# alexsmith1612/hadoofus

Measured on AMD Instinct MI355X. Metric: CRC32C verify GiB/s (device-resident), 512B chunks over 128MiB HDFS blocks, higher is better.
Workload: dtype u8; 1 GPU; C3 verify: 1024 x 128MiB HDFS blocks per GPU of splitmix64 data, 512B chunks, BE wire CRCs, 1/65537 chunks corrupted, bitmap + first-bad out; blocks_per_gpu=1024, block_bytes=134217728, chunk_size=512, parallelism=shard1

## Files before the change

hadoofus_amd/abi.py:

```python
import ctypes
import os

import numpy as np

HERE = os.path.dirname(os.path.abspath(__file__))
LIB_PATH = os.path.join(HERE, "lib", "libhadoofus_crc32c.so")

CSUM_NULL, CSUM_CRC32, CSUM_CRC32C = 0, 1, 2
ERR_UNSUPPORTED_CHECKSUM = 8
ERR_INVALID_PACKETHEADERPROTO = 18
ERR_PACKET_SIZE = 25
ERR_CRC_LEN = 26
ERR_UNEXPECTED_CRC_LEN = 27
ERR_UNEXPECTED_READ_OFFSET = 28
ERR_BAD_CHECKSUM = 29
ERR_BAD_LASTPACKET = 32
EIO = -5
READ_ALL = -1
AGAIN = 1000
ABI_VERSION = 5
MODE_COMPUTE, MODE_VERIFY = 0, 1
PROTO_V1, PROTO_V2 = 1, 2
SEG_BE, SEG_RAW, SEG_CRC32 = 1, 2, 4

# ... 84 lines not shown
    _bind(lib, "hdfs_crc32c_plan_kernel_ms", _int, [_vp, ctypes.POINTER(ctypes.c_double), ctypes.POINTER(_int)])
    _bind(lib, "hdfs_crc32c_plan_stats", _int, [_vp, ctypes.POINTER(_u64), ctypes.POINTER(_u64), ctypes.POINTER(_u64)])
    _bind(lib, "hdfs_crc32c_plan_destroy", None, [_vp])
    _bind(lib, "hdfs_crc32c_plan_time", _int, [_vp, _vp, _int, ctypes.POINTER(ctypes.c_double)])
    _bind(lib, "hdfs_crc32c_stream_dev", _int, [_u32, _vp, _u64, ctypes.POINTER(_u32)])
    _bind(lib, "hdfs_crc32c_stream_ex", _int, [_int, _u32, _vp, _u64, ctypes.POINTER(_u32)])
    _bind(lib, "hdfs_crc32c_verify_crcdata", _int,
          [_vp, ctypes.c_int32, ctypes.c_int32, ctypes.c_int32, _int, ctypes.POINTER(ctypes.c_int32)])
    _bind(lib, "hdfs_crc32c_compose_crcs", _int,
          [ctypes.POINTER(_vp), ctypes.POINTER(_sz), _int, _sz, _u32, _int, _vp])
    for name in ("hdfs_crc32c_parse_packets", "hdfs_crc32c_verify_packets"):
        _bind(lib, name, _int, [_vp, _u64, _int, _u32, _int, ctypes.POINTER(Packet), _sz,
                                ctypes.POINTER(_sz), ctypes.POINTER(_u64)])
    _bind(lib, "hdfs_crc32c_read_packets", _int,
          [_vp, _u64, _int, _u32, _int, ctypes.c_int64, ctypes.c_int64, ctypes.POINTER(IoVec), _int,
           ctypes.POINTER(Packet), _sz, ctypes.POINTER(_sz), ctypes.POINTER(_u64), ctypes.POINTER(_u64)])
    _bind(lib, "hdfs_crc32c_verify_packets_submit", _int,
          [_vp, _u64, _int, _u32, _int, _sz, ctypes.POINTER(_vp)])
    _bind(lib, "hdfs_crc32c_job_wait", _int,
          [_vp, ctypes.POINTER(Packet), _sz, ctypes.POINTER(_sz), ctypes.POINTER(_u64)])
    _bind(lib, "hdfs_crc32c_verify_blocks_submit", _int,
          [ctypes.POINTER(_vp), ctypes.POINTER(_u64), _sz, _int, _u32, _int, _sz, ctypes.POINTER(_vp)])
    _bind(lib, "hdfs_crc32c_job_wait_blocks", _int,
          [_vp, ctypes.POINTER(Packet), _sz, ctypes.POINTER(_sz), ctypes.POINTER(_u64), ctypes.POINTER(_int)])
    _bind(lib, "hdfs_crc32c_reader_open", _int,
          [_vp, _u64, _int, _u32, _int, ctypes.c_int64, ctypes.c_int64, _sz, ctypes.POINTER(_vp)])
    _bind(lib, "hdfs_crc32c_reader_next", _int,
          [_vp, ctypes.POINTER(IoVec), _int, ctypes.POINTER(Packet), _sz, ctypes.POINTER(_sz), ctypes.POINTER(_u64),
           ctypes.POINTER(_u64)])
    _bind(lib, "hdfs_crc32c_reader_close", None, [_vp])
    _bind(lib, "hdfs_crc32c_read_packets_fd", _int,
          [_vp, _u64, _int, _u32, _int, ctypes.c_int64, ctypes.c_int64, _int, ctypes.c_int64,
           ctypes.POINTER(Packet), _sz, ctypes.POINTER(_sz), ctypes.POINTER(_u64), ctypes.POINTER(_u64)])
    _bind(lib, "hdfs_crc32c_abi_version", _int, [])
    _bind(lib, "hdfs_crc32c_session_create", _int, [ctypes.POINTER(_vp), _int, _u32, _int, _u64, _sz])
    _bind(lib, "hdfs_crc32c_session_buffer", _int, [_vp, ctypes.POINTER(_vp), ctypes.POINTER(_u64)])
    _bind(lib, "hdfs_crc32c_session_commit", _int, [_vp, _u64])
    _bind(lib, "hdfs_crc32c_session_flush", _int, [_vp])
    _bind(lib, "hdfs_crc32c_session_poll", _int, [_vp, ctypes.POINTER(Packet), _sz, ctypes.POINTER(_sz), _int])
    _bind(lib, "hdfs_crc32c_session_pending", _int, [_vp, ctypes.POINTER(_u64), ctypes.POINTER(_sz)])
    _bind(lib, "hdfs_crc32c_session_destroy", None, [_vp])
    _bind(lib, "hdfs_crc32c_composite_crcs", _int, [ctypes.POINTER(Segment), _sz, ctypes.POINTER(_u32)])
    _bind(lib, "hdfs_crc32c_dev_alloc", _int, [ctypes.POINTER(_vp), _u64])
    _bind(lib, "hdfs_crc32c_dev_free", _int, [_vp])
    _bind(lib, "hdfs_crc32c_memcpy", _int, [_vp, _vp, _u64, _int])
    _bind(lib, "hdfs_crc32c_memset", _int, [_vp, _int, _u64])
    _bind(lib, "hdfs_crc32c_stream_create", _int, [ctypes.POINTER(_vp)])
    _bind(lib, "hdfs_crc32c_stream_destroy", _int, [_vp])
    _bind(lib, "hdfs_crc32c_stream_sync", _int, [_vp])
    _bind(lib, "hdfs_crc32c_fill_splitmix64", _int, [_vp, _u64, _u64, _u64, _vp])
    _bind(lib, "hdfs_crc32c_corrupt", _int, [_vp, _u64, _u32, _u64, _u64, _u64, _vp])
    _bind(lib, "hdfs_crc32c_device_sync", _int, [])
    _bind(lib, "hdfs_crc32c_mailbox_create", _int, [ctypes.POINTER(_vp), _u32])
    _bind(lib, "hdfs_crc32c_mailbox_stats", _int, [_vp, ctypes.POINTER(_u64), ctypes.POINTER(_u64)])
    _bind(lib, "hdfs_crc32c_mailbox_destroy", _int, [_vp])
    _bind(lib, "hdfs_crc32c_compose_packets", _int,
          [_vp, _u64, ctypes.c_int64, ctypes.c_int64, _int, _int, _int, _vp, _u64, ctypes.POINTER(OutPacket), _sz,
           ctypes.POINTER(_sz), ctypes.POINTER(_u64)])
    _bind(lib, "hdfs_crc32c_compute_host", _int, [_vp, _u64, _u32, _u32, _u32, _vp, _u64])
    _bind(lib, "hdfs_crc32c_verify_host", _int,
          [_vp, _u64, _u32, _u32, _u32, _vp, _vp, _u64, ctypes.POINTER(_u64), ctypes.POINTER(_u64)])
    _bind(lib, "hdfs_crc32c_host_alloc", _int, [ctypes.POINTER(_vp), _u64])
    _bind(lib, "hdfs_crc32c_host_free", _int, [_vp])
    return check_abi(lib)


def bind_diag(lib):
    _bind(lib, "hdfs_crc32c_set_tile_order", _int, [_int])
    _bind(lib, "hdfs_crc32c_set_group_shift", _int, [_int])
    _bind(lib, "hdfs_crc32c_set_xcd_major", _int, [_int])
    _bind(lib, "hdfs_crc32c_probe_read", _int, [_vp, _u64, _vp, _int, ctypes.POINTER(ctypes.c_double)])
    _bind(lib, "hdfs_crc32c_set_tuning", _int, [_int, _vp])
    _bind(lib, "hdfs_crc32c_set_probe", _int, [_int, _int, _int])
    _bind(lib, "hdfs_crc32c_set_depth", _int, [_int])
    _bind(lib, "hdfs_crc32c_set_shape", _int, [_int, _int])
    _bind(lib, "hdfs_crc32c_set_store_policy", _int, [_int])
    _bind(lib, "hdfs_crc32c_set_runs", _int, [_int])
    _bind(lib, "hdfs_crc32c_diag_device_checks", _int, [ctypes.POINTER(_u32), _int])
    _bind(lib, "hdfs_crc32c_set_speculation", _int, [_int])
    _bind(lib, "hdfs_crc32c_set_job_coalesce", _int, [_int])
    _bind(lib, "hdfs_crc32c_set_job_early", _int, [_int])
    _bind(lib, "hdfs_crc32c_diag_job_early", _int, [ctypes.POINTER(_u64), _int])
    _bind(lib, "hdfs_crc32c_diag_spec_stats", _int, [ctypes.POINTER(_u64), _int])
    _bind(lib, "hdfs_crc32c_diag_stream_queries", _int, [ctypes.POINTER(_u64)])
    _bind(lib, "hdfs_crc32c_diag_stream_queues", _int, [ctypes.POINTER(_u64)])
    _bind(lib, "hdfs_crc32c_diag_job_queues", _int, [ctypes.POINTER(_u64)])
    return lib


def load(path=LIB_PATH):
    global _lib
    if _lib is not None:
        return _lib
    if not os.path.exists(path):
        raise ImportError(f"{path} not built; run `python -m hadoofus_amd.build` "
                          "(or __graft_entry__.build())")
    _lib = bind_product(ctypes.CDLL(path))
    return _lib


def check_abi(lib):
    v = lib.hdfs_crc32c_abi_version()
    if v != ABI_VERSION:
        raise ImportError(f"library ABI version {v}, bindings written for {ABI_VERSION}")
    return lib


def _check(rc, lib=None):
    if rc != 0:
        raise CRC32CError(rc, (lib or load()).hdfs_crc32c_last_error().decode(errors="replace"))


def _host(buf):
    if isinstance(buf, np.ndarray):
        a = np.ascontiguousarray(buf)
        return a, a.ctypes.data, a.nbytes
    a = np.frombuffer(memoryview(buf).cast("B"), dtype=np.uint8)
    return a, (a.ctypes.data if a.nbytes else None), a.nbytes


def device_info(device=-1):
    arch = ctypes.create_string_buffer(64)
    ncu = _int(0)
    _check(load().hdfs_crc32c_device_info(device, arch, 64, ctypes.byref(ncu)))
    return arch.value.decode(), ncu.value


def init(device=-1):
    _check(load().hdfs_crc32c_init(device))


def bound_device():
    d = _int(-1)
    bus = ctypes.create_string_buffer(64)
    _check(load().hdfs_crc32c_bound_device(ctypes.byref(d), bus, 64))
    return d.value, bus.value.decode()


def crc32c(crc, buf, entry="_hdfs_crc32c"):
    keep, p, n = _host(buf)
    return getattr(load(), entry)(crc & 0xFFFFFFFF, p, n)


def stream_crc_dev(crc, dptr, nbytes):
    out = _u32(0)
    _check(load().hdfs_crc32c_stream_dev(crc & 0xFFFFFFFF, dptr, nbytes, ctypes.byref(out)))
    return out.value


def verify_crcdata(region, chunksize, crcdlen, dlen, ctype=CSUM_CRC32C):
    keep, p, n = _host(region)
    fb = ctypes.c_int32(-1)
    rc = load().hdfs_crc32c_verify_crcdata(p, chunksize, crcdlen, dlen, ctype, ctypes.byref(fb))
    if rc < 0:
        _check(rc)
    return rc, fb.value


def stream_ex(ctype, crc, buf):
    keep, p, n = _host(buf)
    out = _u32(0)
    _check(load().hdfs_crc32c_stream_ex(ctype, crc & 0xFFFFFFFF, p if n else None, n, ctypes.byref(out)))
    return out.value


def _packets(fn, stream, proto, chunk_size, ctype, max_pkts, dptr=None, nbytes=None, lib=None):
# ... 383 lines not shown
```

hadoofus_amd/csrc/crc32c_engine.cpp:

```cpp
#include <hip/hip_runtime.h>

#include <algorithm>
#include <cstdarg>
#include <cstdio>
#include <cstdlib>
#include <chrono>
#include <cstring>
#include <mutex>
#include <string>
#include <vector>

#include <unistd.h>

#include "crc32c_engine.h"
#include "crc32c_tables.h"
#ifdef HDFS_CRC32C_DIAG
#include "hadoofus_crc32c_diag.h"
#endif

namespace hdfs_crc32c {

thread_local char g_err[512] = "";

int fail(int code, const char *fmt, ...) {
  va_list ap;
  va_start(ap, fmt);
  vsnprintf(g_err, sizeof(g_err), fmt, ap);
  va_end(ap);
  return code;
}

DevCtx g_ctx[kMaxDev];
std::mutex g_init_mu;
std::atomic<int> g_bound_dev{-1};

#ifdef HDFS_CRC32C_DIAG
int env_int(const char *name, int dflt) {
  const char *e = std::getenv(name);
  return e ? std::atoi(e) : dflt;
}
#define HDFS_KNOB(name, dflt) env_int(name, dflt)
#else
#define HDFS_KNOB(name, dflt) (dflt)
#endif
int g_tile_order = HDFS_KNOB("HDFS_CRC32C_TILE_ORDER", 3);
int g_nt_loads = HDFS_KNOB("HDFS_CRC32C_NT", 2);
int g_depth = HDFS_KNOB("HDFS_CRC32C_DEPTH", 3);
int g_streams = HDFS_KNOB("HDFS_CRC32C_STREAMS", 1);
int g_block = HDFS_KNOB("HDFS_CRC32C_BLOCK", 1024);
uint32_t g_store_policy = uint32_t(HDFS_KNOB("HDFS_CRC32C_STORE", 0));
uint32_t g_group_shift = uint32_t(HDFS_KNOB("HDFS_CRC32C_GROUP", 3)) & 15u;
uint32_t g_xcd_major = uint32_t(HDFS_KNOB("HDFS_CRC32C_XCD", 1)) & 3u;
uint32_t g_spec_pool_min = uint32_t(HDFS_KNOB("HDFS_CRC32C_SPEC_POOL", 32)) & 255u;
uint32_t g_copy_wg_units = uint32_t(HDFS_KNOB("HDFS_CRC32C_COPY_WG_UNITS", 1024));
int g_copy_dev_tab = HDFS_KNOB("HDFS_CRC32C_COPY_DEV_TAB", 1);
int g_tail_small = HDFS_KNOB("HDFS_CRC32C_TAIL_SMALL", 1);
int g_tail_stream = HDFS_KNOB("HDFS_CRC32C_TAIL_STREAM", 1);
uint64_t g_mb_copy_max = uint64_t(HDFS_KNOB("HDFS_CRC32C_MB_COPY_MAX", 96 << 10));
int g_runs = HDFS_KNOB("HDFS_CRC32C_RUNS", 2);
int g_spec = HDFS_KNOB("HDFS_CRC32C_SPEC", 1);
int g_job_coalesce = HDFS_KNOB("HDFS_CRC32C_JOB_COALESCE", 1);
int g_job_early = HDFS_KNOB("HDFS_CRC32C_JOB_EARLY", 1);
std::atomic<uint64_t> g_job_early_stats[2];
int g_job_queues = HDFS_KNOB("HDFS_CRC32C_JOB_QUEUES", 1);
int g_stage_vram = HDFS_KNOB("HDFS_CRC32C_MB_STAGE", 1);
int g_mb_exp = HDFS_KNOB("HDFS_CRC32C_MB_EXP", 0);
int g_mb_queue = HDFS_KNOB("HDFS_CRC32C_MB_QUEUE", 1);
unsigned long long *g_diag = nullptr;


int stream_queue(hipStream_t s, uint64_t *dq, uint64_t *q) {
  HIPCHK(launch_queue_probe(dq, s));
  HIPCHK(hipMemcpyAsync(q, dq, sizeof(uint64_t), hipMemcpyDeviceToHost, s));
  HIPCHK(hipStreamSynchronize(s));
  return HDFS_CRC32C_OK;
}

int stream_on_own_queue(DevCtx &c, hipStream_t *s, uint64_t *q, const uint64_t *avoid, int n) {
  *s = nullptr;
  *q = 0;
  uint64_t *dq = nullptr;
  HIPCHK(hipMalloc(&dq, sizeof(uint64_t)));
  auto shared = [&](uint64_t x) {
    for (int i = 0; i < n; i++)
      if (avoid[i] && avoid[i] == x) return true;
    return false;
  };
  int rc = HDFS_CRC32C_OK;
  if (hipStreamCreateWithFlags(s, hipStreamNonBlocking) != hipSuccess) {
    (void)hipGetLastError();
    *s = nullptr;
    rc = fail(HDFS_CRC32C_EHIP, "stream");
  } else if (!(rc = stream_queue(*s, dq, q)) && g_job_queues && shared(*q)) {
    std::vector<uint32_t> mask(size_t((c.num_cu + 31) / 32), 0u);
    for (int cu = 0; cu < c.num_cu; cu++) mask[size_t(cu / 32)] |= 1u << (cu % 32);
    hipStream_t own = nullptr;
    uint64_t q2 = 0;
    if (hipExtStreamCreateWithCUMask(&own, uint32_t(mask.size()), mask.data()) != hipSuccess) {
      (void)hipGetLastError();
    } else if (!stream_queue(own, dq, &q2) && !shared(q2)) {
      (void)hipStreamDestroy(*s);
      *s = own;
      *q = q2;
    } else {
      (void)hipStreamDestroy(own);
    }
  }
  (void)hipFree(dq);
  return rc;
}

int queue_probe_streams(DevCtx &c) {
  uint64_t *dq = nullptr;
  HIPCHK(hipMalloc(&dq, sizeof(uint64_t)));
  int rc = stream_queue(c.stream, dq, &c.q_main);
  for (int k = 0; k < 2 && !rc; k++) {
    hipStream_t &s = k == 0 ? c.t_stream : c.cp_stream;
    uint64_t &q = k == 0 ? c.q_tail : c.q_copy;
    if ((rc = stream_queue(s, dq, &q))) break;
    if (q != c.q_main) continue;
    std::vector<uint32_t> mask(size_t((c.num_cu + 31) / 32), 0u);
    for (int cu = 0; cu < c.num_cu; cu++) mask[size_t(cu / 32)] |= 1u << (cu % 32);
    hipStream_t own = nullptr;
    uint64_t q2 = 0;
    if (hipExtStreamCreateWithCUMask(&own, uint32_t(mask.size()), mask.data()) != hipSuccess) {
      (void)hipGetLastError();
      continue;
    }
    if ((rc = stream_queue(own, dq, &q2))) break;
    if (q2 == c.q_main) {
      (void)hipStreamDestroy(own);
      continue;
    }
    (void)hipStreamDestroy(s);
    s = own;
    q = q2;
  }
  (void)hipFree(dq);
  return rc;
}

int ctx_init(int device, DevCtx **out) {
  int ndev = 0;
// ... 1297 lines not shown
    (void)hipFree(dq);
    if (rc) return rc;
  }
  const uint64_t ms = idle_ms ? idle_ms : 50u;
  c->mb_idle_ticks = uint32_t(std::min<uint64_t>(ms * 100000u, 0xFFFFFFFFu));
  c->mb_calls = c->mb_launches = 0;
  HIPCHK(hipStreamSynchronize(c->stream));
  c->mb_on = true;
  rc = mb_launch(*c, c->mb_posted);
  if (rc) {
    c->mb_on = false;
    return rc;
  }
  *mb = new hdfs_crc32c_mailbox{c->dev};
  return HDFS_CRC32C_OK;
}

int hdfs_crc32c_mailbox_stats(const hdfs_crc32c_mailbox *mb, uint64_t *calls, uint64_t *launches) {
  if (!mb) return fail(HDFS_CRC32C_EINVAL, "null mailbox");
  DevCtx &c = g_ctx[mb->dev];
  std::lock_guard<std::mutex> lk(c.mu);
  if (calls) *calls = c.mb_calls;
  if (launches) *launches = c.mb_launches;
  return HDFS_CRC32C_OK;
}

int hdfs_crc32c_mailbox_destroy(hdfs_crc32c_mailbox *mb) {
  if (!mb) return HDFS_CRC32C_OK;
  DevCtx &c = g_ctx[mb->dev];
  DeviceGuard g(mb->dev);
  delete mb;
  std::lock_guard<std::mutex> lk(c.mu);
  if (!c.mb_on) return HDFS_CRC32C_OK;
  c.mb_on = false;
  if (c.mb_alive && !mb_exited(c)) {
    mb_post(c, ++c.small_seq, 0u, kMbQuitFlag, 0u, nullptr);
  }
  c.mb_alive = false;
  HIPCHK(hipStreamSynchronize(c.mb_stream));
  return HDFS_CRC32C_OK;
}

#ifdef HDFS_CRC32C_DIAG
int hdfs_crc32c_diag_device_checks(uint32_t *out3, int reset) {
  if (!out3) return fail(HDFS_CRC32C_EINVAL, "null output");
  const hipError_t e = read_device_checks(out3, reset);
  if (e != hipSuccess) return fail(HDFS_CRC32C_EHIP, "reading the device checks: %s", hipGetErrorString(e));
  return HDFS_CRC32C_OK;
}

int hdfs_crc32c_set_store_policy(int policy) {
  if (policy < 0 || policy > 28) return fail(HDFS_CRC32C_EINVAL, "store policy 0..28");
  g_store_policy = uint32_t(policy);
  return HDFS_CRC32C_OK;
}

int hdfs_crc32c_diag_stream_queries(uint64_t *out) {
  DevCtx *c = nullptr;
  int rc = ctx_init(-1, &c);
  if (rc) return rc;
  if (!out) return fail(HDFS_CRC32C_EINVAL, "null out");
  *out = c->stream_queries;
  return HDFS_CRC32C_OK;
}

int hdfs_crc32c_diag_stream_queues(uint64_t *out4) {
  DevCtx *c = nullptr;
  int rc = ctx_init(-1, &c);
  if (rc) return rc;
  if (!out4) return fail(HDFS_CRC32C_EINVAL, "null out");
  out4[0] = c->q_main;
  out4[1] = c->q_tail;
  out4[2] = c->q_copy;
  out4[3] = c->q_mb;
  return HDFS_CRC32C_OK;
}

int hdfs_crc32c_set_speculation(int on) {
  if (on != 0 && on != 1) return fail(HDFS_CRC32C_EINVAL, "speculation 0 or 1");
  g_spec = on;
  return HDFS_CRC32C_OK;
}

int hdfs_crc32c_diag_job_queues(uint64_t *out4) {
  DevCtx *c = nullptr;
  int rc = ctx_init(-1, &c);
  if (rc) return rc;
  if (!out4) return fail(HDFS_CRC32C_EINVAL, "null out");
  std::lock_guard<std::mutex> lk(c->mu);
  for (int i = 0; i < kMaxJobs; i++) out4[i] = c->job_slot[i].q;
  return HDFS_CRC32C_OK;
}

int hdfs_crc32c_set_job_coalesce(int mode) {
  if (mode < 0 || mode > 3)
    return fail(HDFS_CRC32C_EINVAL, "job coalescing 0 (off), 1 (product), 2 (hold) or 3 (no lone run behind a launch)");
  g_job_coalesce = mode;
  return HDFS_CRC32C_OK;
}

int hdfs_crc32c_set_job_early(int on) {
  if (on < 0 || on > 1) return fail(HDFS_CRC32C_EINVAL, "per-run completion 0 (off) or 1 (product)");
  g_job_early = on;
  return HDFS_CRC32C_OK;
}

int hdfs_crc32c_diag_job_early(uint64_t *out2, int reset) {
  if (!out2) return fail(HDFS_CRC32C_EINVAL, "null out");
  for (int i = 0; i < 2; i++) out2[i] = reset ? g_job_early_stats[i].exchange(0) : g_job_early_stats[i].load();
  return HDFS_CRC32C_OK;
}

int hdfs_crc32c_set_runs(int on) {
  if (on < 0 || on > 4)
    return fail(HDFS_CRC32C_EINVAL, "runs 0 (schedule 3), 1 (schedule 4), 2 (gather), 3 (lazy gather) or 4 (columns)");
  g_runs = on;
  return HDFS_CRC32C_OK;
}

int hdfs_crc32c_set_depth(int depth) {
  if (depth < 2 || depth > 4) return fail(HDFS_CRC32C_EINVAL, "depth must be 2..4");
  g_depth = depth;
  return HDFS_CRC32C_OK;
}

int hdfs_crc32c_set_shape(int streams, int block) {
  if (streams != 1 && streams != 2 && streams != 4) return fail(HDFS_CRC32C_EINVAL, "streams must be 1, 2 or 4");
  if (block != 512 && block != 768 && block != 1024) return fail(HDFS_CRC32C_EINVAL, "block must be 512, 768 or 1024");
  g_streams = streams;
  g_block = block;
  return HDFS_CRC32C_OK;
}

int hdfs_crc32c_set_tuning(int nt_loads, void *diag) {
  if (nt_loads < 0 || nt_loads > 2) return fail(HDFS_CRC32C_EINVAL, "nt_loads 0..2");
  g_nt_loads = nt_loads;
  g_diag = static_cast<unsigned long long *>(diag);
  return HDFS_CRC32C_OK;
}

int hdfs_crc32c_set_group_shift(int shift) {
  if (shift < 0 || shift > 6) return fail(HDFS_CRC32C_EINVAL, "group shift must be 0..6");
  g_group_shift = uint32_t(shift);
  return HDFS_CRC32C_OK;
}

int hdfs_crc32c_set_xcd_major(int on) {
  if (on < 0 || on > 2) return fail(HDFS_CRC32C_EINVAL, "xcd_major must be 0, 1 or 2");
  g_xcd_major = uint32_t(on);
  return HDFS_CRC32C_OK;
}

int hdfs_crc32c_set_tile_order(int order) {
  if (order < 0 || order > 3) return fail(HDFS_CRC32C_EINVAL, "tile order must be 0..3");
  g_tile_order = order;
  return HDFS_CRC32C_OK;
}

int g_probe_variant = 0, g_probe_grid_per_cu = 2, g_probe_block = 1024;

int hdfs_crc32c_set_probe(int variant, int grid_per_cu, int block) {
  g_probe_variant = variant;
  g_probe_grid_per_cu = grid_per_cu > 0 ? grid_per_cu : 2;
  g_probe_block = block > 0 ? block : 1024;
  return HDFS_CRC32C_OK;
}
// ... 76 lines not shown
```

hadoofus_amd/csrc/crc32c_engine.h:

```cpp
#pragma once
#include <hip/hip_runtime.h>

#include <atomic>
#include <cstdarg>
#include <cstddef>
#include <cstdint>
#include <initializer_list>
#include <mutex>
#include <vector>

#include "crc32c_hostpin.h"
#include "crc32c_internal.h"
#include "hadoofus_crc32c.h"

namespace hdfs_crc32c {

hipError_t launch_tiles(int mode, int order, int nt, int depth, int streams, int block, int grid,
                        const SegDev *segs, uint32_t nseg, uint64_t total_rounds, uint64_t total_tiles,
                        const uint32_t *gtab, uint32_t *first_bad, unsigned long long *mism,
                        unsigned long long *diag, uint32_t tune, uint32_t *gctr, hipStream_t stream,
                        int copy = 0, int una = 0, const GridSummary *dyn = nullptr, uint32_t utiles = 0,
                        int fuse_generic = 0);
hipError_t launch_probe_read(const uint8_t *p, uint64_t nbytes, uint32_t *out, int grid, int block, int variant,
                             hipStream_t stream);
hipError_t launch_generic(int mode, const SegDev *segs, uint32_t nseg, uint64_t total_gtiles,
                          const uint32_t *gtab, uint32_t *first_bad, unsigned long long *mism,
                          hipStream_t stream, const GridSummary *dyn = nullptr);
hipError_t launch_combine(const uint32_t *raws, uint64_t nraw, uint32_t cs, uint64_t len,
                          const uint32_t *pow2, uint32_t reg0, uint32_t *acc, hipStream_t stream);
hipError_t launch_fill(uint64_t *out, uint64_t nwords, uint64_t seed, uint64_t g0, hipStream_t stream);
hipError_t launch_corrupt(uint8_t *data, uint64_t len, uint32_t cs, uint64_t chunk0, uint64_t modulus,
                          uint64_t bitmul, hipStream_t stream);
hipError_t launch_composite(const SegDev *segs, uint32_t nseg, const uint64_t *run_prefix, uint64_t total_runs,
                            const uint32_t *pow2, uint32_t *out, hipStream_t stream);
hipError_t launch_small_chunks(int mode, const uint8_t *p, uint32_t len, uint32_t exact, uint32_t cs, uint32_t reg0,
                               uint32_t be, const uint32_t *expect, const uint32_t *tab, const uint32_t *kx,
                               uint32_t poly, uint32_t *meta, uint32_t *crcs, uint32_t seq, hipStream_t stream);
hipError_t launch_prep(uint32_t *fb, uint32_t nfb, unsigned long long *mism, uint32_t *gctr, hipStream_t stream);
hipError_t launch_queue_probe(uint64_t *out, hipStream_t stream);
int stream_queue(hipStream_t s, uint64_t *dq, uint64_t *q);
hipError_t launch_mailbox(const uint32_t *req, const uint8_t *in, uint32_t *meta, uint32_t *crcs, const uint32_t *tab0,
                          const uint32_t *tab1, const uint32_t *kx, uint32_t *status, uint32_t epoch, uint32_t seq0,
                          uint32_t idle_ticks, uint32_t exp, hipStream_t stream);
hipError_t launch_gather(const uint8_t *raw, const PktDesc *descs, uint32_t npk, uint32_t units, uint8_t *arena,
                         uint8_t *crc_arena, hipStream_t stream);
hipError_t launch_header_window(const uint8_t *s, uint64_t len, uint64_t base, uint64_t stride, uint32_t count,
                                int proto, uint8_t *out, uint64_t *stride_out, hipStream_t stream);

hipError_t launch_copy_pieces(const CopyPieces &a, int grid, hipStream_t stream);
hipError_t launch_copy_beside(const CopyPieces &a, int grid, hipStream_t stream);
hipError_t launch_small_run(const uint8_t *s, uint64_t len, uint32_t count, int proto, uint32_t cs, int ctype,
                            int verify, const uint32_t *tab, const uint32_t *pow2, uint8_t *copy_dst,
                            uint64_t copy_cap, int win, int64_t client_offset, uint8_t *hout, uint32_t seq,
                            hipStream_t stream);
hipError_t launch_frame_grid(const uint8_t *s, uint64_t len, uint64_t base, uint32_t count, int proto, uint32_t cs,
                             int ctype, int verify, uint32_t sflags, uint8_t *bm_base, uint8_t *copy_base,
                             uint64_t copy_cap, int win, int64_t client_offset, GridBufs g, hipStream_t stream,
                             unsigned long long *stamps = nullptr);
hipError_t launch_spec_verify(const SpecArgs &a, int grid, int copy, hipStream_t stream);
extern int g_spec;
extern int g_job_coalesce;
extern int g_job_early;
extern std::atomic<uint64_t> g_job_early_stats[2];
extern int g_job_queues;
extern unsigned long long *g_diag;
constexpr size_t kFrameStampOff = 65536;
hipError_t launch_grid_finalize(const SegDev *segs, uint32_t nseg, const uint32_t *seg2pkt, const uint32_t *fb,
                                GridBad *bad, uint32_t bad_cap, GridSummary *sum, uint8_t *hsum2, uint32_t host_cap,
                                uint32_t seq, hipStream_t stream);

extern thread_local char g_err[512];
int fail(int code, const char *fmt, ...);
hipError_t read_device_checks(uint32_t out[3], int reset);
int device_checks(const char *call);

#define HIPCHK(expr)                                                                   \
  do {                                                                                 \
    hipError_t e_ = (expr);                                                            \
    if (e_ != hipSuccess)                                                              \
      return ::hdfs_crc32c::fail(HDFS_CRC32C_EHIP, "%s: %s (%s:%d)", #expr,            \
                                 hipGetErrorString(e_), __FILE__, __LINE__);           \
  } while (0)

constexpr int kMaxDev = 64;
constexpr uint32_t kStreamPiece = 4096;
constexpr size_t kStageCap = size_t(64) << 20;
constexpr size_t kSmallIn = kSmallMax + size_t(kSmallMaxChunks) * 4 + 64;
constexpr uint32_t kSmallMeta = 16;
constexpr size_t kSmallOut = (kSmallMeta + size_t(kSmallMaxChunks)) * 4;

struct PieceSlot {
  uint8_t *raw = nullptr, *arena = nullptr, *crc = nullptr, *meta = nullptr;
  size_t raw_cap = 0, arena_cap = 0, crc_cap = 0, meta_cap = 0;
  uint32_t *gctr = nullptr;
  unsigned long long *mism = nullptr;
  hipEvent_t copied = nullptr;
  hipEvent_t done = nullptr;
};

struct CopyCtl {
  uint32_t *hdone = nullptr, *ddone = nullptr, *count = nullptr;
  uint32_t seq = 0;
  uint8_t *htab = nullptr, *dtab = nullptr;
  size_t tab_cap = 0;
  uint8_t *vtab = nullptr;
  size_t vtab_cap = 0;
};

struct SpecSlot {
  SpecCtl *ctl = nullptr;
  SpecExc *exc = nullptr;
  SpecRunTail *xtail = nullptr;
  SpecTabData *tabs = nullptr;
  uint8_t *h = nullptr, *hd = nullptr;
  uint64_t n = 0;
  hipStream_t stream = nullptr;
  uint64_t q = 0;
  uint8_t *scratch = nullptr;
  uint64_t scratch_cap = 0;
};
constexpr int kMaxJobs = 4;
constexpr size_t kMaxJobsOut = 64;
struct JobQueue;

struct DevCtx {
  std::atomic<bool> ready{false};
  int dev = -1;
  int num_cu = 0;
  int num_xcd = 8;
  char arch[64] = "";
  uint32_t *d_tab_main_t[2] = {nullptr, nullptr};
  uint32_t *d_tab_pow2_t[2] = {nullptr, nullptr};
  uint32_t *d_tab_kx = nullptr;
  hipStream_t stream = nullptr;
  uint8_t *h_stage = nullptr;
  uint8_t *d_stage = nullptr;
  uint32_t *d_raw = nullptr;
  size_t raw_cap = 0;
  SegDev *d_seg = nullptr;
  uint32_t *d_small = nullptr;
  uint8_t *h_small_in = nullptr, *dv_small_in = nullptr;
  uint8_t *stage_vram = nullptr;
  uint32_t *h_small_out = nullptr, *dv_small_out = nullptr;
  uint32_t small_seq = 0;
  std::atomic<uint64_t> queued_epoch{0}, confirmed_epoch{0};
  bool unconfirmed() const {
    return queued_epoch.load(std::memory_order_acquire) != confirmed_epoch.load(std::memory_order_acquire);
  }
  void confirm(uint64_t e) {
    uint64_t cur = confirmed_epoch.load(std::memory_order_acquire);
    while (cur < e && !confirmed_epoch.compare_exchange_weak(cur, e, std::memory_order_acq_rel)) {
    }
  }
  uint64_t stream_queries = 0;
  void *d_crc_scratch = nullptr;
  uint64_t crc_scratch_cap = 0;
  hipStream_t copy_stream = nullptr, comp_stream = nullptr;
  hipEvent_t ev_copy[2] = {nullptr, nullptr}, ev_comp[2] = {nullptr, nullptr};
  uint8_t *p_data[2] = {nullptr, nullptr};
  uint32_t *p_crc[2] = {nullptr, nullptr};
  uint8_t *p_bm[2] = {nullptr, nullptr};
  size_t p_cap = 0;
  size_t p_chunk_cap = 0;
  SegDev *p_segs = nullptr;
  uint32_t *p_fb = nullptr;
  uint32_t *p_gctr = nullptr;
  unsigned long long *p_mism = nullptr;
  size_t p_npieces_cap = 0;
  PieceSlot kslot[2];
  uint8_t *k_hmeta = nullptr;
  size_t k_hmeta_cap = 0;
  uint8_t *w_dev = nullptr, *w_host = nullptr;
  uint32_t w_cap = 0;
  struct VBatch {
    uint8_t *h = nullptr, *d = nullptr;
    size_t hcap = 0, dcap = 0;
  };
  std::vector<VBatch> v_batch;
  hipStream_t v_stream = nullptr;
  struct GridSlot {
    uint8_t *d = nullptr, *h = nullptr;
    size_t dcap = 0, hcap = 0;
    uint8_t *hd = nullptr;
  };
  uint32_t grid_seq = 0;
  uint8_t *sr_h = nullptr, *sr_hd = nullptr;
  uint8_t *sr2_h = nullptr, *sr2_hd = nullptr;
  hipStream_t t_stream = nullptr;
  uint64_t q_main = 0, q_tail = 0, q_copy = 0, q_mb = 0;
  hipStream_t r_stream = nullptr;
  std::vector<GridSlot> grid;
  SpecSlot spec;
  SpecSlot job_slot[kMaxJobs];
  bool job_busy[kMaxJobs] = {};
  JobQueue *jobq = nullptr;
  std::mutex rd_mu;
  uint8_t *rd_stage = nullptr;
  uint64_t rd_stage_cap = 0;
  CopyCtl cp;
  CopyCtl cp_beside;
  hipStream_t cp_stream = nullptr;
  std::mutex beside_mu;
  std::vector<CopyCtl> cp_pool;
  bool mb_on = false, mb_alive = false;
  uint32_t *h_mb = nullptr, *dv_mb = nullptr;
  uint32_t *mb_req = nullptr, *mb_req_d = nullptr;
  uint32_t mb_posted = 0;
  hipStream_t mb_stream = nullptr;
  uint32_t mb_epoch = 0, mb_idle_ticks = 0;
  uint64_t mb_calls = 0, mb_launches = 0;
  std::vector<hipStream_t> user_streams;
  int bulk_cus() const { return num_cu - (mb_on ? num_xcd : 0); }
  std::mutex mu;
};

extern DevCtx g_ctx[kMaxDev];
int stream_on_own_queue(DevCtx &c, hipStream_t *s, uint64_t *q, const uint64_t *avoid, int n);

struct DeviceGuard {
  int prev = -1;
  bool changed = false;
  explicit DeviceGuard(int dev) {
    if (hipGetDevice(&prev) == hipSuccess && prev != dev) {
      changed = hipSetDevice(dev) == hipSuccess;
    }
  }
  ~DeviceGuard() {
    if (changed) (void)hipSetDevice(prev);
  }
};

int ctx_init(int device, DevCtx **out);
void classify(SegDev &s, uint64_t &rounds, uint64_t &gtiles, uint64_t &mtiles);
int fill_seg(const hdfs_crc32c_segment &in, int mode, SegDev &s, size_t idx);
inline int seg_ctype(uint32_t flags) { return (flags & HDFS_CRC32C_SEG_CRC32) ? 1 : 0; }
bool device_accessible(const void *p);
int launch_all(DevCtx &c, int mode, const SegDev *d_segs, uint32_t nseg, uint64_t rounds, uint64_t mtiles,
               uint64_t gtiles, uint32_t *d_fb, unsigned long long *d_mism, uint32_t *d_gctr, hipStream_t st,
               hipEvent_t ev0 = nullptr, hipEvent_t ev1 = nullptr, bool reset = true, int ctype = 0,
               bool copy = false, bool gctr_zeroed = false, bool una = false, uint32_t utiles = 0,
               bool runs = false);
bool whole_groups(const SegDev *segs, size_t n);
uint32_t uniform_tiles(const SegDev *segs, size_t n);
int launch_verify_dyn(DevCtx &c, const SegDev *d_segs, const GridSummary *dyn, uint64_t rounds_ub, uint64_t gtiles_ub,
                      uint32_t *d_fb, unsigned long long *d_mism, uint32_t *d_gctr, hipStream_t st, int ctype,
                      bool copy);
uint32_t tile_tune();
extern uint32_t g_spec_pool_min;
extern uint32_t g_copy_wg_units;
extern int g_copy_dev_tab;
bool any_unaligned(const SegDev *segs, size_t n);
int pipe_reserve(DevCtx &c, size_t piece, uint32_t cs, size_t npieces);
int mailbox_copy(DevCtx &c, const CopyEntry *e, uint32_t n);
extern uint64_t g_mb_copy_max;
extern int g_tail_small;
extern int g_tail_stream;

bool small_ok(uint64_t len, uint64_t cs);
int small_call(DevCtx &c, int mode, uint32_t len, uint32_t cs, uint32_t reg0, bool be, int ctype,
               const uint8_t *dsrc = nullptr, const uint8_t *hsrc = nullptr, const uint8_t *hcrc = nullptr,
               uint32_t crc_bytes = 0);
int chunk_crcs_to_host(const void *data, uint64_t len, uint32_t cs, int ctype, uint32_t *out_be);
int host_pipeline(int mode, const uint8_t *data, uint64_t len, uint32_t cs, uint32_t flags, uint32_t crc_init,
                  void *crcs, uint8_t *bitmap, uint64_t piece_req, uint64_t *first_bad, uint64_t *mismatches);

PinRegistry &pins();
struct HostPins {
  PinRegistry::Scope s;
  std::vector<hipStream_t> drain;
  bool finished = false;
  explicit HostPins(std::initializer_list<hipStream_t> st) : s(pins()), drain(st) {}
  HostPins(const HostPins &) = delete;
  HostPins &operator=(const HostPins &) = delete;
  ~HostPins() {
    if (!finished)
      for (hipStream_t st : drain)
        if (st) (void)hipStreamSynchronize(st);
  }
  int pin(std::initializer_list<std::pair<const void *, size_t>> bufs);
  int done(int rc);
};

inline uint64_t align_up(uint64_t v, uint64_t a) { return (v + a - 1) / a * a; }

}
```

hadoofus_amd/csrc/crc32c_internal.h:

```cpp
#pragma once
#include <cstdint>

struct hdfs_crc32c_packet;

namespace hdfs_crc32c {

#ifdef HDFS_CRC32C_DIAG
constexpr bool kDiag = true;
#else
constexpr bool kDiag = false;
#endif

enum DevCheckKernel : uint32_t {
  kDkFrameGrid = 1,
  kDkGridBuild = 2,
  kDkHeaderWindow = 3,
  kDkSmallRun = 4,
  kDkFinalize = 5,
  kDkSpecEarly = 6,
};

enum : uint32_t {
  kSegBigEndian = 1u,
  kSegRaw = 2u,
};

enum Mode : int { kModeCompute = 0, kModeVerify = 1, kModeLoadOnly = 2 };

struct SegDev {
  const uint8_t *data;
  uint32_t *crcs;
  uint8_t *bitmap;
  uint64_t mtile_start;
  uint32_t chunk_size;
  uint32_t flags;
  uint32_t nchunks;
  uint32_t main_tiles;
  uint32_t reg_init;
  uint32_t gen_tiles;
  uint64_t len;
  uint64_t round_start;
  uint64_t gtile_start;
  uint8_t *copy_dst;
  uint32_t copy_w0, copy_w1;
};
static_assert(sizeof(SegDev) == 96, "SegDev layout");

enum : uint32_t {
  kGridOn = 0,
  kGridOff = 1,
  kGridStop = 2,
  kGridMore = 3,
};
struct GridSummary {
  uint32_t first_break;
  uint32_t recorded;
  uint32_t last_status;
  uint32_t nseg;
  uint64_t stride;
  uint64_t rounds, mtiles, gtiles;
  uint64_t payload;
  uint64_t consumed;
  uint64_t next_pos;
  uint64_t bm_bytes;
  uint32_t nbad;
  uint32_t unaligned;
  uint32_t seq;
  uint32_t nonuni;
  uint32_t utiles;
  uint32_t nexc;
};
constexpr uint32_t kExcMax = 64;
constexpr uint32_t kGridRecBytes = 56;
constexpr uint32_t kGridHostRec0 = 256;
constexpr uint32_t kGridHostIdx = kGridHostRec0 + 64;
constexpr uint32_t kGridHostExc = kGridHostIdx + kExcMax * 4;
constexpr uint32_t kGridHostBytes = kGridHostExc + kExcMax * kGridRecBytes;
struct GridBufs {
  ::hdfs_crc32c_packet *recs;
  void *look;
  SegDev *segs;
  uint32_t *seg2pkt;
  uint32_t *fb;
  uint32_t *gctr;
  uint32_t *done;
  uint32_t *exc;
  GridSummary *sum;
  uint8_t *hsum;
  uint32_t seq;
};
constexpr uint32_t kGridLookBytes = 256;

constexpr uint32_t kSpecExcMax = 64;
struct SpecExc {
  uint64_t rec[7];
  uint32_t k, pad;
};
static_assert(sizeof(SpecExc) == 64, "SpecExc");
struct SpecCtl {
  unsigned long long mism;
  uint32_t gctr;
  uint32_t done;
// ... 1 lines not shown
  uint32_t tail_status;
  uint64_t tail_total;
  uint64_t tail[7];
  uint32_t nexc, pad0;
  uint32_t run_done[16];
  uint32_t run_mism[16];
  uint32_t run_bad, pad1[7];
};
static_assert(sizeof(SpecCtl) == 256, "SpecCtl");
struct SpecEarly {
  uint64_t r0[7];
  uint64_t stride;
  uint32_t eligible;
  uint32_t count;
  uint32_t seq;
  uint32_t pad[13];
};
struct SpecFinal {
  unsigned long long mism;
  uint32_t exc, tail_status;
  uint64_t tail_total;
  uint64_t tail[7];
  uint32_t seq, nexc;
  uint32_t pad[10];
};
static_assert(sizeof(SpecEarly) == 128 && sizeof(SpecFinal) == 128, "spec host blocks");
constexpr uint32_t kSpecRunsMax = 16;
struct SpecRunEarly {
  uint64_t r0[7];
  uint32_t count;
  uint32_t early;
};
static_assert(kSpecRunsMax == 16, "SpecCtl's per-run words");
struct SpecRunTail {
  uint64_t rec[7];
  uint64_t total;
  uint32_t status, seq;
};
struct SpecRunDone {
  uint32_t seq, mism, bad, pad;
};
static_assert(sizeof(SpecRunEarly) == 64 && sizeof(SpecRunTail) == 72 && sizeof(SpecRunDone) == 16, "spec run blocks");
constexpr size_t kSpecRunEarlyOff = 256 + size_t(kSpecExcMax) * sizeof(SpecExc);
constexpr size_t kSpecRunTailOff = kSpecRunEarlyOff + size_t(kSpecRunsMax) * sizeof(SpecRunEarly);
constexpr size_t kSpecRunDoneOff = kSpecRunTailOff + size_t(kSpecRunsMax) * sizeof(SpecRunTail);
constexpr size_t kSpecHostBytes = kSpecRunDoneOff + size_t(kSpecRunsMax) * sizeof(SpecRunDone);
struct SpecTabData {
  const uint8_t *crc0;
  uint8_t *bm0, *copy_base;
  uint64_t stride, copy_cap;
  uint32_t nch, cs, cb0, nruns;
  uint64_t um;
  uint32_t per, pad;
  const uint8_t *crc0r[kSpecRunsMax];
  SpecCtl *ctl;
  uint8_t *hdone;
  uint32_t seq, pad1;
};
static_assert(sizeof(SpecTabData) == 56 + 16 + 128 + 24, "SpecTabData");
struct SpecArgs {
  const uint8_t *s;
  uint64_t len, base;
  uint32_t max_count;
  int proto, ctype;
  uint32_t cs, sflags;
  int rwin;
  int64_t client_offset;
  uint8_t *bm;
  uint8_t *copy_base;
  uint64_t copy_cap;
  const uint32_t *gtab;
  uint32_t *fb;
  SpecCtl *ctl;
  SpecExc *exc;
  uint32_t parity, seq, tune;
  uint8_t *hout;
  SpecTabData *tabs;
  unsigned long long *stamps;
  uint32_t nruns;
  uint32_t early;
  const uint8_t *xs[kSpecRunsMax];
  uint64_t xlen[kSpecRunsMax];
  SpecRunTail *xtail;
};
constexpr size_t kSpecStampOff = 98304;
constexpr uint64_t kSpecMaxStride = uint64_t(1) << 26;

struct GridBad {
  uint32_t pkt;
  int32_t first_bad;
  uint32_t bad_chunks;
  uint32_t pad;
};


constexpr uint32_t kLdsSliceBytes = 131072;
constexpr uint32_t kLdsZposBytes = 7 * 4096;
constexpr uint32_t kLdsBytes = kLdsSliceBytes + kLdsZposBytes;
constexpr uint32_t kLdsWords = kLdsBytes / 4;

constexpr uint32_t kTabSliceWords = 1024;
constexpr uint32_t kTabZposWords = 7 * 1024;
constexpr uint32_t kTabMainWords = kTabSliceWords + kTabZposWords;
constexpr uint32_t kPow2Levels = 48;
constexpr uint32_t kTabPow2Words = kPow2Levels * 1024;

constexpr uint32_t kTabKxWords = 1088;

struct PktDesc {
  uint64_t src_crc;
  uint64_t dst_data;
  uint64_t dst_crc;
  uint32_t dlen;
  uint32_t ncrc;
  uint32_t unit0;
  uint32_t nunits;
};
constexpr uint32_t kGatherSlice = 65536;
constexpr uint32_t kHdrWin = 64;

constexpr uint32_t kGridMaxCount = 65536;
constexpr uint32_t kGridGroups = kGridMaxCount / 64 / 64;

constexpr uint32_t kSmallRunMax = 64;
constexpr uint32_t kCopyPiecesMax = 32;
constexpr uint32_t kCopyBlocksMax = 512;
constexpr uint32_t kCopyTabBlocks = 4096;
constexpr uint32_t kCopyTabGrid = 1024;
constexpr uint32_t kCopyTabStage = 64;
struct CopyEntry {
  const uint8_t *src;
  uint8_t *dst;
  uint32_t len, uend;
};
static_assert(sizeof(CopyEntry) == 24, "CopyEntry layout (the mailbox reads it as 6 words)");
struct CopyPieces {
  const uint8_t *src[kCopyPiecesMax];
  uint8_t *dst[kCopyPiecesMax];
  uint32_t len[kCopyPiecesMax];
  uint32_t uend[kCopyPiecesMax];
  uint32_t n, seq;
  uint32_t *done;
  uint32_t *count;
  const CopyEntry *tab;
  const uint32_t *wg0;
  uint32_t per, total;
  unsigned long long *stamps;
};
constexpr size_t kCopyStampOff = 110592;
inline uint32_t copy_units(uintptr_t d, uint64_t len) {
  return len ? uint32_t(((d + len + 15u) & ~uintptr_t(15)) - (d & ~uintptr_t(15))) / 16u : 0u;
}
constexpr uint32_t kSrSlot = 128;
constexpr uint32_t kSrHostBytes = kSmallRunMax * kSrSlot;
constexpr uint64_t kSmallRunBytes = uint64_t(kSmallRunMax) * (65536 + 4096);

constexpr uint32_t kSmallMax = 65536;
constexpr uint32_t kSmallMaxChunks = 2048;

constexpr uint32_t kMbVerifyFlag = 1u << 24, kMbBeFlag = 1u << 25, kMbCrc32Flag = 1u << 26, kMbQuitFlag = 1u << 27;
constexpr uint32_t kMbDevFlag = 1u << 28;
constexpr uint32_t kMbCopyFlag = 1u << 29;


constexpr uint32_t kRoundBytes = 512;
constexpr uint32_t kTileChunks = 8;
// ... 3 lines not shown
```

hadoofus_amd/csrc/crc32c_kernels.hip:

```cpp
#include <hip/hip_runtime.h>

#include "crc32c_frame.h"
#include "crc32c_internal.h"

namespace hdfs_crc32c {

#define DEV __device__ __forceinline__

typedef uint32_t u32x4 __attribute__((ext_vector_type(4)));
#define GAS __attribute__((address_space(1)))
DEV u32x4 gload16(const void *p) { return *(const GAS u32x4 *)(const GAS uint8_t *)p; }
DEV u32x4 gload16_nt(const void *p) {
  return __builtin_nontemporal_load((const GAS u32x4 *)(const GAS uint8_t *)p);
}
DEV uint32_t gload32(const void *p) { return *(const GAS uint32_t *)(const GAS uint8_t *)p; }
DEV uint8_t gload8(const void *p) { return *(const GAS uint8_t *)p; }
DEV void gstore32(void *p, uint32_t v) { *(GAS uint32_t *)(GAS uint8_t *)p = v; }
DEV void gstore8(void *p, uint8_t v) { *(GAS uint8_t *)p = v; }

DEV uint32_t lds_at(const uint32_t *lds, uint32_t byteaddr) {
  return *reinterpret_cast<const uint32_t *>(reinterpret_cast<const char *>(lds) + byteaddr);
}

template <int CTRL>
// ... 8 lines not shown

DEV uint32_t xor3(uint32_t a, uint32_t b, uint32_t c) { return __builtin_amdgcn_bitop3_b32(a, b, c, 0x96); }

DEV uint32_t slice4(const uint32_t *lds, uint32_t x, uint32_t next, uint32_t lb0, uint32_t lb1) {
  const uint32_t a0 = __builtin_amdgcn_perm(x, lb0, 0x0C020400u);
  const uint32_t a1 = __builtin_amdgcn_perm(x, lb0, 0x0C020500u);
  const uint32_t a2 = __builtin_amdgcn_perm(x, lb1, 0x0C020600u);
  const uint32_t a3 = __builtin_amdgcn_perm(x, lb1, 0x0C020700u);
  return xor3(xor3(lds_at(lds, a0), lds_at(lds, a1 + 128u), lds_at(lds, a2)), lds_at(lds, a3 + 128u), next);
}

DEV uint32_t zshift(const uint32_t *lds, uint32_t base, uint32_t x) {
  const uint32_t *t = lds + base;
  return t[x & 0xffu] ^ t[256u + ((x >> 8) & 0xffu)] ^ t[512u + ((x >> 16) & 0xffu)] ^
         t[768u + (x >> 24)];
}

DEV void transpose(uint32_t (&d)[16]) {
#pragma unroll
  for (int c = 0; c < 4; c++) {
#pragma unroll
    for (int k = 0; k < 4; k += 2) {
      const auto r = __builtin_amdgcn_permlane16_swap(d[k * 4 + c], d[(k + 1) * 4 + c], false, false);
      d[k * 4 + c] = r[0];
      d[(k + 1) * 4 + c] = r[1];
    }
  }
#pragma unroll
  for (int c = 0; c < 4; c++) {
#pragma unroll
    for (int k = 0; k < 2; k++) {
      const auto r = __builtin_amdgcn_permlane32_swap(d[k * 4 + c], d[(k + 2) * 4 + c], false, false);
      d[k * 4 + c] = r[0];
      d[(k + 2) * 4 + c] = r[1];
    }
  }
}

DEV uint32_t rfl(uint32_t x) { return __builtin_amdgcn_readfirstlane(x); }
DEV uint64_t rfl64(uint64_t x) {
  return (static_cast<uint64_t>(rfl(static_cast<uint32_t>(x >> 32))) << 32) | rfl(static_cast<uint32_t>(x));
}

#ifdef HDFS_CRC32C_DIAG
__device__ uint32_t g_dchk[4];
DEV bool dchk(bool ok, uint32_t kid, uint32_t line) {
  if (!ok && atomicAdd(&g_dchk[2], 1u) == 0u) {
    g_dchk[0] = kid;
    g_dchk[1] = line;
  }
  return ok;
}
#define DCHK(c, kid) dchk((c), (kid), __LINE__)
#else
#define DCHK(c, kid) true
#endif

#define CAS __attribute__((address_space(4)))
typedef const CAS SegDev *SegP;

struct SegHot {
  const uint8_t *data;
  uint32_t *crcs;
  uint8_t *bitmap;
  uint64_t mtile_start;
  uint32_t chunk_size, flags, nchunks, main_tiles;
};
static_assert(sizeof(SegHot) == 48, "SegHot is the head of SegDev");
DEV SegHot seg_hot(SegP segs, uint32_t s) {
  const CAS SegHot *p = reinterpret_cast<const CAS SegHot *>(&segs[s]);
  return SegHot{p->data, p->crcs, p->bitmap, p->mtile_start, p->chunk_size, p->flags, p->nchunks, p->main_tiles};
}

DEV void spec_run_contribute(SpecCtl *ctl, uint8_t *hdone, uint32_t seq, uint32_t target, uint32_t r) {
  const uint32_t n = __hip_atomic_fetch_add(&ctl->run_done[r], 1u, __ATOMIC_RELAXED, __HIP_MEMORY_SCOPE_AGENT);
  if (n + 1u != target) return;
  const uint32_t mism = __hip_atomic_load(&ctl->run_mism[r], __ATOMIC_RELAXED, __HIP_MEMORY_SCOPE_AGENT);
  const uint32_t bad = (__hip_atomic_load(&ctl->run_bad, __ATOMIC_RELAXED, __HIP_MEMORY_SCOPE_AGENT) >> r) & 1u;
  *(volatile GAS u32x4 *)(GAS uint8_t *)(hdone + sizeof(SpecRunDone) * r) = u32x4{seq, mism, bad, 0u};
}

constexpr uint32_t kEarlyWords = 50, kEarlyOff = 0xFFFFFFFFu;

template <bool BATCH>
struct SpecTabT {
  const CAS SpecTabData *p;
  uint32_t *e;
  DEV uint32_t early_ok(uint32_t nk) const {
    if constexpr (BATCH) return rfl(e[49] != 0u && e[48] == nk ? 1u : 0u);
    return 0u;
  }
  DEV void tile_done(uint32_t k, uint32_t byte, uint32_t lane) const {
    if constexpr (BATCH) {
      const uint32_t r = rfl(static_cast<uint32_t>(__umul64hi(static_cast<uint64_t>(k), p->um)));
      SpecCtl *const ctl = p->ctl;
      if (byte) {
        if (lane == 0)
          __hip_atomic_fetch_add(&ctl->run_mism[r], static_cast<uint32_t>(__builtin_popcount(byte)), __ATOMIC_RELAXED,
                                 __HIP_MEMORY_SCOPE_AGENT);
        __builtin_amdgcn_s_waitcnt(0x0F70);
      }
      uint32_t old = 0;
      if (lane == 0) old = __hip_atomic_fetch_add(&e[r], 1u, __ATOMIC_RELAXED, __HIP_MEMORY_SCOPE_WORKGROUP);
      old = __builtin_amdgcn_readlane(old, 0);
      if (old + 1u == rfl(e[16u + r]) && lane == 0) spec_run_contribute(ctl, p->hdone, p->seq, e[32u + r], r);
    }
  }
  DEV SegDev operator[](uint32_t k) const {
    SegDev d;
    SpecTabData q;
    q.crc0 = p->crc0;
    q.bm0 = p->bm0;
    q.copy_base = p->copy_base;
    q.stride = p->stride;
    q.copy_cap = p->copy_cap;
    q.nch = p->nch;
    q.cs = p->cs;
    q.cb0 = p->cb0;
    const uint32_t T = (q.nch + kTileChunks - 1u) / kTileChunks, dlen = q.nch * q.cs;
    const uint8_t *c;
    if constexpr (BATCH) {
      const uint32_t r = static_cast<uint32_t>(__umul64hi(static_cast<uint64_t>(k), p->um));
      c = p->crc0r[r] + static_cast<uint64_t>(k - r * p->per) * q.stride;
    } else {
      c = q.crc0 + static_cast<uint64_t>(k) * q.stride;
    }
    d.data = c + 4u * q.nch;
    d.crcs = reinterpret_cast<uint32_t *>(const_cast<uint8_t *>(c));
    d.bitmap = q.bm0 + static_cast<uint64_t>(k) * T;
    d.mtile_start = static_cast<uint64_t>(k) * T;
    d.chunk_size = q.cs;
    d.flags = kSegBigEndian;
    d.nchunks = q.nch;
    d.main_tiles = T;
    d.reg_init = 0xFFFFFFFFu;
    d.gen_tiles = 0u;
    d.len = dlen;
    d.round_start = static_cast<uint64_t>(k) * T * (q.cs / kRoundBytes);
    d.gtile_start = 0u;
    const uint32_t w0 = k ? 0u : q.cb0;
    const uint64_t before = k ? static_cast<uint64_t>(k) * dlen - q.cb0 : 0u;
    uint64_t at = 0;
    uint32_t clen = 0;
    frame::read_place(before, dlen - w0, q.copy_cap, at, clen);
    d.copy_dst = q.copy_base && clen ? q.copy_base + at : nullptr;
    d.copy_w0 = w0;
    d.copy_w1 = w0 + clen;
    return d;
  }
};
using SpecTab = SpecTabT<false>;
template <class Tab>
struct TabEarly {
  static constexpr bool value = false;
};
template <>
struct TabEarly<SpecTabT<true>> {
  static constexpr bool value = true;
};
template <bool BATCH>
DEV SegHot seg_hot(const SpecTabT<BATCH> &t, uint32_t k) {
  const SegDev d = t[k];
  return SegHot{d.data, d.crcs, d.bitmap, d.mtile_start, d.chunk_size, d.flags, d.nchunks, d.main_tiles};
}

struct SegCache {
  uint32_t seg;
  uint32_t reg_init;
  SegHot h;
};
template <class Tab>
DEV const SegCache &hot(SegCache &k, Tab segs, uint32_t s) {
  if (s != k.seg) {
    k.h = seg_hot(segs, s);
    k.reg_init = segs[s].reg_init;
    k.seg = s;
  }
  return k;
}

struct Cursor {
  uint32_t seg, tile, r;
  bool valid;
  uint32_t grp = 0;
};

constexpr uint32_t kUnitMaxShift = 8, kUnitMinShift = 4;
constexpr uint32_t kColBytes = 128;
constexpr uint32_t kColShift = 2;
constexpr uint32_t kSlots = 8;
#ifndef HDFS_GATHER_SLOTS
#define HDFS_GATHER_SLOTS 8
#endif
static_assert((HDFS_GATHER_SLOTS & (HDFS_GATHER_SLOTS - 1)) == 0, "gather slots: a power of two");
constexpr uint32_t kGatherSlots = HDFS_GATHER_SLOTS, kGatherWords = kGatherSlots * 65;
#ifndef HDFS_PHASE1_NUM
#define HDFS_PHASE1_NUM 23
#endif
constexpr uint64_t kPhase1Num = HDFS_PHASE1_NUM, kPhase1Den = 25;

struct Sched {
  uint64_t r1;
  uint64_t gfirst;
  uint32_t nk;
  uint32_t *ctr;
  uint32_t lane;
  uint64_t p2first;
  uint64_t ntiles;
  uint32_t *gctr;
  uint64_t *slots;
  uint32_t ushift;
  uint32_t gstride;
  uint32_t gshift;
  uint32_t ut, ush;
  uint64_t um;
};

DEV Cursor ulocate(const Sched &w, uint64_t g) {
  const uint32_t s = w.ush != 0xFFFFFFFFu ? static_cast<uint32_t>(g >> w.ush) : static_cast<uint32_t>(__umul64hi(g, w.um));
  return Cursor{rfl(s), rfl(static_cast<uint32_t>(g - uint64_t(s) * w.ut)), 0u, true};
}

DEV uint32_t grab(const Sched &w) {
  uint32_t k = 0;
  if (w.lane == 0) k = atomicAdd(w.ctr, 1u);
  return rfl(k);
}

template <int ORDER>
DEV bool ticket_tile(const Sched &w, uint32_t t, uint64_t &g) {
  if (t < w.nk) {
    if (ORDER == 4 || ORDER == 7)
      g = (w.gfirst + uint64_t(t) * w.gstride) << w.gshift;
    else if (ORDER == 3)
      g = ((w.gfirst + uint64_t(t >> w.gshift) * w.gstride) << w.gshift) + (t & ((1u << w.gshift) - 1u));
    else
      g = w.gfirst + t;
    return true;
  }
  if (ORDER < 2) return false;
  const uint32_t tsh = (ORDER == 4 || ORDER == 7) ? w.gshift : 0u;
  const uint32_t j = t - w.nk, u = j >> (w.ushift - tsh), o = (j & ((1u << (w.ushift - tsh)) - 1u)) << tsh,
                 s = u % kSlots;
  if (o == 0) {
    uint32_t gu = 0;
    if (w.lane == 0) gu = atomicAdd(w.gctr, 1u);
    gu = rfl(gu);
    if (w.lane == 0)
      __hip_atomic_store(&w.slots[s], (uint64_t(u + 1) << 32) | gu, __ATOMIC_RELAXED, __HIP_MEMORY_SCOPE_WORKGROUP);
  }
  uint64_t v;
  for (;;) {
    v = __hip_atomic_load(&w.slots[s], __ATOMIC_RELAXED, __HIP_MEMORY_SCOPE_WORKGROUP);
    if (rfl(static_cast<uint32_t>(v >> 32)) == u + 1) break;
    __builtin_amdgcn_s_sleep(2);
  }
  g = w.p2first + (uint64_t(rfl(static_cast<uint32_t>(v))) << w.ushift) + o;
  return g < w.ntiles;
}

constexpr uint64_t kWalkTiles = 64;

template <class Tab>
DEV Cursor locate(Tab segs, uint32_t s, uint64_t g) {
  while (g >= segs[s].mtile_start + segs[s].main_tiles) s++;
  return Cursor{rfl(s), rfl(static_cast<uint32_t>(g - segs[s].mtile_start)), 0u, true};
}

template <int ORDER, class Tab>
DEV Cursor find_tile(const Cursor c, const SegHot &sh, Tab segs, uint32_t nseg, const Sched &w, uint64_t g) {
  const uint64_t end = sh.mtile_start + sh.main_tiles;
  if (w.ut && (g < sh.mtile_start || g >= end)) return ulocate(w, g);
  if (g < sh.mtile_start || g >= end + (ORDER >= 3 ? 0u : kWalkTiles)) {
    uint32_t lo = 0, hi = nseg;
    while (hi - lo > 1) {
      const uint32_t mid = (lo + hi) >> 1;
      if (segs[mid].mtile_start <= g) lo = mid; else hi = mid;
    }
    return locate(segs, lo, g);
  }
  if (g < end)
    return Cursor{c.seg, rfl(static_cast<uint32_t>(g - sh.mtile_start)), 0u, true};
  return locate(segs, c.seg, g);
}

template <int ORDER, class Tab>
DEV Cursor advance(Cursor c, Tab segs, uint32_t nseg, const Sched &w, SegCache &kc) {
  if (!c.valid) return c;
  const SegHot &sh = hot(kc, segs, c.seg).h;
  if (c.r + 1 < (ORDER == 7 ? sh.chunk_size / kColBytes : sh.chunk_size / kRoundBytes)) {
    c.r++;
    return c;
  }
  if (ORDER == 4 && ((c.tile + 1u) & ((1u << w.gshift) - 1u)) != 0u) {
    c.tile++;
    c.r = 0;
    return c;
  }
  if (ORDER != 0) {
    uint64_t g;
    const uint32_t tk = grab(w);
    if (!ticket_tile<ORDER>(w, tk, g)) {
      c.valid = false;
      return c;
    }
    Cursor n = find_tile<ORDER>(c, sh, segs, nseg, w, g);
    n.grp = tk >> 3;
    return n;
  }
  uint32_t s = c.seg, t = c.tile + 1;
  while (s < nseg && t >= segs[s].main_tiles) {
    t = 0;
    s++;
  }
  if (s >= nseg || segs[s].round_start + uint64_t(t) * (segs[s].chunk_size / kRoundBytes) >= w.r1) {
    c.valid = false;
    return c;
  }
  return Cursor{rfl(s), rfl(t), 0u, true};
}
// ... 480 lines not shown
        c = lds_at(lds, L.lb1 + 128u + (((c ^ gload8(p++)) & 0xffu) << 8)) ^ (c >> 8);
        n--;
      }
      out = (flags & kSegRaw) ? c : ~c;
    }
  }
  bool bad = false;
  if (valid) {
    uint32_t e = gload32(segs[s].crcs + chunk);
    if (flags & kSegBigEndian) e = __builtin_bswap32(e);
    bad = e != out;
  }
  const uint64_t m = __ballot(bad);
  if (active && g == 0) {
    const uint32_t byte = static_cast<uint32_t>((m >> (L.lane & 56u)) & 0xffu);
    gstore8(segs[s].bitmap + tile, static_cast<uint8_t>(byte));
    if (byte) {
      atomicMin(&first_bad[s], tile * kTileChunks + __builtin_ctz(byte));
      atomicAdd(mism, static_cast<unsigned long long>(__builtin_popcount(byte)));
    }
  }
}

template <int BLOCK>
DEV void bad_list(const SegDev *__restrict__ segs, uint32_t nseg, const uint32_t *__restrict__ seg2pkt,
                  const uint32_t *__restrict__ fb, GridBad *__restrict__ bad, uint32_t bad_cap,
                  GridSummary *__restrict__ sum, uint8_t *__restrict__ hsum2, uint32_t host_cap, uint32_t seq,
                  uint32_t *nb) {
  if (threadIdx.x == 0) *nb = 0u;
  __syncthreads();
  auto *hbad = reinterpret_cast<GridBad *>(hsum2 + 256);
  for (uint32_t i0 = threadIdx.x; i0 < nseg; i0 += 16u * BLOCK) {
    uint32_t f[16];
#pragma unroll
    for (uint32_t u = 0; u < 16; u++) f[u] = i0 + u * BLOCK < nseg ? fb[i0 + u * BLOCK] : 0xFFFFFFFFu;
#pragma unroll
    for (uint32_t u = 0; u < 16; u++) {
      if (f[u] == 0xFFFFFFFFu) continue;
      const uint32_t i = i0 + u * BLOCK;
      const SegDev d = segs[i];
      const uint32_t nbyte = (d.nchunks + 7u) / 8u;
      uint32_t n = 0;
      for (uint32_t j0 = 0; j0 < nbyte; j0 += 16u) {
        uint32_t by[16];
#pragma unroll
        for (uint32_t u = 0; u < 16; u++) by[u] = j0 + u < nbyte ? uint32_t(d.bitmap[j0 + u]) : 0u;
#pragma unroll
        for (uint32_t u = 0; u < 16; u++) {
          uint32_t byte = by[u];
          if (j0 + u == d.nchunks / 8u) byte &= (1u << (d.nchunks % 8u)) - 1u;
          n += __builtin_popcount(byte);
        }
      }
      const uint32_t slot = atomicAdd(nb, 1u);
      const GridBad g{seg2pkt[i], int32_t(f[u]), n, 0u};
      if (slot < bad_cap) bad[slot] = g;
      if (slot < host_cap) hbad[slot] = g;
    }
  }
  __syncthreads();
  if (threadIdx.x == 0) {
    sum->nbad = *nb;
    reinterpret_cast<GridSummary *>(hsum2)->nbad = *nb;
  }
  __threadfence_system();
  __syncthreads();
  if (threadIdx.x == 0)
    __hip_atomic_store(&reinterpret_cast<GridSummary *>(hsum2)->seq, seq, __ATOMIC_RELAXED, __HIP_MEMORY_SCOPE_SYSTEM);
}

template <int BLOCK>
DEV void fused_generic(const uint32_t *lds, const SegDev *__restrict__ segs, const GridSummary *__restrict__ dyn,
                       const LaneConst &L, uint32_t *__restrict__ first_bad, unsigned long long *__restrict__ mism) {
  const uint32_t nseg = dyn->nseg;
  const uint64_t ngt = dyn->gtiles;
  const uint64_t nw = uint64_t(gridDim.x) * (BLOCK / 64);
  const uint64_t wid = uint64_t(blockIdx.x) * (BLOCK / 64) + (threadIdx.x >> 6);
  for (uint64_t g0 = wid * 8u; g0 < ngt; g0 += nw * 8u) {
    const uint64_t gt = g0 + (L.lane >> 3);
    fused_generic_chunk(lds, segs, nseg, gt, gt < ngt, L, first_bad, mism);
  }
}

template <int BLOCK, int GATHER>
DEV void fill_tables(uint32_t *lds, const uint32_t *__restrict__ gtab) {
  if (threadIdx.x < 2 + 2 * kSlots) lds[kLdsWords + threadIdx.x] = 0u;
  if (GATHER && threadIdx.x < kGatherSlots) lds[kLdsWords + 2 + 2 * kSlots + threadIdx.x] = threadIdx.x << 4;
  constexpr uint32_t kStores = kLdsSliceBytes / 16;
  constexpr uint32_t kQ = (kStores + BLOCK - 1) / BLOCK;
  constexpr uint32_t kZ = (kTabZposWords / 4 + BLOCK - 1) / BLOCK;
  uint32_t v[kQ];
#pragma unroll
  for (uint32_t k = 0; k < kQ; k++) {
    const uint32_t idx = 4u * min(k * BLOCK + threadIdx.x, kStores - 1u);
    const uint32_t P = idx >> 14, e = (idx >> 6) & 255u, h = (idx >> 5) & 1u;
    v[k] = gtab[(3u - (2u * P + h)) * 256u + e];
  }
  u32x4 z[kZ];
#pragma unroll
  for (uint32_t k = 0; k < kZ; k++) {
    const uint32_t q = k * BLOCK + threadIdx.x;
    z[k] = q < kTabZposWords / 4 ? gload16(gtab + kTabSliceWords + 4u * q) : u32x4{0u, 0u, 0u, 0u};
  }
#pragma unroll
  for (uint32_t k = 0; k < kQ; k++) {
    const uint32_t q = k * BLOCK + threadIdx.x;
    if (kStores % BLOCK == 0 || q < kStores)
      *reinterpret_cast<u32x4 *>(&lds[4u * q]) = u32x4{v[k], v[k], v[k], v[k]};
  }
#pragma unroll
  for (uint32_t k = 0; k < kZ; k++) {
    const uint32_t q = k * BLOCK + threadIdx.x;
    if (q < kTabZposWords / 4) *reinterpret_cast<u32x4 *>(&lds[kLdsSliceBytes / 4 + 4u * q]) = z[k];
  }
}

template <int MODE, int ORDER, int NT, int DEPTH, int S, int BLOCK, int BUF, int COPY, int UNA, int GATHER,
          class Tab>
DEV void tiles_run(uint32_t *lds, const Tab sg, const SegDev *__restrict__ segs, uint32_t nseg, uint64_t total_rounds,
                   uint64_t total_tiles, uint32_t *__restrict__ first_bad, unsigned long long *__restrict__ mism,
                   unsigned long long *__restrict__ diag, uint32_t tune, uint32_t *__restrict__ gctr,
                   const GridSummary *__restrict__ dyn, uint32_t utiles, bool fused) {
  static_assert(ORDER != 0 || S == 1, "static per-wave slices serve one stream");
  static_assert(ORDER != 7 || (MODE == kModeCompute && S == 1 && BUF && !COPY && !UNA && !GATHER), "columns shape");
  static_assert(DEPTH >= 2 && DEPTH <= 4 && S >= 1 && S <= 4, "shape");
  static_assert(GATHER == 0 || (MODE == kModeCompute && ORDER == 3 && S == 1), "gather: compute, schedule 3");
  LaneConst L;
  L.store_policy = EP::policy(tune & 0xffu);
  L.lane = threadIdx.x & 63u;
  L.hsel = (L.lane >> 3) & 1u;
  L.loff = 16u * (4u * (L.lane & 7u) + (L.lane >> 4));
  L.lb0 = (L.lane & 31u) * 4u;
  L.lb1 = 65536u + (L.lane & 31u) * 4u;
  L.qi = L.lane & 7u;
  L.qg = L.lane >> 3;
  L.zk = 7u - L.qi;
  L.zbase = kLdsSliceBytes / 4 + (L.zk ? L.zk - 1u : 0u) * 1024u;
  L.z448 = kLdsSliceBytes / 4 + 6u * 1024u;
  L.z64 = kLdsSliceBytes / 4;
  L.ntiles = total_tiles;
  L.gslot = &lds[kLdsWords + 2 + 2 * kSlots];
  L.rmask = 7u;
  L.early = 0u;

  constexpr uint32_t wpb = BLOCK / 64;
  const uint32_t wave = rfl(blockIdx.x * wpb + (threadIdx.x >> 6));
  const uint32_t nwaves = gridDim.x * wpb;
  if (kDiag && diag && L.lane == 0) diag[3 * wave] = __builtin_amdgcn_s_memrealtime();
  uint64_t nrounds = 0;
  Sched w{0, 0, 0, &lds[kLdsWords], L.lane};
  w.ut = utiles;
  w.ush = (utiles & (utiles - 1u)) == 0u ? static_cast<uint32_t>(__builtin_ctz(utiles | (utiles == 0u ? 1u : 0u)))
                                         : 0xFFFFFFFFu;
  w.um = (utiles && w.ush == 0xFFFFFFFFu) ? ~0ull / utiles + 1ull : 0ull;
  Cursor cur[DEPTH][S];
#pragma unroll
  for (int s = 0; s < S; s++) cur[0][s] = Cursor{0u, 0u, 0u, false};
  if (ORDER == 0) {
    Cursor &c0 = cur[0][0];
    const uint64_t r0 = rfl64(total_rounds * wave / nwaves);
    w.r1 = rfl64(total_rounds * (wave + 1) / nwaves);
    if (r0 < w.r1) {
      const uint64_t g = tile_at_round(sg, nseg, r0, total_tiles);
      if (g < total_tiles) {
        uint32_t lo = 0, hi = nseg;
        while (hi - lo > 1) {
          const uint32_t mid = (lo + hi) >> 1;
          if (sg[mid].mtile_start <= g) lo = mid; else hi = mid;
        }
        c0 = locate(sg, lo, g);
        c0.valid = sg[c0.seg].round_start + uint64_t(c0.tile) * (sg[c0.seg].chunk_size / kRoundBytes) < w.r1;
      }
    }
  } else {
    const uint32_t pmin = (tune >> 16) & 0xffu;
    const bool pool = ORDER >= 2 && total_rounds >= uint64_t(pmin ? pmin : 32u) * nwaves * S;
    if (ORDER >= 3) {
      w.gshift = ORDER == 7 ? kColShift : ORDER == 4 ? min((tune >> 8) & 15u, 3u) : (tune >> 8) & 15u;
      if (ORDER == 4) L.rmask = (1u << w.gshift) - 1u;
      const uint64_t ngroups = (pool ? total_tiles * kPhase1Num / kPhase1Den : total_tiles) >> w.gshift;
      const uint32_t b = blockIdx.x, G = gridDim.x, xm = (tune >> 12) & 3u;
      if (xm == 2u && (G % 8u) == 0 && ngroups >= 8ull * (G / 8u)) {
        const uint64_t ngx = ngroups / 8u;
        const uint32_t G8 = G / 8u, l = b / 8u;
        w.gfirst = (b % 8u) * ngx + l;
        w.gstride = G8;
        w.nk = static_cast<uint32_t>(((ngx - 1 - l) / G8 + 1) << (ORDER == 4 || ORDER == 7 ? 0u : w.gshift));
        w.p2first = (ngx * 8u) << w.gshift;
      } else {
        w.gfirst = xm != 0u && (G % 8u) == 0 ? (b % 8u) * (G / 8u) + b / 8u : b;
        w.gstride = gridDim.x;
        w.nk = ngroups > w.gfirst
                   ? static_cast<uint32_t>(((ngroups - 1 - w.gfirst) / gridDim.x + 1) << (ORDER == 4 || ORDER == 7 ? 0u : w.gshift))
                   : 0u;
        w.p2first = ngroups << w.gshift;
      }
    } else {
      const uint64_t r_static = pool ? total_rounds * kPhase1Num / kPhase1Den : total_rounds;
      const uint64_t b0 = rfl64(r_static * blockIdx.x / gridDim.x);
      const uint64_t b1 = rfl64(r_static * (blockIdx.x + 1) / gridDim.x);
      w.gfirst = tile_at_round(sg, nseg, b0, total_tiles);
      w.nk = static_cast<uint32_t>(tile_at_round(sg, nseg, b1, total_tiles) - w.gfirst);
      w.p2first = tile_at_round(sg, nseg, r_static, total_tiles);
    }
    w.ntiles = total_tiles;
    if constexpr (TabEarly<Tab>::value) L.early = sg.early_ok(w.nk);
    {
      const uint64_t per = (total_tiles - w.p2first) / (4ull * gridDim.x);
      w.ushift = per >= (1ull << kUnitMaxShift) ? kUnitMaxShift
               : per < (1ull << kUnitMinShift) ? kUnitMinShift
                                               : 63u - static_cast<uint32_t>(__builtin_clzll(per));
    }
    w.gctr = gctr;
    w.slots = reinterpret_cast<uint64_t *>(&lds[kLdsWords + 2]);
#pragma unroll
    for (int s = 0; s < S; s++) {
      uint64_t g;
      const uint32_t tk = grab(w);
      if (ticket_tile<ORDER>(w, tk, g)) {
        if (w.ut) {
          cur[0][s] = ulocate(w, g);
        } else {
          uint32_t lo = 0, hi = nseg;
          while (hi - lo > 1) {
            const uint32_t mid = (lo + hi) >> 1;
            if (sg[mid].mtile_start <= g) lo = mid; else hi = mid;
          }
          cur[0][s] = locate(sg, lo, g);
        }
        cur[0][s].grp = tk >> 3;
      }
    }
  }
  bool any = false;
#pragma unroll
  for (int s = 0; s < S; s++) any |= cur[0][s].valid;
  if (!any) {
    if constexpr (MODE == kModeVerify)
      if (fused) fused_generic<BLOCK>(lds, segs, dyn, L, first_bad, mism);
    if (kDiag && diag && L.lane == 0) diag[3 * wave + 1] = __builtin_amdgcn_s_memrealtime();
    return;
  }
#pragma unroll
  for (int s = 1; s < S; s++)
    if (!cur[0][s].valid) cur[0][s] = Cursor{cur[0][0].seg, cur[0][0].tile, cur[0][0].r, false};

  uint32_t buf[DEPTH][S][16];
  uint32_t ex[DEPTH][S];
  uint32_t tl[DEPTH][S];
  uint32_t sha[DEPTH][S];
  uint32_t st[S];
  Gst gs[S];
  LaneOff lo{0u, {0u, 0u, 0u, 0u}, 0u};
  SegCache kc[S];
#pragma unroll
  for (int s = 0; s < S; s++) {
    st[s] = 0u;
    gs[s] = Gst{0u, 0u, 0u, 0u, kNoSlot, 0u, 0u, 0u, 0u, nullptr};
    kc[s].seg = 0xFFFFFFFFu;
  }
#pragma unroll
  for (int k = 1; k < DEPTH; k++) {
#pragma unroll
    for (int s = 0; s < S; s++) cur[k][s] = advance<ORDER>(cur[k - 1][s], sg, nseg, w, kc[s]);
  }
#pragma unroll
  for (int k = 0; k < DEPTH; k++) {
#pragma unroll
    for (int s = 0; s < S; s++) {
      ex[k][s] = 0u;
      tl[k][s] = 0u;
      sha[k][s] = 0u;
      issue<MODE, NT, BUF, UNA, ORDER == 7>(buf[k][s], ex[k][s], tl[k][s], sha[k][s], cur[k][s], sg, L.hsel, L.loff, L.qg, L.lane,
                                lo, kc[s], L.store_policy);
    }
    if (k + 1 < DEPTH) {
      constexpr int RUN = ORDER == 7 ? 4 : (ORDER == 4 && MODE == kModeCompute) ? 1 : GATHER == 2 ? 3 : GATHER ? 2 : 0;
#pragma unroll
      for (int j = 0; j < S * round_stores<MODE, COPY, RUN>(); j++) pad_store(first_bad);
    }
  }
  for (uint32_t it = 0;; it++) {
    EP::loop_hook(L.store_policy, it);
#pragma unroll
    for (int k = 0; k < DEPTH; k++) {
      process<MODE, S, COPY, UNA,
              ORDER == 7 ? 4 : (ORDER == 4 && MODE == kModeCompute) ? 1 : GATHER == 2 ? 3 : GATHER ? 2 : 0>(
          lds, buf[k], ex[k], tl[k], sha[k], cur[k], sg, st, L, first_bad, mism, kc, gs);
#pragma unroll
      for (int s = 0; s < S; s++) nrounds += cur[k][s].valid ? 1u : 0u;
      const int prev = (k + DEPTH - 1) % DEPTH;
#pragma unroll
      for (int s = 0; s < S; s++) {
        cur[k][s] = advance<ORDER>(cur[prev][s], sg, nseg, w, kc[s]);
        issue<MODE, NT, BUF, UNA, ORDER == 7>(buf[k][s], ex[k][s], tl[k][s], sha[k][s], cur[k][s], sg, L.hsel, L.loff, L.qg,
                                  L.lane, lo, kc[s], L.store_policy);
      }
    }
    bool more = false;
#pragma unroll
    for (int s = 0; s < S; s++) more |= cur[0][s].valid;
    if (!more) break;
  }
  if constexpr (GATHER == 2) {
#pragma unroll
    for (int s = 0; s < S; s++) {
      lazy_pre(gs[s], cur[0][s], sg, kc[s], L);
      lazy_flush<EP>(gs[s], hot(kc[s], sg, cur[0][s].seg).h, L);
    }
  }
  if constexpr (MODE == kModeVerify)
    if (fused) fused_generic<BLOCK>(lds, segs, dyn, L, first_bad, mism);
  if (kDiag && diag && L.lane == 0) {
    diag[3 * wave + 1] = __builtin_amdgcn_s_memrealtime();
    diag[3 * wave + 2] = nrounds;
  }
}

template <int MODE, int ORDER, int NT, int DEPTH, int S, int BLOCK, int BUF = 0, int COPY = 0, int UNA = 0,
          int GATHER = 0>
__global__ __launch_bounds__(BLOCK) void crc32c_tiles_kernel(
    const SegDev *__restrict__ segs, uint32_t nseg, uint64_t total_rounds, uint64_t total_tiles,
    const uint32_t *__restrict__ gtab, uint32_t *__restrict__ first_bad,
    unsigned long long *__restrict__ mism, unsigned long long *__restrict__ diag, uint32_t tune,
    uint32_t *__restrict__ gctr, const GridSummary *__restrict__ dyn, uint32_t utiles, uint32_t fuse) {
  const bool fused = MODE == kModeVerify && dyn && fuse;
  if (dyn) {
    nseg = dyn->nseg;
    total_rounds = dyn->rounds;
    total_tiles = dyn->mtiles;
    utiles = dyn->utiles;
  }
  __shared__ __attribute__((aligned(16))) uint32_t lds[kLdsWords + 2 + 2 * kSlots + (GATHER ? kGatherWords : 0)];
  fill_tables<BLOCK, GATHER>(lds, gtab);
  __syncthreads();
  tiles_run<MODE, ORDER, NT, DEPTH, S, BLOCK, BUF, COPY, UNA, GATHER>(lds, (SegP)(segs), segs, nseg, total_rounds,
                                                                       total_tiles, first_bad, mism, diag, tune, gctr,
                                                                       dyn, utiles, fused);
}


template <int MODE>
__global__ __launch_bounds__(256) void crc32c_generic_kernel(
    const SegDev *__restrict__ segs, uint32_t nseg, uint64_t total_gtiles,
    const uint32_t *__restrict__ gtab, uint32_t *__restrict__ first_bad,
    unsigned long long *__restrict__ mism, const GridSummary *__restrict__ dyn) {
  if (dyn) {
    nseg = dyn->nseg;
    total_gtiles = dyn->gtiles;
  }
// ... 1137 lines not shown
    sum->utiles = (sum->nonuni || (sum->mtiles >> 32)) ? 0u : T;
    GridSummary h = *sum;
    h.seq = 0u;
    *reinterpret_cast<GridSummary *>(hsum) = h;
    const uint64_t *x = reinterpret_cast<const uint64_t *>(&recs[0]);
    uint64_t *y = reinterpret_cast<uint64_t *>(hsum + kGridHostRec0);
    for (int q = 0; q < int(kGridRecBytes / 8); q++) y[q] = x[q];
  }
  for (uint32_t j = t; j < min(nexc, kExcMax); j += kGridBlock) {
    const uint32_t i = exc[j];
    reinterpret_cast<uint32_t *>(hsum + kGridHostIdx)[j] = i;
    const uint64_t *x = reinterpret_cast<const uint64_t *>(&recs[i]);
    uint64_t *y = reinterpret_cast<uint64_t *>(hsum + kGridHostExc + size_t(j) * kGridRecBytes);
    for (int q = 0; q < int(kGridRecBytes / 8); q++) y[q] = x[q];
  }
  __threadfence_system();
  __syncthreads();
  if (t == 0)
    __hip_atomic_store(&reinterpret_cast<GridSummary *>(hsum)->seq, seq, __ATOMIC_RELAXED, __HIP_MEMORY_SCOPE_SYSTEM);
  stamp(6);
}

__global__ __launch_bounds__(1024) void grid_finalize_kernel(const SegDev *__restrict__ segs, uint32_t nseg,
                                                             const uint32_t *__restrict__ seg2pkt,
                                                             const uint32_t *__restrict__ fb,
                                                             GridBad *__restrict__ bad, uint32_t bad_cap,
                                                             GridSummary *__restrict__ sum, uint8_t *__restrict__ hsum2,
                                                             uint32_t host_cap, uint32_t seq) {
  __shared__ uint32_t nb;
  if (nseg == 0xFFFFFFFFu) nseg = sum->nseg;
  if (!DCHK(nseg <= bad_cap, kDkFinalize)) nseg = bad_cap;
  bad_list<1024>(segs, nseg, seg2pkt, fb, bad, bad_cap, sum, hsum2, host_cap, seq, &nb);
}

DEV bool spec_canonical(const uint8_t *w, int proto, uint32_t hl) {
  if (proto == HDFS_CRC32C_PROTO_V1) return hl == 25u;
  const uint32_t n = hl - 6u;
  const uint8_t *p = w + 6;
  return (n == 25u || n == 27u) && p[0] == 0x09 && p[9] == 0x11 && p[18] == 0x18 && p[19] < 0x80 && p[20] == 0x25 &&
         (n == 25u || (p[25] == 0x28 && p[26] < 0x80));
}

template <uint32_t J>
DEV uint32_t spec_hdr_byte(uint32_t b0, bool v1, uint64_t off, uint64_t sq) {
  uint32_t e1 = b0, e2 = b0;
  if constexpr (J >= 4 && J < 12) e1 = static_cast<uint32_t>(off >> (8 * (11 - J))) & 0xffu;
  if constexpr (J >= 12 && J < 20) e1 = static_cast<uint32_t>(sq >> (8 * (19 - J))) & 0xffu;
  if constexpr (J >= 7 && J < 15) e2 = static_cast<uint32_t>(off >> (8 * (J - 7))) & 0xffu;
  if constexpr (J >= 16 && J < 24) e2 = static_cast<uint32_t>(sq >> (8 * (J - 16))) & 0xffu;
  return v1 ? e1 : e2;
}

template <uint32_t D>
DEV uint32_t spec_hdr_word(const uint8_t *w0, bool v1, uint64_t off, uint64_t sq) {
  return spec_hdr_byte<4 * D>(w0[4 * D], v1, off, sq) | (spec_hdr_byte<4 * D + 1>(w0[4 * D + 1], v1, off, sq) << 8) |
         (spec_hdr_byte<4 * D + 2>(w0[4 * D + 2], v1, off, sq) << 16) |
         (spec_hdr_byte<4 * D + 3>(w0[4 * D + 3], v1, off, sq) << 24);
}

struct SpecRun {
  uint32_t eligible, count, hl, crc_len, dlen, nch, T, cb0, v1;
  uint64_t stride, off0, seq0;
};

constexpr uint32_t kSpecHdrBytes = 48;

template <int COPY, int BATCH>
__global__ __launch_bounds__(1024) void spec_verify_kernel(SpecArgs a) {
  static_assert(!(COPY && BATCH), "a batch is verify only");
  __shared__ __attribute__((aligned(16))) uint32_t lds[kLdsWords + 2 + 2 * kSlots];
  __shared__ __attribute__((aligned(16))) uint8_t win[kSpecRunsMax + 1][kHdrWin];
  __shared__ SpecRun run;
  __shared__ uint64_t run_r0[kSpecRunsMax][7];
  __shared__ uint64_t run_total;
  __shared__ const uint8_t *rS[kSpecRunsMax];
  __shared__ uint64_t rN[kSpecRunsMax], rP[kSpecRunsMax], roff0[kSpecRunsMax], rseq0[kSpecRunsMax];
  __shared__ uint32_t rcount[kSpecRunsMax], rprefix[kSpecRunsMax + 1], gprefix[kSpecRunsMax + 1];
  __shared__ SpecCtl *ep_ctl;
  __shared__ SpecExc *ep_exc;
  __shared__ uint8_t *ep_hout;
  __shared__ SpecRunTail *ep_xtail;
  __shared__ uint32_t ep_seq, ep_nruns;
  __shared__ uint32_t ecnt[kEarlyWords];
  const uint32_t t = threadIdx.x, lane = t & 63u, wv = t >> 6;
  unsigned long long *const ps = kDiag && a.stamps ? a.stamps + kSpecStampOff + 8u * blockIdx.x : nullptr;
  auto stamp = [&](int ph) {
    if (kDiag && ps && t == 0) ps[ph] = __builtin_amdgcn_s_memrealtime();
  };
  stamp(0);
  const uint32_t nruns = !BATCH || a.nruns < 1u ? 1u : (a.nruns > kSpecRunsMax ? kSpecRunsMax : a.nruns);
  if (t == 0) {
    ep_ctl = a.ctl + a.parity;
    ep_exc = a.exc + a.parity * kSpecExcMax;
    ep_hout = a.hout;
    ep_xtail = a.xtail ? a.xtail + a.parity * kSpecRunsMax : nullptr;
    ep_seq = a.seq;
    ep_nruns = nruns;
  }
  SpecCtl *const ctl = a.ctl + a.parity;
  const uint64_t rem = a.len > a.base ? a.len - a.base : 0u;
  auto run_of = [&](uint32_t r, const uint8_t *&S, uint64_t &N, uint64_t &P) {
    S = a.s;
    N = a.len;
    P = rem ? a.base : 0u;
#pragma unroll
    for (uint32_t i = 1; i < kSpecRunsMax; i++)
      if (r == i) {
        S = a.xs[i];
        N = a.xlen[i];
        P = 0u;
      }
  };
  if (wv == 0) {
    const uint32_t r = lane >> 2, q = lane & 3u;
    if (r < nruns) {
      const uint8_t *S;
      uint64_t N, P;
      run_of(r, S, N, P);
      const uint64_t left = N > P ? N - P : 0u;
      if (r == 0) {
        const __amdgpu_buffer_rsrc_t rs = __builtin_amdgcn_make_buffer_rsrc(
            const_cast<uint8_t *>(a.s + (rem ? a.base : 0u)), 0, static_cast<int>(rem < kHdrWin ? rem : kHdrWin),
            0x00020000);
        *reinterpret_cast<u32x4 *>(&win[0][16 * q]) =
            __builtin_bit_cast(u32x4, __builtin_amdgcn_raw_buffer_load_b128(rs, 16u * q, 0, 0));
      } else {
        uint32_t wd[4] = {0u, 0u, 0u, 0u};
#pragma unroll
        for (uint32_t i = 0; i < 16; i++)
          if (16u * q + i < left) wd[i / 4] |= uint32_t(S[P + 16u * q + i]) << (8u * (i % 4));
        *reinterpret_cast<u32x4 *>(&win[r][16 * q]) = u32x4{wd[0], wd[1], wd[2], wd[3]};
      }
    }
  }
  fill_tables<1024, 0>(lds, a.gtab);
  if (wv == 0) {
    __builtin_amdgcn_fence(__ATOMIC_ACQUIRE, "wavefront", "local");
    const uint32_t r = lane;
    SpecRun d{};
    hdfs_crc32c_packet rr{};
    uint64_t total = 0;
    bool ok = false;
    uint32_t count = 0;
    const uint8_t *S = a.s;
    uint64_t N = 0, P = 0;
    if (r < nruns) {
      run_of(r, S, N, P);
      const uint64_t left = N > P ? N - P : 0u;
      const uint32_t hl = a.proto == HDFS_CRC32C_PROTO_V2 ? 6u + ((uint32_t(win[r][4]) << 8) | win[r][5]) : 25u;
      const bool fits = left >= 6u && hl <= kHdrWin;
      const int st = fits ? frame::frame_step(win[r], left, P, a.proto, a.cs, a.ctype, rr, total) : frame::kStepMore;
      uint32_t cb0 = 0;
      const bool rwin = a.rwin != 0 && nruns == 1u;
      const uint32_t avail0 = st == frame::kStepNext ? frame::read_avail(rr, rwin, a.client_offset, cb0) : 0u;
      ok = st == frame::kStepNext && !rr.error && !rr.last && rr.crc_len > 0 && rr.data_len > 0 &&
           a.cs % kRoundBytes == 0 && uint32_t(rr.data_len) % a.cs == 0 && total < kSpecMaxStride &&
           spec_canonical(win[r], a.proto, hl) && avail0 > 0u;
      if (ok) {
        const uint64_t by_len = left / total;
        uint64_t cnt = min<uint64_t>(by_len, a.max_count);
        if (rwin && a.copy_cap > avail0)
          cnt = min<uint64_t>(cnt, 1u + (a.copy_cap - avail0 + uint64_t(rr.data_len) - 1u) / uint64_t(rr.data_len));
        else if (rwin)
          cnt = 1u;
        count = static_cast<uint32_t>(cnt);
        ok = count >= 2u;
        d.stride = total;
        d.hl = rr.header_len;
        d.crc_len = uint32_t(rr.crc_len);
        d.dlen = uint32_t(rr.data_len);
        d.nch = uint32_t(rr.crc_len) / 4u;
        d.T = (d.nch + kTileChunks - 1u) / kTileChunks;
        d.cb0 = cb0;
        d.v1 = a.proto == HDFS_CRC32C_PROTO_V1 ? 1u : 0u;
        d.off0 = uint64_t(rr.offset_in_block);
        d.seq0 = uint64_t(rr.seqno);
      }
    }
    const uint32_t hl0 = __builtin_amdgcn_readlane(d.hl, 0), cl0 = __builtin_amdgcn_readlane(d.crc_len, 0),
                   dl0 = __builtin_amdgcn_readlane(d.dlen, 0);
    const uint64_t st0 = (uint64_t(__builtin_amdgcn_readlane(static_cast<uint32_t>(total >> 32), 0)) << 32) |
                         __builtin_amdgcn_readlane(static_cast<uint32_t>(total), 0);
    const uint32_t cnt0 = __builtin_amdgcn_readlane(count, 0);
    const bool bad = r < nruns && !(ok && d.hl == hl0 && d.crc_len == cl0 && d.dlen == dl0 && total == st0 &&
                                    (nruns == 1u || count == cnt0));
    const bool all_ok = __builtin_amdgcn_ballot_w64(bad) == 0ull;
    uint32_t pre = 0, tot = 0, gpre = 0, gtot = 0;
#pragma unroll
    for (uint32_t i = 0; i < kSpecRunsMax; i++) {
      const uint32_t ci = __builtin_amdgcn_readlane(count, i);
      if (i < nruns) {
        if (i < r) {
          pre += ci;
          gpre += (ci + 63u) / 64u;
        }
        tot += ci;
        gtot += (ci + 63u) / 64u;
      }
    }
    if (r < nruns) {
      rS[r] = S;
      rN[r] = N;
      rP[r] = P;
      roff0[r] = d.off0;
      rseq0[r] = d.seq0;
      rcount[r] = count;
      rprefix[r] = pre;
      gprefix[r] = gpre;
      const uint64_t *x = reinterpret_cast<const uint64_t *>(&rr);
#pragma unroll
      for (int q = 0; q < 7; q++) run_r0[r][q] = x[q];
    }
    if (r == 0) {
      rprefix[nruns] = tot;
      gprefix[nruns] = gtot;
      d.eligible = all_ok ? 1u : 0u;
      d.count = tot;
      run = d;
      run_total = total;
    }
    if (all_ok) {
      SpecTabData *q = a.tabs + blockIdx.x;
      if (r < nruns) q->crc0r[r] = S + P + d.hl;
      if (r == 0) {
        q->crc0 = S + P + d.hl;
        q->bm0 = a.bm;
        q->copy_base = COPY ? a.copy_base : nullptr;
        q->stride = d.stride;
        q->copy_cap = COPY ? a.copy_cap : 0u;
        q->nch = d.nch;
        q->cs = a.cs;
        q->cb0 = COPY ? d.cb0 : 0u;
        q->nruns = nruns;
        q->per = count;
        q->um = count ? ~0ull / count + 1ull : 0ull;
        q->pad = 0u;
        q->ctl = ctl;
        q->hdone = a.hout + kSpecRunDoneOff;
        q->seq = a.seq;
      }
      stores_done();
    }
    if (BATCH && r < kSpecRunsMax) ecnt[r] = 0u;
    if (BATCH && r == 0) ecnt[49] = 0u;
  }
  __syncthreads();
  stamp(1);
  SpecRun d;
  d.eligible = rfl(run.eligible);
  d.count = rfl(run.count);
  d.hl = rfl(run.hl);
  d.crc_len = rfl(run.crc_len);
  d.dlen = rfl(run.dlen);
  d.nch = rfl(run.nch);
  d.T = rfl(run.T);
  d.cb0 = rfl(run.cb0);
  d.v1 = rfl(run.v1);
  d.stride = rfl64(run.stride);
  d.off0 = rfl64(run.off0);
  d.seq0 = rfl64(run.seq0);
  if (BATCH && d.eligible) {
    const uint32_t cnt0 = rfl(rcount[0]);
    const uint32_t per_t = cnt0 * d.T, ntl = per_t * nruns;
    const uint32_t G = gridDim.x, b = blockIdx.x, pmin = (a.tune >> 16) & 0xffu;
    const bool pool = uint64_t(ntl) * (a.cs / kRoundBytes) >= uint64_t(pmin ? pmin : 32u) * G * 16u;
    const uint32_t gsh = (a.tune >> 8) & 15u, xm = (a.tune >> 12) & 3u;
    const uint32_t ng = static_cast<uint32_t>((pool ? uint64_t(ntl) * kPhase1Num / kPhase1Den : ntl) >> gsh);
    uint32_t gf, gst, nkg, p2;
    if (xm == 2u && (G % 8u) == 0 && ng >= 8u * (G / 8u)) {
      const uint32_t ngx = ng / 8u, G8 = G / 8u, l = b / 8u;
      gf = (b % 8u) * ngx + l;
      gst = G8;
      nkg = (ngx - 1u - l) / G8 + 1u;
      p2 = (ngx * 8u) << gsh;
    } else {
      gf = xm != 0u && (G % 8u) == 0 ? (b % 8u) * (G / 8u) + b / 8u : b;
      gst = G;
      nkg = ng > gf ? (ng - 1u - gf) / G + 1u : 0u;
      p2 = ng << gsh;
    }
    auto below = [&](uint32_t x) -> uint32_t {
      return x > gf ? min(nkg, (x - gf + gst - 1u) / gst) : 0u;
    };
    const bool on = a.early != 0u && nruns > 1u && (per_t & ((1u << gsh) - 1u)) == 0u &&
                    uint64_t(cnt0) * d.T * nruns < (1ull << 31);
    const uint32_t r = lane;
    uint32_t owned = 0, dis = 1;
    if (r < nruns) {
      owned = (below(((r + 1u) * per_t) >> gsh) - below((r * per_t) >> gsh)) << gsh;
      dis = (r + 1u) * per_t > p2 ? 1u : 0u;
      ecnt[16u + r] = dis ? kEarlyOff : owned;
      ecnt[32u + r] = G + (rcount[r] + 63u) / 64u;
    }
    uint32_t sum = 0;
#pragma unroll
    for (uint32_t i = 0; i < kSpecRunsMax; i++) sum += __builtin_amdgcn_readlane(owned, i);
    if (r == 0) {
      ecnt[48] = sum;
      ecnt[49] = on ? 1u : 0u;
    }
    __builtin_amdgcn_fence(__ATOMIC_RELEASE, "wavefront", "local");
    if (wv == 0 && on && r < nruns && !dis && owned == 0u)
      spec_run_contribute(ctl, a.hout + kSpecRunDoneOff, a.seq, G + (rcount[r] + 63u) / 64u, r);
  }
  if (blockIdx.x == 0 && wv == 15u) {
    if (lane < nruns && nruns > 1u) {
      auto *er = reinterpret_cast<SpecRunEarly *>(a.hout + kSpecRunEarlyOff) + lane;
#pragma unroll
      for (int q = 0; q < 7; q++) er->r0[q] = run_r0[lane][q];
      er->count = rcount[lane];
      er->early = BATCH && ecnt[49] != 0u &&
                          ecnt[16u + lane] != kEarlyOff ? 1u : 0u;
    }
    if (lane < kSpecRunsMax) {
      SpecCtl *nx = a.ctl + (a.parity ^ 1u);
      nx->run_done[lane] = 0u;
      nx->run_mism[lane] = 0u;
      if (lane == 0) nx->run_bad = 0u;
    }
    if (lane == 0) {
      SpecCtl *nx = a.ctl + (a.parity ^ 1u);
      nx->mism = 0ull;
      nx->gctr = 0u;
      nx->done = 0u;
      nx->exc = 0u;
      nx->nexc = 0u;
      auto *e = reinterpret_cast<SpecEarly *>(a.hout);
#pragma unroll
      for (int q = 0; q < 7; q++) e->r0[q] = run_r0[0][q];
      e->stride = run_total;
      e->eligible = d.eligible;
      e->count = d.count;
    }
    stores_done();
    __threadfence_system();
    if (lane == 0) __hip_atomic_store(&reinterpret_cast<SpecEarly *>(a.hout)->seq, a.seq, __ATOMIC_RELAXED,
                                      __HIP_MEMORY_SCOPE_SYSTEM);
    for (uint32_t r = 0; lane == 0 && d.eligible && r < nruns; r++) {
      const uint8_t *S = rS[r];
      const uint64_t N = rN[r], P = rP[r], cnt = rcount[r];
      uint32_t ts = kGridOn;
      uint64_t ttot = 0;
      hdfs_crc32c_packet tr{};
// ... 43 lines not shown
#pragma unroll
    for (uint32_t i = 1; i < kSpecRunsMax; i++) r += (i < nruns && g >= gprefix[i]) ? 1u : 0u;
    return rfl(r);
  };
  auto hdr_rsrc = [&](uint32_t r, uint32_t jr) {
    const uint64_t p0 = rfl64(rP[r]) + uint64_t(64u * jr) * d.stride;
    const uint64_t n = rfl64(rN[r]);
    const uint64_t span = n > p0 ? n - p0 : 0u;
    return __builtin_amdgcn_make_buffer_rsrc(
        reinterpret_cast<uint8_t *>(rfl64(reinterpret_cast<uint64_t>(rS[r] + p0))), 0,
        static_cast<int>(rfl(span > 0xFFFFFFFFull ? 0xFFFFFFFFu : static_cast<uint32_t>(span))), 0x00020000);
  };
  const uint32_t vo = lane * static_cast<uint32_t>(d.stride);
  u32x4 h0[kSpecHdrBytes / 16];
  if (j0 < ngroups) {
    const uint32_t r = group_run(j0);
    const __amdgpu_buffer_rsrc_t rs = hdr_rsrc(r, j0 - rfl(gprefix[r]));
#pragma unroll
    for (int q = 0; q < int(kSpecHdrBytes / 16); q++)
      h0[q] = __builtin_bit_cast(u32x4, __builtin_amdgcn_raw_buffer_load_b128(rs, vo + 16u * q, 0, 0));
  }
  stamp(2);
  const bool hdr_first = BATCH && rfl(ecnt[49]) != 0u;
  auto check = [&](uint32_t j, const u32x4 (&h)[kSpecHdrBytes / 16]) {
    const uint32_t r = group_run(j), jr = j - rfl(gprefix[r]);
    const uint64_t p0 = rfl64(rP[r]) + uint64_t(64u * jr) * d.stride;
    const uint32_t kr = 64u * jr + lane;
    const uint32_t cnt_r = rfl(rcount[r]);
    const uint64_t off = rfl64(roff0[r]) + uint64_t(kr) * d.dlen, sq = rfl64(rseq0[r]) + kr;
    uint32_t e[kSpecHdrBytes / 4];
    e[0] = spec_hdr_word<0>(win[0], v1, off, sq);
    e[1] = spec_hdr_word<1>(win[0], v1, off, sq);
    e[2] = spec_hdr_word<2>(win[0], v1, off, sq);
    e[3] = spec_hdr_word<3>(win[0], v1, off, sq);
    e[4] = spec_hdr_word<4>(win[0], v1, off, sq);
    e[5] = spec_hdr_word<5>(win[0], v1, off, sq);
    e[6] = spec_hdr_word<6>(win[0], v1, off, sq);
    e[7] = spec_hdr_word<7>(win[0], v1, off, sq);
    e[8] = spec_hdr_word<8>(win[0], v1, off, sq);
    e[9] = spec_hdr_word<9>(win[0], v1, off, sq);
    e[10] = spec_hdr_word<10>(win[0], v1, off, sq);
    e[11] = spec_hdr_word<11>(win[0], v1, off, sq);
    uint32_t diff = 0;
#pragma unroll
    for (uint32_t w = 0; w < kSpecHdrBytes / 4; w++) {
      const uint32_t m = 4u * w >= d.hl ? 0u : 4u * w + 4u <= d.hl ? 0xFFFFFFFFu : (1u << (8u * (d.hl - 4u * w))) - 1u;
      diff |= (h[w / 4][w % 4] ^ e[w]) & m;
    }
    if (kr < cnt_r && diff != 0u) {
      hdfs_crc32c_packet rec{};
      uint64_t tot = 0;
      const uint64_t pos = p0 + vo;
      const uint8_t *S = rS[r];
      const uint64_t N = rfl64(rN[r]);
      const int st = frame::frame_step(S + pos, N - pos, pos, a.proto, a.cs, a.ctype, rec, tot);
      bool keep = st == frame::kStepNext && !rec.error && tot == d.stride && rec.header_len == d.hl &&
                  static_cast<uint32_t>(rec.data_len) == d.dlen && static_cast<uint32_t>(rec.crc_len) == d.crc_len &&
                  (!a.rwin || static_cast<uint64_t>(rec.offset_in_block) == off);
      if (keep) {
        const uint32_t slot = __hip_atomic_fetch_add(&ctl->nexc, 1u, __ATOMIC_RELAXED, __HIP_MEMORY_SCOPE_AGENT);
        if (slot < kSpecExcMax) {
          SpecExc *x = a.exc + a.parity * kSpecExcMax + slot;
          const uint64_t *w = reinterpret_cast<const uint64_t *>(&rec);
#pragma unroll
          for (int q = 0; q < 7; q++) at_st(&x->rec[q], w[q]);
          at_st32(&x->k, rfl(rprefix[r]) + kr);
        } else {
          keep = false;
        }
      }
      if (!keep) __hip_atomic_fetch_or(&ctl->exc, 1u, __ATOMIC_RELAXED, __HIP_MEMORY_SCOPE_AGENT);
    }
    if (hdr_first) {
      if (__ballot(kr < cnt_r && diff != 0u) != 0ull) {
        if (lane == 0) __hip_atomic_fetch_or(&ctl->run_bad, 1u << r, __ATOMIC_RELAXED, __HIP_MEMORY_SCOPE_AGENT);
        stores_done();
      }
      if (lane == 0) spec_run_contribute(ctl, a.hout + kSpecRunDoneOff, a.seq, ecnt[32u + r], r);
    }
  };
  if (hdr_first && j0 < ngroups) check(j0, h0);
  const SpecTabT<BATCH != 0> tab{(const CAS SpecTabData *)(a.tabs + blockIdx.x), ecnt};
  const uint64_t tiles = uint64_t(d.count) * d.T;
  tiles_run<kModeVerify, 3, 1, 3, 1, 1024, 1, COPY, 1, 0>(lds, tab, nullptr, d.count, tiles * (a.cs / kRoundBytes),
                                                          tiles, a.fb, &ctl->mism, kDiag ? a.stamps : nullptr, a.tune,
                                                          &ctl->gctr, nullptr, d.T, false);
  for (uint32_t j = hdr_first ? j0 + 16u * G : j0; j < ngroups; j += 16u * G) {
    u32x4 h[kSpecHdrBytes / 16];
    if (j == j0) {
#pragma unroll
      for (int q = 0; q < int(kSpecHdrBytes / 16); q++) h[q] = h0[q];
    } else {
      const uint32_t r = group_run(j), jr = j - rfl(gprefix[r]);
      const __amdgpu_buffer_rsrc_t rs = hdr_rsrc(r, jr);
#pragma unroll
      for (int q = 0; q < int(kSpecHdrBytes / 16); q++)
        h[q] = __builtin_bit_cast(u32x4, __builtin_amdgcn_raw_buffer_load_b128(rs, vo + 16u * q, 0, 0));
    }
    check(j, h);
  }
  stores_done();
  __syncthreads();
  stamp(3);
  if (kDiag && BATCH && wv == 0 && lane < nruns && ecnt[49] && ecnt[16u + lane] != kEarlyOff)
    (void)DCHK(ecnt[lane] == ecnt[16u + lane], kDkSpecEarly);
  if (t < 64u) {
    SpecCtl *const c = ep_ctl;
    uint32_t n = 0;
    if (lane == 0) n = __hip_atomic_fetch_add(&c->done, 1u, __ATOMIC_RELAXED, __HIP_MEMORY_SCOPE_AGENT);
    n = static_cast<uint32_t>(__shfl(static_cast<int>(n), 0));
    if (n == gridDim.x - 1u) {
      static_assert(offsetof(SpecCtl, exc) == 16 && offsetof(SpecCtl, tail_total) == 24 &&
                        offsetof(SpecCtl, tail) == 32 && offsetof(SpecCtl, nexc) == 88 &&
                        offsetof(SpecFinal, exc) == 8 && offsetof(SpecFinal, tail_total) == 16 &&
                        offsetof(SpecFinal, tail) == 24 && offsetof(SpecFinal, seq) == 80 &&
                        offsetof(SpecFinal, nexc) == 84,
                    "the final block's dword map");
      const uint32_t src = lane < 2u ? lane : lane < 20u ? lane + 2u : 22u;
      uint32_t v = 0;
      if (lane < 22u && lane != 20u)
        v = __hip_atomic_load(reinterpret_cast<const uint32_t *>(c) + src, __ATOMIC_RELAXED, __HIP_MEMORY_SCOPE_AGENT);
      auto *f = reinterpret_cast<uint32_t *>(ep_hout + sizeof(SpecEarly));
      if (lane < 22u && lane != 20u) f[lane] = v;
      const uint32_t nexc = static_cast<uint32_t>(__shfl(static_cast<int>(v), 21));
      const uint32_t nxd = min(nexc, kSpecExcMax) * uint32_t(sizeof(SpecExc) / 4u);
      const auto *xs = reinterpret_cast<const uint32_t *>(ep_exc);
      auto *xd = reinterpret_cast<uint32_t *>(ep_hout + 256);
      for (uint32_t q = lane; q < nxd; q += 64u)
        xd[q] = __hip_atomic_load(xs + q, __ATOMIC_RELAXED, __HIP_MEMORY_SCOPE_AGENT);
      if (ep_xtail) {
        constexpr uint32_t kW = uint32_t(sizeof(SpecRunTail) / 4u);
        const auto *ts = reinterpret_cast<const uint32_t *>(ep_xtail);
        auto *td = reinterpret_cast<uint32_t *>(ep_hout + kSpecRunTailOff);
        for (uint32_t q = kW + lane; q < kW * ep_nruns; q += 64u)
          td[q] = __hip_atomic_load(ts + q, __ATOMIC_RELAXED, __HIP_MEMORY_SCOPE_AGENT);
      }
      __threadfence_system();
      if (lane == 0) __hip_atomic_store(&f[20], ep_seq, __ATOMIC_RELAXED, __HIP_MEMORY_SCOPE_SYSTEM);
      stamp(4);
    }
  }
}

hipError_t launch_spec_verify(const SpecArgs &a, int grid, int copy, hipStream_t stream) {
  if (grid < 1 || !a.seq || !a.ctl || !a.exc || !a.hout || !a.tabs || a.parity > 1u) return hipErrorInvalidValue;
  if (a.nruns > 1u && (copy || a.rwin || a.nruns > kSpecRunsMax || !a.xtail)) return hipErrorInvalidValue;
  if (a.nruns > 1u) hipLaunchKernelGGL((spec_verify_kernel<0, 1>), dim3(grid), dim3(1024), 0, stream, a);
  else if (copy) hipLaunchKernelGGL((spec_verify_kernel<1, 0>), dim3(grid), dim3(1024), 0, stream, a);
  else hipLaunchKernelGGL((spec_verify_kernel<0, 0>), dim3(grid), dim3(1024), 0, stream, a);
  return hipGetLastError();
}

__global__ __launch_bounds__(1024) void small_run_kernel(const uint8_t *__restrict__ s, uint64_t len, uint32_t count,
                                                         int proto, uint32_t cs, int ctype, int verify,
                                                         const uint32_t *__restrict__ tab,
                                                         const uint32_t *__restrict__ pow2,
                                                         uint8_t *__restrict__ copy_dst, uint64_t copy_cap,
                                                         int rwin, int64_t client_offset,
                                                         uint8_t *__restrict__ hout, uint32_t seq) {
  __shared__ uint32_t tt[1024];
  __shared__ __attribute__((aligned(16))) uint32_t zt[16 * 1024];
  __shared__ uint32_t acc[kSmallMaxChunks];
  __shared__ __attribute__((aligned(16))) uint8_t win[kSmallRunMax][kHdrWin];
  __shared__ hdfs_crc32c_packet rec;
  __shared__ uint32_t ctl[11];
  __shared__ uint32_t sdl[kSmallRunMax], son[kSmallRunMax];
  const uint32_t tid = threadIdx.x, k = blockIdx.x;
  tt[tid] = tab[tid];
  const uint32_t nfr = copy_dst ? k + 1u : 1u;
// ... 648 lines not shown
```

hadoofus_amd/csrc/crc32c_packets.cpp:

```cpp
#include "crc32c_packets.h"

#include <algorithm>
#include <cerrno>
#include <cstdio>
#include <chrono>
#include <cstdlib>
#include <cstring>
#include <deque>
#include <functional>
#include <memory>
#include <thread>
#include <vector>

#include <unistd.h>

#include "crc32c_engine.h"

namespace hdfs_crc32c {

int check_framing_args(int proto, uint32_t chunk_size, int ctype, char *errbuf, size_t errlen) {
  if (proto != HDFS_CRC32C_PROTO_V1 && proto != HDFS_CRC32C_PROTO_V2) {
    std::snprintf(errbuf, errlen, "bad packet protocol %d", proto);
    return HDFS_CRC32C_EINVAL;
  }
// ... 523 lines not shown
      return fail(HDFS_CRC32C_EHIP, "earlier work on the stream: %s", hipGetErrorString(q));
  }
  auto word = [&](uint32_t k, int i) -> const uint32_t * {
    return reinterpret_cast<const uint32_t *>(L.h + size_t(k) * kSrSlot + kGridRecBytes) + i;
  };
  using clk = std::chrono::steady_clock;
  const auto t0 = clk::now();
  for (uint32_t k = 0; k < count; k++) {
    for (uint32_t spin = 1; __atomic_load_n(word(k, 3), __ATOMIC_ACQUIRE) != seq; spin++) {
      if ((spin & 4095u) == 0 && clk::now() - t0 > std::chrono::milliseconds(200)) {
        HIPCHK(hipStreamSynchronize(L.st));
        if (__atomic_load_n(word(k, 3), __ATOMIC_ACQUIRE) != seq) return fail(HDFS_CRC32C_EHIP, "short-run kernel");
        break;
      }
#if defined(__x86_64__) || defined(__i386__)
      __builtin_ia32_pause();
#endif
    }
  }
  if (L.st == c.stream) c.confirm(epoch);
  auto rec = [&](uint32_t k) {
    hdfs_crc32c_packet r;
    std::memcpy(&r, L.h + size_t(k) * kSrSlot, sizeof(r));
    return r;
  };
  uint32_t fbk = count, unsup = 0;
  for (uint32_t k = 0; k < count; k++)
    if ((*word(k, 0) & 0xffu) != kGridOn) {
      fbk = k;
      break;
    }
  const uint32_t st_fb = fbk < count ? (*word(fbk, 0) & 0xffu) : uint32_t(kGridOn);
  const uint32_t recorded = fbk + (fbk < count && st_fb != kGridMore ? 1u : 0u);
  const hdfs_crc32c_packet r0 = rec(0);
  const uint64_t stride = recorded && (*word(0, 0) & 0xffu) == kGridOn
                              ? uint64_t(r0.header_len) + uint64_t(r0.crc_len) + uint64_t(r0.data_len)
                              : 0u;
  uint64_t next = 0, used = 0, pay = 0;
  if (fbk == count) {
    used = next = uint64_t(count) * stride;
  } else if (st_fb == kGridMore) {
    used = next = uint64_t(fbk) * stride;
  } else {
    const hdfs_crc32c_packet rf = rec(fbk);
    next = rf.stream_off + rf.header_len + uint64_t(rf.crc_len) + uint64_t(rf.data_len);
    used = rf.error ? uint64_t(fbk) * stride : next;
  }
  for (uint32_t k = 0; k < recorded; k++) unsup |= *word(k, 0) >> 8;
  const bool ended = st_fb == kGridStop || st_fb == kGridMore || (fbk == count && (count == max_pkts || next >= len));
  if (unsup || !(ended || truncated)) return 0;
  for (uint32_t k = 0; k < recorded; k++) {
    dst[k] = rec(k);
    uint32_t cb = 0;
    pay += frame::read_avail(dst[k], co.win, co.client_offset, cb);
    if (*word(k, 2)) {
      dst[k].error = HDFS_CRC32C_ERR_DATANODE_BAD_CHECKSUM;
      dst[k].first_bad = int32_t(*word(k, 1));
      dst[k].bad_chunks = *word(k, 2);
    }
  }
  if (truncated) {
    bool decided = co.win && pay >= co.cap;
    for (uint32_t k = 0; k < recorded && !decided; k++) decided = dst[k].error && dst[k].error != HDFS_CRC32C_ERR_DATANODE_BAD_CHECKSUM;
    if (!decided) decided = co.win && read_window_over(dst, recorded, co, nullptr, 0);
    if (!decided) return 0;
  }
  *nout = recorded;
  *consumed = used;
  *payload = pay;
  return 1;
}

struct SpecResult {
  std::vector<uint32_t> exc_idx;
  bool taken = false;
  bool end = false;
  uint32_t recorded = 0;
  uint64_t payload = 0;
  uint64_t consumed = 0, next = 0;
  uint32_t first_err = UINT32_MAX;
};

uint64_t g_spec_stats[4] = {0, 0, 0, 0};

int spec_alloc(DevCtx &c, SpecSlot &S) {
  if (S.ctl) return HDFS_CRC32C_OK;
  SpecCtl *ctl = nullptr;
  SpecExc *exc = nullptr;
  SpecRunTail *xtail = nullptr;
  SpecTabData *tabs = nullptr;
  uint8_t *h = nullptr, *hd = nullptr;
  hipError_t e = hipMalloc(&ctl, 2 * sizeof(SpecCtl));
  if (e == hipSuccess) e = hipMemset(ctl, 0, 2 * sizeof(SpecCtl));
  if (e == hipSuccess) e = hipMalloc(&exc, 2 * kSpecExcMax * sizeof(SpecExc));
  if (e == hipSuccess) e = hipMalloc(&xtail, 2 * kSpecRunsMax * sizeof(SpecRunTail));
  if (e == hipSuccess) e = hipMalloc(&tabs, size_t(std::max(c.num_cu, 1)) * sizeof(SpecTabData));
  if (e == hipSuccess) e = hipHostMalloc(&h, kSpecHostBytes, hipHostMallocCoherent | hipHostMallocMapped);
  if (e == hipSuccess) {
    std::memset(h, 0, kSpecHostBytes);
    e = hipHostGetDevicePointer(reinterpret_cast<void **>(&hd), h, 0);
  }
  if (e != hipSuccess) {
    if (ctl) (void)hipFree(ctl);
    if (exc) (void)hipFree(exc);
    if (xtail) (void)hipFree(xtail);
    if (tabs) (void)hipFree(tabs);
    if (h) (void)hipHostFree(h);
    return fail(HDFS_CRC32C_EHIP, "speculative verify buffers: %s", hipGetErrorString(e));
  }
  S.exc = exc;
  S.xtail = xtail;
  S.tabs = tabs;
  S.h = h;
  S.hd = hd;
  S.n = 0;
  S.ctl = ctl;
  return HDFS_CRC32C_OK;
}

int poll_seq(const uint32_t *word, uint32_t seq, const char *what, hipStream_t st) {
  using clk = std::chrono::steady_clock;
  const auto t0 = clk::now();
  for (uint32_t spin = 1; __atomic_load_n(word, __ATOMIC_ACQUIRE) != seq; spin++) {
    if ((spin & 4095u) == 0 && clk::now() - t0 > std::chrono::milliseconds(200)) {
      HIPCHK(hipStreamSynchronize(st));
      if (__atomic_load_n(word, __ATOMIC_ACQUIRE) != seq) return fail(HDFS_CRC32C_EHIP, "%s: no completion word", what);
      break;
    }
#if defined(__x86_64__) || defined(__i386__)
    __builtin_ia32_pause();
#endif
  }
  return HDFS_CRC32C_OK;
}

struct SpecLaunch {
  uint32_t seq = 0;
  int grid = 0;
  uint64_t pos = 0;
  uint8_t *bm = nullptr;
  hipStream_t st = nullptr;
  std::chrono::steady_clock::time_point t0, t1;
};

int spec_launch(DevCtx &c, SpecSlot &S, hipStream_t st, const uint8_t *d, uint64_t len, uint64_t pos,
                uint32_t max_count, int proto, uint32_t cs, int ctype, const CopyOut &co, uint64_t done_b, uint8_t *bm,
                uint32_t *fb, SpecLaunch &L, uint32_t nruns = 1, const uint8_t *const *xs = nullptr,
                const uint64_t *xlen = nullptr, bool per_run = false) {
  int rc = spec_alloc(c, S);
  if (rc) return rc;
  uint64_t left = len - pos;
  for (uint32_t r = 1; r < nruns; r++) left += xlen[r];
  const uint64_t want = (left / kRoundBytes + 63) / 64;
  L.grid = int(std::max<uint64_t>(1, std::min<uint64_t>(want, uint64_t(c.bulk_cus()))));
  L.seq = next_grid_seq(c);
  L.pos = pos;
  L.bm = bm;
  L.st = st;
  auto *early = reinterpret_cast<SpecEarly *>(S.h);
  auto *fin = reinterpret_cast<SpecFinal *>(S.h + sizeof(SpecEarly));
  __atomic_store_n(&early->seq, 0u, __ATOMIC_RELEASE);
  __atomic_store_n(&fin->seq, 0u, __ATOMIC_RELEASE);
  SpecArgs a{};
  a.s = d;
  a.len = len;
  a.base = pos;
  a.max_count = max_count;
  a.proto = proto;
  a.ctype = ctype;
  a.cs = cs;
  a.sflags = HDFS_CRC32C_SEG_BE | (ctype == HDFS_CRC32C_CSUM_CRC32 ? HDFS_CRC32C_SEG_CRC32 : 0u);
  a.rwin = co.win ? 1 : 0;
  a.client_offset = co.client_offset;
  a.bm = bm;
  a.copy_base = co.dst ? co.dst + done_b : nullptr;
  a.copy_cap = (co.dst || co.win) ? co.cap - done_b : 0u;
  a.gtab = c.d_tab_main_t[ctype == HDFS_CRC32C_CSUM_CRC32 ? 1 : 0];
  a.fb = fb;
  a.ctl = S.ctl;
  a.exc = S.exc;
  a.parity = uint32_t(S.n & 1u);
  a.seq = L.seq;
  a.tune = tile_tune() | (g_spec_pool_min << 16);
  a.hout = S.hd;
  a.tabs = S.tabs;
  a.stamps = kDiag ? g_diag : nullptr;
  a.nruns = nruns;
  a.early = per_run && nruns > 1 ? 1u : 0u;
  for (uint32_t r = 1; r < nruns; r++) {
    a.xs[r] = xs[r];
    a.xlen[r] = xlen[r];
  }
  a.xtail = S.xtail;
  L.t0 = std::chrono::steady_clock::now();
  HIPCHK(launch_spec_verify(a, L.grid, co.dst ? 1 : 0, st));
  S.n++;
  if (kDiag) g_spec_stats[0]++;
  L.t1 = std::chrono::steady_clock::now();
  return HDFS_CRC32C_OK;
}

struct EarlyHook {
  std::function<void(const hdfs_crc32c_packet *recs, uint32_t count)> fn;
};
thread_local const EarlyHook *t_early_hook = nullptr;
thread_local const std::function<void(uint32_t count, uint64_t stride)> *t_tail_hook = nullptr;

int spec_collect(DevCtx &c, SpecSlot &S, const SpecLaunch &L, const CopyOut &co, hdfs_crc32c_packet *dst,
                 SpecResult &res) {
  (void)c;
  res = SpecResult{};
  using clk = std::chrono::steady_clock;
  auto *early = reinterpret_cast<SpecEarly *>(S.h);
  auto *fin = reinterpret_cast<SpecFinal *>(S.h + sizeof(SpecEarly));
  const uint64_t pos = L.pos;
  int rc;
  if ((rc = poll_seq(&early->seq, L.seq, "speculative verify", L.st))) return rc;
  const auto t2 = clk::now();
  SpecEarly E;
  std::memcpy(&E, early, sizeof(E));
  if (!E.eligible) return HDFS_CRC32C_OK;
  if (kDiag) g_spec_stats[1]++;
  hdfs_crc32c_packet r0;
  std::memcpy(&r0, E.r0, sizeof(r0));
  for (uint32_t k = 0; k < E.count; k++) {
    hdfs_crc32c_packet &r = dst[k];
    r = r0;
    r.stream_off = pos + uint64_t(k) * E.stride;
    r.offset_in_block = r0.offset_in_block + int64_t(k) * r0.data_len;
    r.seqno = r0.seqno + int64_t(k);
  }
  if (t_early_hook && pos == 0) t_early_hook->fn(dst, E.count);
  if (t_tail_hook) (*t_tail_hook)(E.count, E.stride);
  const auto t3 = clk::now();
  if ((rc = poll_seq(&fin->seq, L.seq, "speculative verify", L.st))) return rc;
  if (g_dstream_trace) {
    auto us = [](clk::time_point x, clk::time_point y) { return std::chrono::duration<double, std::micro>(y - x).count(); };
    std::fprintf(stderr, "dstream spec grid=%d count=%u launch_us=%.1f early_us=%.1f fill_us=%.1f final_us=%.1f\n", L.grid,
                 E.count, us(L.t0, L.t1), us(L.t1, t2), us(t2, t3), us(t3, clk::now()));
  }
  SpecFinal F;
  std::memcpy(&F, fin, sizeof(F));
  if (F.exc) {
    if (kDiag) g_spec_stats[3]++;
    return HDFS_CRC32C_OK;
  }
  res.taken = true;
  if (kDiag) g_spec_stats[2]++;
  const auto *hx = reinterpret_cast<const SpecExc *>(S.h + 256);
  for (uint32_t j = 0; j < F.nexc; j++) {
    SpecExc x;
    std::memcpy(&x, hx + j, sizeof(x));
    if (x.k >= E.count) return fail(HDFS_CRC32C_EHIP, "speculative verify: exception record %u of %u", x.k, E.count);
    std::memcpy(&dst[x.k], x.rec, sizeof(hdfs_crc32c_packet));
    res.exc_idx.push_back(x.k);
    if (dst[x.k].error) res.first_err = std::min(res.first_err, x.k);
  }
  if (r0.error) res.first_err = 0;
  if (F.mism) {
    const uint32_t nch = uint32_t(r0.crc_len) / 4u, nb = (nch + 7u) / 8u;
    std::vector<uint8_t> bmh(size_t(E.count) * nb);
    HIPCHK(hipMemcpyAsync(bmh.data(), L.bm, bmh.size(), hipMemcpyDeviceToHost, L.st));
    HIPCHK(hipStreamSynchronize(L.st));
    for (uint32_t k = 0; k < E.count; k++) {
      const uint8_t *b = bmh.data() + size_t(k) * nb;
      uint32_t bad = 0;
      int32_t first = -1;
      for (uint32_t j = 0; j < nb; j++) {
        uint32_t byte = b[j];
        if (j == nch / 8u) byte &= (1u << (nch % 8u)) - 1u;
        if (!byte) continue;
        if (first < 0) first = int32_t(8u * j + uint32_t(__builtin_ctz(byte)));
        bad += uint32_t(__builtin_popcount(byte));
      }
      if (bad) {
        dst[k].error = HDFS_CRC32C_ERR_DATANODE_BAD_CHECKSUM;
        dst[k].first_bad = first;
        dst[k].bad_chunks = bad;
        if (res.first_err == UINT32_MAX) res.first_err = k;
      }
    }
  }
  uint32_t cb0 = 0;
  const uint64_t avail0 = frame::read_avail(r0, co.win, co.client_offset, cb0);
  res.payload = uint64_t(E.count - 1u) * uint64_t(r0.data_len) + avail0;
  const uint64_t run_end = pos + uint64_t(E.count) * E.stride;
  res.recorded = E.count;
  res.consumed = res.next = run_end;
  if (F.tail_status == kGridStop) {
    hdfs_crc32c_packet &t = dst[E.count];
    std::memcpy(&t, F.tail, sizeof(t));
    if (!t.error) res.consumed = run_end + F.tail_total;
    else res.first_err = std::min(res.first_err, E.count);
    res.exc_idx.push_back(E.count);
    res.recorded++;
    res.end = true;
  } else if (F.tail_status == kGridMore) {
    res.end = true;
  }
  return HDFS_CRC32C_OK;
}

struct SpecRunResult {
  bool taken = false, end = false;
  uint32_t recorded = 0;
  uint64_t consumed = 0, next = 0;
};
void predict_run(const hdfs_crc32c_packet &r0, uint32_t count, uint64_t stride, uint64_t pos0, hdfs_crc32c_packet *dst) {
  for (uint32_t k = 0; k < count; k++) {
    hdfs_crc32c_packet &q = dst[k];
    q = r0;
    q.stream_off = pos0 + uint64_t(k) * stride;
    q.offset_in_block = r0.offset_in_block + int64_t(k) * r0.data_len;
    q.seqno = r0.seqno + int64_t(k);
  }
}
void run_tail(uint32_t count, uint64_t stride, uint64_t pos0, uint32_t status, uint64_t total, const uint64_t *rec,
              hdfs_crc32c_packet *dst, SpecRunResult &o) {
  o.taken = true;
  o.recorded = count;
  const uint64_t run_end = pos0 + uint64_t(count) * stride;
  o.consumed = o.next = run_end;
  if (status == kGridStop) {
    hdfs_crc32c_packet &t = dst[count];
    std::memcpy(&t, rec, sizeof(t));
    if (!t.error) o.consumed = run_end + total;
    o.recorded++;
    o.end = true;
  } else if (status == kGridMore) {
    o.end = true;
  }
}

int spec_collect_batch(SpecSlot &S, const SpecLaunch &L, uint32_t nruns, const uint64_t *pos0,
                       hdfs_crc32c_packet *const *dst, std::vector<SpecRunResult> &res) {
  res.assign(nruns, SpecRunResult{});
  auto *early = reinterpret_cast<SpecEarly *>(S.h);
  auto *fin = reinterpret_cast<SpecFinal *>(S.h + sizeof(SpecEarly));
  int rc;
  if ((rc = poll_seq(&early->seq, L.seq, "speculative batch verify", L.st))) return rc;
  SpecEarly E;
  std::memcpy(&E, early, sizeof(E));
  if (!E.eligible) return HDFS_CRC32C_OK;
  if (kDiag) g_spec_stats[1]++;
  std::vector<SpecRunEarly> er(nruns);
  std::memcpy(er.data(), S.h + kSpecRunEarlyOff, nruns * sizeof(SpecRunEarly));
  std::vector<uint32_t> prefix(nruns + 1, 0);
  std::vector<hdfs_crc32c_packet> r0(nruns);
  for (uint32_t r = 0; r < nruns; r++) {
    std::memcpy(&r0[r], er[r].r0, sizeof(hdfs_crc32c_packet));
    prefix[r + 1] = prefix[r] + er[r].count;
    predict_run(r0[r], er[r].count, E.stride, pos0[r], dst[r]);
  }
  if (prefix[nruns] != E.count) return fail(HDFS_CRC32C_EHIP, "speculative batch: %u packets, runs hold %u", E.count,
                                            prefix[nruns]);
  if ((rc = poll_seq(&fin->seq, L.seq, "speculative batch verify", L.st))) return rc;
  SpecFinal F;
  std::memcpy(&F, fin, sizeof(F));
  if (F.exc) {
    if (kDiag) g_spec_stats[3]++;
    return HDFS_CRC32C_OK;
  }
  if (kDiag) g_spec_stats[2]++;
  auto run_of = [&](uint32_t k) {
    return uint32_t(std::upper_bound(prefix.begin(), prefix.end(), k) - prefix.begin()) - 1u;
  };
  const auto *hx = reinterpret_cast<const SpecExc *>(S.h + 256);
  for (uint32_t j = 0; j < F.nexc; j++) {
    SpecExc x;
    std::memcpy(&x, hx + j, sizeof(x));
    if (x.k >= E.count) return fail(HDFS_CRC32C_EHIP, "speculative batch: exception record %u of %u", x.k, E.count);
    const uint32_t r = run_of(x.k);
    std::memcpy(&dst[r][x.k - prefix[r]], x.rec, sizeof(hdfs_crc32c_packet));
  }
  if (F.mism) {
    const uint32_t nch = uint32_t(r0[0].crc_len) / 4u, nb = (nch + 7u) / 8u;
    std::vector<uint8_t> bmh(size_t(E.count) * nb);
    HIPCHK(hipMemcpyAsync(bmh.data(), L.bm, bmh.size(), hipMemcpyDeviceToHost, L.st));
    HIPCHK(hipStreamSynchronize(L.st));
    for (uint32_t k = 0; k < E.count; k++) {
      const uint8_t *b = bmh.data() + size_t(k) * nb;
      uint32_t bad = 0;
      int32_t first = -1;
      for (uint32_t j = 0; j < nb; j++) {
        uint32_t byte = b[j];
        if (j == nch / 8u) byte &= (1u << (nch % 8u)) - 1u;
        if (!byte) continue;
        if (first < 0) first = int32_t(8u * j + uint32_t(__builtin_ctz(byte)));
        bad += uint32_t(__builtin_popcount(byte));
      }
      if (bad) {
        const uint32_t r = run_of(k);
        hdfs_crc32c_packet &q = dst[r][k - prefix[r]];
        q.error = HDFS_CRC32C_ERR_DATANODE_BAD_CHECKSUM;
        q.first_bad = first;
        q.bad_chunks = bad;
      }
    }
  }
  std::vector<SpecRunTail> tails(nruns);
  std::memcpy(tails.data(), S.h + kSpecRunTailOff, nruns * sizeof(SpecRunTail));
  for (uint32_t r = 0; r < nruns; r++) {
    uint32_t status;
    uint64_t total;
    const uint64_t *rec;
    if (r == 0) {
      status = F.tail_status;
      total = F.tail_total;
      rec = F.tail;
    } else {
      status = tails[r].status;
      total = tails[r].total;
      rec = tails[r].rec;
    }
    run_tail(er[r].count, E.stride, pos0[r], status, total, rec, dst[r], res[r]);
  }
  return HDFS_CRC32C_OK;
}

int spec_run_early(const SpecSlot &S, const SpecLaunch &L, uint32_t i, size_t cap, hdfs_crc32c_packet *dst,
                   SpecRunResult &o) {
  const auto *early = reinterpret_cast<const SpecEarly *>(S.h);
  if (__atomic_load_n(&early->seq, __ATOMIC_ACQUIRE) != L.seq) return 0;
  if (!early->eligible) return -1;
  const auto *er = reinterpret_cast<const SpecRunEarly *>(S.h + kSpecRunEarlyOff) + i;
  if (!er->early) return -1;
  const auto *f = reinterpret_cast<const SpecRunDone *>(S.h + kSpecRunDoneOff) + i;
  if (__atomic_load_n(&f->seq, __ATOMIC_ACQUIRE) != L.seq) return 0;
  if (f->mism || f->bad) return -1;
  const auto *tl = reinterpret_cast<const SpecRunTail *>(S.h + kSpecRunTailOff) + i;
  if (__atomic_load_n(&tl->seq, __ATOMIC_ACQUIRE) != L.seq) return 0;
  SpecRunEarly e;
  SpecRunTail t;
  std::memcpy(&e, er, sizeof(e));
  std::memcpy(&t, tl, sizeof(t));
  if (size_t(e.count) + (t.status == kGridStop ? 1u : 0u) > cap) return -1;
// ... 566 lines not shown
  uint32_t m = 0;
  size_t per = 0;
  bool collected = false, single_not_taken = false;
  int rc = 0;
  std::unique_ptr<hdfs_crc32c_packet[]> recs;
  std::vector<SpecRunResult> rr;
  int refs = 0;
};
}
struct JobQueue {
  std::vector<hdfs_crc32c_job *> pending;
  struct Key {
    int proto, ctype;
    uint32_t cs;
    uint64_t len;
    size_t max_pkts;
    bool operator==(const Key &o) const {
      return proto == o.proto && ctype == o.ctype && cs == o.cs && len == o.len && max_pkts == o.max_pkts;
    }
  } key{};
  std::vector<JobGroup *> running;
  size_t outstanding = 0;
};
}

struct hdfs_crc32c_job {
  int dev = -1;
  std::vector<const uint8_t *> runs;
  std::vector<uint64_t> lens;
  bool batch = false;
  std::vector<size_t> sel;
  int proto = 0, ctype = 0;
  uint32_t cs = 0;
  size_t max_pkts = 0;
  bool queued = false;
  hdfs_crc32c::JobGroup *grp = nullptr;
  uint32_t grp_run = 0;
};

namespace hdfs_crc32c {
namespace {

JobQueue &jobq(DevCtx &c) {
  if (!c.jobq) c.jobq = new JobQueue;
  return *c.jobq;
}

bool group_done(DevCtx &c, const JobGroup &g) {
  const SpecSlot &S = c.job_slot[g.slot];
  const auto *early = reinterpret_cast<const SpecEarly *>(S.h);
  const auto *fin = reinterpret_cast<const SpecFinal *>(S.h + sizeof(SpecEarly));
  if (__atomic_load_n(&early->seq, __ATOMIC_ACQUIRE) != g.L.seq) return false;
  if (!__atomic_load_n(&early->eligible, __ATOMIC_RELAXED)) return true;
  return __atomic_load_n(&fin->seq, __ATOMIC_ACQUIRE) == g.L.seq;
}

int group_collect(DevCtx &c, JobQueue &q, JobGroup *g) {
  if (g->collected) return g->rc;
  SpecSlot &S = c.job_slot[g->slot];
  g->recs.reset(new (std::nothrow) hdfs_crc32c_packet[g->per * g->m]);
  g->rr.assign(g->m, SpecRunResult{});
  if (!g->recs) {
    g->collected = true;
    g->rc = fail(HDFS_CRC32C_ENOMEM, "records of %u runs", g->m);
    (void)hipStreamSynchronize(S.stream);
    c.job_busy[g->slot] = false;
    q.running.erase(std::remove(q.running.begin(), q.running.end(), g), q.running.end());
    return g->rc;
  }
  int rc;
  if (g->m == 1) {
    SpecResult sr;
    rc = spec_collect(c, S, g->L, CopyOut{}, g->recs.get(), sr);
    g->rr[0].taken = sr.taken;
    g->rr[0].end = sr.end;
    g->rr[0].recorded = sr.recorded;
    g->rr[0].consumed = sr.consumed;
    g->rr[0].next = sr.next;
    g->single_not_taken = !sr.taken;
  } else {
    std::vector<hdfs_crc32c_packet *> dst(g->m);
    std::vector<uint64_t> pos0(g->m, 0);
    for (uint32_t r = 0; r < g->m; r++) dst[r] = g->recs.get() + r * g->per;
    rc = spec_collect_batch(S, g->L, g->m, pos0.data(), dst.data(), g->rr);
  }
  g->collected = true;
  g->rc = rc;
  c.job_busy[g->slot] = false;
  q.running.erase(std::remove(q.running.begin(), q.running.end(), g), q.running.end());
  return rc;
}

JobGroup *group_launch(DevCtx &c, JobQueue &q, const uint8_t *const *streams, const uint64_t *lens, uint32_t m,
                       int proto, uint32_t cs, int ctype, size_t max_pkts, int *rcp, bool early) {
  int slot = -1;
  for (;;) {
    for (int i = 0; i < kMaxJobs && slot < 0; i++)
      if (!c.job_busy[i]) slot = i;
    if (slot >= 0 || q.running.empty()) break;
    JobGroup *old = q.running.front();
    (void)group_collect(c, q, old);
    if (old->refs == 0) delete old;
  }
  if (slot < 0) {
    *rcp = fail(HDFS_CRC32C_EHIP, "no free job slot");
    return nullptr;
  }
  SpecSlot &S = c.job_slot[slot];
  if (!S.stream) {
    uint64_t avoid[kMaxJobs + 1] = {c.q_main};
    for (int i = 0; i < kMaxJobs; i++) avoid[i + 1] = c.job_slot[i].q;
    int rq;
    if ((rq = stream_on_own_queue(c, &S.stream, &S.q, avoid, kMaxJobs + 1))) {
      *rcp = rq;
      return nullptr;
    }
  }
  const uint32_t count = uint32_t(std::min<uint64_t>(uint64_t(max_pkts), kGridMaxCount));
  uint64_t bm_cap = 64, fbw = 0;
  for (uint32_t r = 0; r < m; r++) {
    const uint64_t cr = std::min<uint64_t>(count, lens[r] / 6 + 1);
    bm_cap += lens[r] / 32 + cr;
    fbw += cr;
  }
  bm_cap = align_up(bm_cap, 256);
  const uint64_t need = bm_cap + fbw * 4u + 256u;
  if (need > S.scratch_cap) {
    if (S.scratch) (void)hipFree(S.scratch);
    S.scratch = nullptr;
    S.scratch_cap = 0;
    if (hipMalloc(&S.scratch, need) != hipSuccess) {
      (void)hipGetLastError();
      *rcp = fail(HDFS_CRC32C_ENOMEM, "job scratch of %llu bytes", (unsigned long long)need);
      return nullptr;
    }
    S.scratch_cap = need;
  }
  auto *g = new (std::nothrow) JobGroup;
  if (!g) {
    *rcp = fail(HDFS_CRC32C_ENOMEM, "job launch");
    return nullptr;
  }
  g->slot = slot;
  g->m = m;
  g->per = size_t(count) + 1;
  int rc = spec_launch(c, S, S.stream, streams[0], lens[0], 0, count, proto, cs, ctype, CopyOut{}, 0, S.scratch,
                       reinterpret_cast<uint32_t *>(S.scratch + bm_cap), g->L, m, streams, lens, early);
  if (rc) {
    delete g;
    *rcp = rc;
    return nullptr;
  }
  c.job_busy[slot] = true;
  q.running.push_back(g);
  *rcp = HDFS_CRC32C_OK;
  return g;
}

void queue_flush(DevCtx &c, JobQueue &q) {
  if (q.pending.empty()) return;
  std::vector<const uint8_t *> s;
  std::vector<uint64_t> l;
  for (hdfs_crc32c_job *j : q.pending) {
    s.push_back(j->runs[0]);
    l.push_back(j->lens[0]);
  }
  int rc = 0;
// ... 1188 lines not shown
        if (consumed) *consumed = used;
        if (delivered) *delivered = got_all;
        return fail(HDFS_CRC32C_EIO, "pwrite to fd %d at %lld: %s", fd, (long long)(fd_offset + int64_t(got_all)),
                    e ? std::strerror(e) : "wrote nothing (end of file)");
      }
      w += uint64_t(k);
    }
    got_all += got;
    if (rc != HDFS_CRC32C_AGAIN) break;
  }
  hdfs_crc32c_reader_close(rd);
  if (rc < 0) return rc;
  if (npkts) *npkts = n_all;
  if (consumed) *consumed = used;
  if (delivered) *delivered = got_all;
  return rc;
}

int hdfs_crc32c_verify_packets_submit(const void *stream, uint64_t len, int proto, uint32_t chunk_size, int ctype,
                                      size_t max_pkts, hdfs_crc32c_job **job) {
  if (!job) return fail(HDFS_CRC32C_EINVAL, "null job");
  *job = nullptr;
  int rc = check_framing_args(proto, chunk_size, ctype, g_err, sizeof(g_err));
  if (rc) return rc;
  if (!stream || !len) return fail(HDFS_CRC32C_EINVAL, "empty stream");
  const uint8_t *s = static_cast<const uint8_t *>(stream);
  return job_submit(&s, &len, 1, false, proto, chunk_size, ctype, max_pkts, job);
}

int hdfs_crc32c_verify_blocks_submit(const void *const *streams, const uint64_t *lens, size_t nblocks, int proto,
                                     uint32_t chunk_size, int ctype, size_t max_pkts, hdfs_crc32c_job **job) {
  if (!job) return fail(HDFS_CRC32C_EINVAL, "null job");
  *job = nullptr;
  int rc = check_framing_args(proto, chunk_size, ctype, g_err, sizeof(g_err));
  if (rc) return rc;
  if (!streams || !lens || nblocks < 1 || nblocks > kSpecRunsMax)
    return fail(HDFS_CRC32C_EINVAL, "blocks: 1 to %u streams (%zu given)", kSpecRunsMax, nblocks);
  for (size_t b = 0; b < nblocks; b++)
    if (!streams[b] || !lens[b]) return fail(HDFS_CRC32C_EINVAL, "block %zu: empty stream", b);
  return job_submit(reinterpret_cast<const uint8_t *const *>(streams), lens, nblocks, true, proto, chunk_size, ctype,
                    max_pkts, job);
}

int hdfs_crc32c_job_wait(hdfs_crc32c_job *job, hdfs_crc32c_packet *pkts, size_t max_pkts, size_t *npkts,
                         uint64_t *consumed) {
  if (npkts) *npkts = 0;
  if (consumed) *consumed = 0;
  if (!job) return fail(HDFS_CRC32C_EINVAL, "null job");
  if (job->batch) return fail(HDFS_CRC32C_EINVAL, "a job of blocks: hdfs_crc32c_job_wait_blocks");
  if (max_pkts && !pkts) return fail(HDFS_CRC32C_EINVAL, "null packet array");
  size_t n = 0;
  uint64_t used = 0;
  int rcb = 0;
  const int rc = job_wait(job, pkts, max_pkts, &n, &used, &rcb);
  if (rc < 0) return rc;
  if (npkts) *npkts = n;
  if (consumed) *consumed = used;
  return rc;
}

int hdfs_crc32c_job_wait_blocks(hdfs_crc32c_job *job, hdfs_crc32c_packet *pkts, size_t max_pkts, size_t *npkts,
                                uint64_t *consumed, int *rcs) {
  if (!job) return fail(HDFS_CRC32C_EINVAL, "null job");
  const size_t n = job->runs.size();
  if (!npkts || !consumed || !rcs || (max_pkts && !pkts))
    return fail(HDFS_CRC32C_EINVAL, "null output arrays (%zu blocks)", n);
  for (size_t b = 0; b < n; b++) {
    npkts[b] = 0;
    consumed[b] = 0;
    rcs[b] = 0;
  }
  return job_wait(job, pkts, max_pkts, npkts, consumed, rcs);
}

#ifdef HDFS_CRC32C_DIAG
int hdfs_crc32c_diag_spec_stats(uint64_t *out4, int reset) {
  if (!out4) return fail(HDFS_CRC32C_EINVAL, "null out4");
  for (int i = 0; i < 4; i++) {
    out4[i] = g_spec_stats[i];
    if (reset) g_spec_stats[i] = 0;
  }
  return HDFS_CRC32C_OK;
}
#endif

int hdfs_crc32c_compose_packets(const void *data, uint64_t len, int64_t offset_in_block, int64_t seqno, int proto,
                                int ctype, int finish, void *hdr_out, uint64_t hdr_cap, hdfs_crc32c_out_packet *pkts,
                                size_t max_pkts, size_t *npkts, uint64_t *hdr_used) {
  if (npkts) *npkts = 0;
  if (hdr_used) *hdr_used = 0;
  if (proto != HDFS_CRC32C_PROTO_V1 && proto != HDFS_CRC32C_PROTO_V2)
    return fail(HDFS_CRC32C_EINVAL, "proto must be 1 or 2");
  if (ctype != HDFS_CRC32C_CSUM_NULL && ctype != HDFS_CRC32C_CSUM_CRC32 && ctype != HDFS_CRC32C_CSUM_CRC32C)
    return fail(HDFS_CRC32C_EINVAL, "bad checksum type %d", ctype);
  if (offset_in_block < 0) return fail(HDFS_CRC32C_EINVAL, "negative block offset");
  if (len && !data) return fail(HDFS_CRC32C_EINVAL, "null data");
  std::vector<OutPlan> plan;
  plan_out_packets(len, offset_in_block, seqno, finish != 0, plan);
  const bool csum = ctype != HDFS_CRC32C_CSUM_NULL;
  const uint32_t hb = out_header_bytes(proto);
  uint64_t need = 0;
  for (const OutPlan &k : plan)
    need += hb + (csum ? 4ull * ((uint64_t(k.dlen) + kWriteChunk - 1) / kWriteChunk) : 0ull);
  if (npkts) *npkts = plan.size();
  if (hdr_used) *hdr_used = need;
  if (!hdr_out || !pkts) return HDFS_CRC32C_OK;
  if (max_pkts < plan.size() || hdr_cap < need)
    return fail(HDFS_CRC32C_EINVAL, "need %zu packets / %llu header bytes", plan.size(), (unsigned long long)need);
  std::vector<uint32_t> head, body;
  uint64_t n0 = 0;
  if (csum && len) {
    n0 = (offset_in_block % kWriteChunk) ? uint64_t(plan[0].dlen) : 0;
    if (n0) {
      head.resize(1);
      int rc = chunk_crcs_to_host(data, n0, uint32_t(n0), ctype, head.data());
      if (rc) return rc;
    }
    if (len > n0) {
      body.resize((len - n0 + kWriteChunk - 1) / kWriteChunk);
      int rc = chunk_crcs_to_host(static_cast<const uint8_t *>(data) + n0, len - n0, kWriteChunk, ctype,
                                  body.data());
      if (rc) return rc;
    }
  }
  uint8_t *out = static_cast<uint8_t *>(hdr_out);
  uint64_t pos = 0;
  for (size_t i = 0; i < plan.size(); i++) {
    const OutPlan &k = plan[i];
    const uint64_t ncrc = csum ? (uint64_t(k.dlen) + kWriteChunk - 1) / kWriteChunk : 0;
    uint8_t *p = out + pos;
    p = put_be(p, uint64_t(uint32_t(int32_t(k.dlen + 4 * ncrc + 4))), 4);
    if (proto == HDFS_CRC32C_PROTO_V2) {
      p = put_be(p, kHdrProtoBytes, 2);
      p = put_header_proto(p, k.offset, k.seqno, k.last, k.dlen);
    } else {
      p = put_be(p, uint64_t(k.offset), 8);
      p = put_be(p, uint64_t(k.seqno), 8);
      *p++ = k.last ? 1 : 0;
      p = put_be(p, uint32_t(k.dlen), 4);
    }
    if (ncrc) {
      const uint32_t *src = (n0 && i == 0) ? head.data() : body.data() + (k.data_off - n0) / kWriteChunk;
      std::memcpy(p, src, size_t(ncrc) * 4);
      p += ncrc * 4;
    }
    hdfs_crc32c_out_packet &o = pkts[i];
    std::memset(&o, 0, sizeof(o));
    o.hdr_off = pos;
    o.data_off = k.data_off;
    o.offset_in_block = k.offset;
    o.seqno = k.seqno;
    o.data_len = k.dlen;
    o.hdr_len = uint32_t(p - (out + pos));
    o.crc_len = uint32_t(ncrc * 4);
    o.last = k.last ? 1 : 0;
    pos += o.hdr_len;
  }
  return HDFS_CRC32C_OK;
}

int hdfs_crc32c_session_create(hdfs_crc32c_session **out, int proto, uint32_t chunk_size, int ctype,
                               uint64_t slot_bytes, size_t nslots) {
  if (!out) return fail(HDFS_CRC32C_EINVAL, "null session pointer");
  *out = nullptr;
  if (proto != HDFS_CRC32C_PROTO_V1 && proto != HDFS_CRC32C_PROTO_V2)
    return fail(HDFS_CRC32C_EINVAL, "bad packet protocol %d", proto);
// ... 96 lines not shown
```

include/hadoofus_crc32c_diag.h:

```cpp
#ifndef HADOOFUS_CRC32C_DIAG_H
#define HADOOFUS_CRC32C_DIAG_H

#include "hadoofus_crc32c.h"

#ifdef __cplusplus
extern "C" {
#endif
int hdfs_crc32c_set_tile_order(int order);
int hdfs_crc32c_set_group_shift(int shift);
int hdfs_crc32c_set_xcd_major(int on);
int hdfs_crc32c_set_tuning(int nt_loads, void *diag);
int hdfs_crc32c_set_depth(int depth);
int hdfs_crc32c_set_shape(int streams, int block);
int hdfs_crc32c_set_store_policy(int policy);
int hdfs_crc32c_set_runs(int on);
int hdfs_crc32c_set_speculation(int on);
int hdfs_crc32c_set_job_coalesce(int mode);
int hdfs_crc32c_set_job_early(int on);
int hdfs_crc32c_diag_job_early(uint64_t *out2, int reset);
int hdfs_crc32c_diag_spec_stats(uint64_t *out4, int reset);
int hdfs_crc32c_diag_stream_queries(uint64_t *out);
int hdfs_crc32c_diag_stream_queues(uint64_t *out4);
int hdfs_crc32c_diag_job_queues(uint64_t *out4);
int hdfs_crc32c_diag_device_checks(uint32_t *out3, int reset);
int hdfs_crc32c_probe_read(const void *dptr, uint64_t bytes, void *stream, int iters, double *gbps);
int hdfs_crc32c_set_probe(int variant, int grid_per_cu, int block);


#ifdef __cplusplus
}
#endif
#endif
```

Measured before the change: 6566 GiB/s.

## Prime speculative verify loads using a host-side layout hint from the previous call

The host records the packet layout (header length, data length, CRC length, stride) seen in the last speculative verify and passes it to the next launch as a hint. Early workgroups use the hint to start issuing the first tile loads of the CRC pipeline before header parsing confirms the layout, then hand those in-flight buffers to tiles_run. If the parsed layout differs, the primed state is dropped. This hides the header-parse latency at kernel start, at the cost of extra registers, code complexity, and possibly wasted loads when the hint is wrong.

```diff
diff --git a/hadoofus_amd/abi.py b/hadoofus_amd/abi.py
--- a/hadoofus_amd/abi.py
+++ b/hadoofus_amd/abi.py
@@ -190,6 +190,9 @@
     _bind(lib, "hdfs_crc32c_set_job_early", _int, [_int])
     _bind(lib, "hdfs_crc32c_diag_job_early", _int, [ctypes.POINTER(_u64), _int])
     _bind(lib, "hdfs_crc32c_diag_spec_stats", _int, [ctypes.POINTER(_u64), _int])
+    if hasattr(lib, "hdfs_crc32c_set_spec_hint"):
+        _bind(lib, "hdfs_crc32c_set_spec_hint", _int, [_int])
+        _bind(lib, "hdfs_crc32c_diag_spec_hint_stats", _int, [ctypes.POINTER(_u64), _int])
     _bind(lib, "hdfs_crc32c_diag_stream_queries", _int, [ctypes.POINTER(_u64)])
     _bind(lib, "hdfs_crc32c_diag_stream_queues", _int, [ctypes.POINTER(_u64)])
     _bind(lib, "hdfs_crc32c_diag_job_queues", _int, [ctypes.POINTER(_u64)])
diff --git a/hadoofus_amd/csrc/crc32c_engine.cpp b/hadoofus_amd/csrc/crc32c_engine.cpp
--- a/hadoofus_amd/csrc/crc32c_engine.cpp
+++ b/hadoofus_amd/csrc/crc32c_engine.cpp
@@ -59,6 +59,7 @@
 uint64_t g_mb_copy_max = uint64_t(HDFS_KNOB("HDFS_CRC32C_MB_COPY_MAX", 96 << 10));
 int g_runs = HDFS_KNOB("HDFS_CRC32C_RUNS", 2);
 int g_spec = HDFS_KNOB("HDFS_CRC32C_SPEC", 1);
+int g_spec_hint = HDFS_KNOB("HDFS_CRC32C_SPEC_HINT", 1);
 int g_job_coalesce = HDFS_KNOB("HDFS_CRC32C_JOB_COALESCE", 1);
 int g_job_early = HDFS_KNOB("HDFS_CRC32C_JOB_EARLY", 1);
 std::atomic<uint64_t> g_job_early_stats[2];
@@ -1522,6 +1523,12 @@
   return HDFS_CRC32C_OK;
 }
 
+int hdfs_crc32c_set_spec_hint(int on) {
+  if (on != 0 && on != 1) return fail(HDFS_CRC32C_EINVAL, "layout hint 0 or 1");
+  g_spec_hint = on;
+  return HDFS_CRC32C_OK;
+}
+
 int hdfs_crc32c_diag_job_queues(uint64_t *out4) {
   DevCtx *c = nullptr;
   int rc = ctx_init(-1, &c);
diff --git a/hadoofus_amd/csrc/crc32c_engine.h b/hadoofus_amd/csrc/crc32c_engine.h
--- a/hadoofus_amd/csrc/crc32c_engine.h
+++ b/hadoofus_amd/csrc/crc32c_engine.h
@@ -59,6 +59,7 @@
                              unsigned long long *stamps = nullptr);
 hipError_t launch_spec_verify(const SpecArgs &a, int grid, int copy, hipStream_t stream);
 extern int g_spec;
+extern int g_spec_hint;
 extern int g_job_coalesce;
 extern int g_job_early;
 extern std::atomic<uint64_t> g_job_early_stats[2];
@@ -211,6 +212,7 @@
   uint64_t mb_calls = 0, mb_launches = 0;
   std::vector<hipStream_t> user_streams;
   int bulk_cus() const { return num_cu - (mb_on ? num_xcd : 0); }
+  SpecHint spec_hint;
   std::mutex mu;
 };
 
diff --git a/hadoofus_amd/csrc/crc32c_internal.h b/hadoofus_amd/csrc/crc32c_internal.h
--- a/hadoofus_amd/csrc/crc32c_internal.h
+++ b/hadoofus_amd/csrc/crc32c_internal.h
@@ -18,6 +18,7 @@
   kDkSmallRun = 4,
   kDkFinalize = 5,
   kDkSpecEarly = 6,
+  kDkSpecHint = 7,
 };
 
 enum : uint32_t {
@@ -185,6 +186,13 @@
   const uint8_t *xs[kSpecRunsMax];
   uint64_t xlen[kSpecRunsMax];
   SpecRunTail *xtail;
+  uint32_t hint_hl, hint_dlen, hint_crc_len, hint_pad;
+  uint64_t hint_stride;
+};
+struct SpecHint {
+  int proto = 0, ctype = 0;
+  uint32_t cs = 0, hl = 0, dlen = 0, crc_len = 0;
+  uint64_t stride = 0;
 };
 constexpr size_t kSpecStampOff = 98304;
 constexpr uint64_t kSpecMaxStride = uint64_t(1) << 26;
diff --git a/hadoofus_amd/csrc/crc32c_kernels.hip b/hadoofus_amd/csrc/crc32c_kernels.hip
--- a/hadoofus_amd/csrc/crc32c_kernels.hip
+++ b/hadoofus_amd/csrc/crc32c_kernels.hip
@@ -114,6 +114,33 @@
 
 constexpr uint32_t kEarlyWords = 50, kEarlyOff = 0xFFFFFFFFu;
 
+DEV SegDev spec_seg(const SpecTabData &q, const uint8_t *c, uint32_t k) {
+  SegDev d;
+  const uint32_t T = (q.nch + kTileChunks - 1u) / kTileChunks, dlen = q.nch * q.cs;
+  d.data = c + 4u * q.nch;
+  d.crcs = reinterpret_cast<uint32_t *>(const_cast<uint8_t *>(c));
+  d.bitmap = q.bm0 + static_cast<uint64_t>(k) * T;
+  d.mtile_start = static_cast<uint64_t>(k) * T;
+  d.chunk_size = q.cs;
+  d.flags = kSegBigEndian;
+  d.nchunks = q.nch;
+  d.main_tiles = T;
+  d.reg_init = 0xFFFFFFFFu;
+  d.gen_tiles = 0u;
+  d.len = dlen;
+  d.round_start = static_cast<uint64_t>(k) * T * (q.cs / kRoundBytes);
+  d.gtile_start = 0u;
+  const uint32_t w0 = k ? 0u : q.cb0;
+  const uint64_t before = k ? static_cast<uint64_t>(k) * dlen - q.cb0 : 0u;
+  uint64_t at = 0;
+  uint32_t clen = 0;
+  frame::read_place(before, dlen - w0, q.copy_cap, at, clen);
+  d.copy_dst = q.copy_base && clen ? q.copy_base + at : nullptr;
+  d.copy_w0 = w0;
+  d.copy_w1 = w0 + clen;
+  return d;
+}
+
 template <bool BATCH>
 struct SpecTabT {
   const CAS SpecTabData *p;
@@ -139,7 +166,6 @@
     }
   }
   DEV SegDev operator[](uint32_t k) const {
-    SegDev d;
     SpecTabData q;
     q.crc0 = p->crc0;
     q.bm0 = p->bm0;
@@ -149,7 +175,6 @@
     q.nch = p->nch;
     q.cs = p->cs;
     q.cb0 = p->cb0;
-    const uint32_t T = (q.nch + kTileChunks - 1u) / kTileChunks, dlen = q.nch * q.cs;
     const uint8_t *c;
     if constexpr (BATCH) {
       const uint32_t r = static_cast<uint32_t>(__umul64hi(static_cast<uint64_t>(k), p->um));
@@ -157,31 +182,30 @@
     } else {
       c = q.crc0 + static_cast<uint64_t>(k) * q.stride;
     }
-    d.data = c + 4u * q.nch;
-    d.crcs = reinterpret_cast<uint32_t *>(const_cast<uint8_t *>(c));
-    d.bitmap = q.bm0 + static_cast<uint64_t>(k) * T;
-    d.mtile_start = static_cast<uint64_t>(k) * T;
-    d.chunk_size = q.cs;
-    d.flags = kSegBigEndian;
-    d.nchunks = q.nch;
-    d.main_tiles = T;
-    d.reg_init = 0xFFFFFFFFu;
-    d.gen_tiles = 0u;
-    d.len = dlen;
-    d.round_start = static_cast<uint64_t>(k) * T * (q.cs / kRoundBytes);
-    d.gtile_start = 0u;
-    const uint32_t w0 = k ? 0u : q.cb0;
-    const uint64_t before = k ? static_cast<uint64_t>(k) * dlen - q.cb0 : 0u;
-    uint64_t at = 0;
-    uint32_t clen = 0;
-    frame::read_place(before, dlen - w0, q.copy_cap, at, clen);
-    d.copy_dst = q.copy_base && clen ? q.copy_base + at : nullptr;
-    d.copy_w0 = w0;
-    d.copy_w1 = w0 + clen;
-    return d;
+    return spec_seg(q, c, k);
   }
 };
 using SpecTab = SpecTabT<false>;
+struct SpecHintTab {
+  const uint8_t *crc0;
+  uint8_t *bm0;
+  uint64_t stride;
+  uint32_t nch, cs;
+  DEV SegDev operator[](uint32_t k) const {
+    SpecTabData q;
+    q.bm0 = bm0;
+    q.copy_base = nullptr;
+    q.copy_cap = 0u;
+    q.nch = nch;
+    q.cs = cs;
+    q.cb0 = 0u;
+    return spec_seg(q, crc0 + static_cast<uint64_t>(k) * stride, k);
+  }
+};
+DEV SegHot seg_hot(const SpecHintTab &t, uint32_t k) {
+  const SegDev d = t[k];
+  return SegHot{d.data, d.crcs, d.bitmap, d.mtile_start, d.chunk_size, d.flags, d.nchunks, d.main_tiles};
+}
 template <class Tab>
 struct TabEarly {
   static constexpr bool value = false;
@@ -260,14 +284,17 @@
 }
 
 template <int ORDER>
+DEV uint64_t static_tile(const Sched &w, uint32_t t) {
+  if (ORDER == 4 || ORDER == 7) return (w.gfirst + uint64_t(t) * w.gstride) << w.gshift;
+  if (ORDER == 3)
+    return ((w.gfirst + uint64_t(t >> w.gshift) * w.gstride) << w.gshift) + (t & ((1u << w.gshift) - 1u));
+  return w.gfirst + t;
+}
+
+template <int ORDER>
 DEV bool ticket_tile(const Sched &w, uint32_t t, uint64_t &g) {
   if (t < w.nk) {
-    if (ORDER == 4 || ORDER == 7)
-      g = (w.gfirst + uint64_t(t) * w.gstride) << w.gshift;
-    else if (ORDER == 3)
-      g = ((w.gfirst + uint64_t(t >> w.gshift) * w.gstride) << w.gshift) + (t & ((1u << w.gshift) - 1u));
-    else
-      g = w.gfirst + t;
+    g = static_tile<ORDER>(w, t);
     return true;
   }
   if (ORDER < 2) return false;
@@ -914,50 +941,58 @@
   }
 }
 
+template <int BLOCK>
+struct TabRegs {
+  static constexpr uint32_t kStores = kLdsSliceBytes / 16;
+  static constexpr uint32_t kQ = (kStores + BLOCK - 1) / BLOCK;
+  static constexpr uint32_t kZ = (kTabZposWords / 4 + BLOCK - 1) / BLOCK;
+  uint32_t v[kQ];
+  u32x4 z[kZ];
+};
 template <int BLOCK, int GATHER>
-DEV void fill_tables(uint32_t *lds, const uint32_t *__restrict__ gtab) {
+DEV void fill_tables_zero(uint32_t *lds) {
   if (threadIdx.x < 2 + 2 * kSlots) lds[kLdsWords + threadIdx.x] = 0u;
   if (GATHER && threadIdx.x < kGatherSlots) lds[kLdsWords + 2 + 2 * kSlots + threadIdx.x] = threadIdx.x << 4;
-  constexpr uint32_t kStores = kLdsSliceBytes / 16;
-  constexpr uint32_t kQ = (kStores + BLOCK - 1) / BLOCK;
-  constexpr uint32_t kZ = (kTabZposWords / 4 + BLOCK - 1) / BLOCK;
-  uint32_t v[kQ];
+}
+template <int BLOCK>
+DEV void fill_tables_load(const uint32_t *__restrict__ gtab, TabRegs<BLOCK> &t) {
+  constexpr uint32_t kStores = TabRegs<BLOCK>::kStores, kQ = TabRegs<BLOCK>::kQ, kZ = TabRegs<BLOCK>::kZ;
 #pragma unroll
   for (uint32_t k = 0; k < kQ; k++) {
     const uint32_t idx = 4u * min(k * BLOCK + threadIdx.x, kStores - 1u);
     const uint32_t P = idx >> 14, e = (idx >> 6) & 255u, h = (idx >> 5) & 1u;
-    v[k] = gtab[(3u - (2u * P + h)) * 256u + e];
-  }
-  u32x4 z[kZ];
+    t.v[k] = gtab[(3u - (2u * P + h)) * 256u + e];
+  }
 #pragma unroll
   for (uint32_t k = 0; k < kZ; k++) {
     const uint32_t q = k * BLOCK + threadIdx.x;
-    z[k] = q < kTabZposWords / 4 ? gload16(gtab + kTabSliceWords + 4u * q) : u32x4{0u, 0u, 0u, 0u};
-  }
+    t.z[k] = q < kTabZposWords / 4 ? gload16(gtab + kTabSliceWords + 4u * q) : u32x4{0u, 0u, 0u, 0u};
+  }
+}
+template <int BLOCK>
+DEV void fill_tables_store(uint32_t *lds, const TabRegs<BLOCK> &t) {
+  constexpr uint32_t kStores = TabRegs<BLOCK>::kStores, kQ = TabRegs<BLOCK>::kQ, kZ = TabRegs<BLOCK>::kZ;
 #pragma unroll
   for (uint32_t k = 0; k < kQ; k++) {
     const uint32_t q = k * BLOCK + threadIdx.x;
     if (kStores % BLOCK == 0 || q < kStores)
-      *reinterpret_cast<u32x4 *>(&lds[4u * q]) = u32x4{v[k], v[k], v[k], v[k]};
+      *reinterpret_cast<u32x4 *>(&lds[4u * q]) = u32x4{t.v[k], t.v[k], t.v[k], t.v[k]};
   }
 #pragma unroll
   for (uint32_t k = 0; k < kZ; k++) {
     const uint32_t q = k * BLOCK + threadIdx.x;
-    if (q < kTabZposWords / 4) *reinterpret_cast<u32x4 *>(&lds[kLdsSliceBytes / 4 + 4u * q]) = z[k];
-  }
-}
-
-template <int MODE, int ORDER, int NT, int DEPTH, int S, int BLOCK, int BUF, int COPY, int UNA, int GATHER,
-          class Tab>
-DEV void tiles_run(uint32_t *lds, const Tab sg, const SegDev *__restrict__ segs, uint32_t nseg, uint64_t total_rounds,
-                   uint64_t total_tiles, uint32_t *__restrict__ first_bad, unsigned long long *__restrict__ mism,
-                   unsigned long long *__restrict__ diag, uint32_t tune, uint32_t *__restrict__ gctr,
-                   const GridSummary *__restrict__ dyn, uint32_t utiles, bool fused) {
-  static_assert(ORDER != 0 || S == 1, "static per-wave slices serve one stream");
-  static_assert(ORDER != 7 || (MODE == kModeCompute && S == 1 && BUF && !COPY && !UNA && !GATHER), "columns shape");
-  static_assert(DEPTH >= 2 && DEPTH <= 4 && S >= 1 && S <= 4, "shape");
-  static_assert(GATHER == 0 || (MODE == kModeCompute && ORDER == 3 && S == 1), "gather: compute, schedule 3");
-  LaneConst L;
+    if (q < kTabZposWords / 4) *reinterpret_cast<u32x4 *>(&lds[kLdsSliceBytes / 4 + 4u * q]) = t.z[k];
+  }
+}
+template <int BLOCK, int GATHER>
+DEV void fill_tables(uint32_t *lds, const uint32_t *__restrict__ gtab) {
+  fill_tables_zero<BLOCK, GATHER>(lds);
+  TabRegs<BLOCK> t;
+  fill_tables_load<BLOCK>(gtab, t);
+  fill_tables_store<BLOCK>(lds, t);
+}
+
+DEV void lane_const(LaneConst &L, uint32_t *lds, uint32_t tune, uint64_t total_tiles) {
   L.store_policy = EP::policy(tune & 0xffu);
   L.lane = threadIdx.x & 63u;
   L.hsel = (L.lane >> 3) & 1u;
@@ -974,17 +1009,98 @@
   L.gslot = &lds[kLdsWords + 2 + 2 * kSlots];
   L.rmask = 7u;
   L.early = 0u;
+}
+
+DEV Sched sched_init(uint32_t *lds, uint32_t lane, uint32_t utiles) {
+  Sched w{0, 0, 0, &lds[kLdsWords], lane};
+  w.ut = utiles;
+  w.ush = (utiles & (utiles - 1u)) == 0u ? static_cast<uint32_t>(__builtin_ctz(utiles | (utiles == 0u ? 1u : 0u)))
+                                         : 0xFFFFFFFFu;
+  w.um = (utiles && w.ush == 0xFFFFFFFFu) ? ~0ull / utiles + 1ull : 0ull;
+  return w;
+}
+
+template <int ORDER, int S>
+DEV bool pool_on(uint64_t total_rounds, uint32_t nwaves, uint32_t tune) {
+  const uint32_t pmin = (tune >> 16) & 0xffu;
+  return ORDER >= 2 && total_rounds >= uint64_t(pmin ? pmin : 32u) * nwaves * S;
+}
+
+template <int ORDER>
+DEV void deal_static(Sched &w, uint64_t total_tiles, bool pool, uint32_t tune) {
+  const uint64_t ngroups = (pool ? total_tiles * kPhase1Num / kPhase1Den : total_tiles) >> w.gshift;
+  const uint32_t b = blockIdx.x, G = gridDim.x, xm = (tune >> 12) & 3u;
+  if (xm == 2u && (G % 8u) == 0 && ngroups >= 8ull * (G / 8u)) {
+    const uint64_t ngx = ngroups / 8u;
+    const uint32_t G8 = G / 8u, l = b / 8u;
+    w.gfirst = (b % 8u) * ngx + l;
+    w.gstride = G8;
+    w.nk = static_cast<uint32_t>(((ngx - 1 - l) / G8 + 1) << (ORDER == 4 || ORDER == 7 ? 0u : w.gshift));
+    w.p2first = (ngx * 8u) << w.gshift;
+  } else {
+    w.gfirst = xm != 0u && (G % 8u) == 0 ? (b % 8u) * (G / 8u) + b / 8u : b;
+    w.gstride = gridDim.x;
+    w.nk = ngroups > w.gfirst
+               ? static_cast<uint32_t>(((ngroups - 1 - w.gfirst) / gridDim.x + 1) << (ORDER == 4 || ORDER == 7 ? 0u : w.gshift))
+               : 0u;
+    w.p2first = ngroups << w.gshift;
+  }
+}
+
+template <int DEPTH>
+DEV uint32_t fixed_tickets(uint32_t rpt) {
+  return (DEPTH + rpt - 1u) / rpt;
+}
+template <int ORDER, int DEPTH>
+DEV void fixed_cursors(const Sched &w, uint32_t slot, uint32_t nslots, uint32_t rpt, Cursor (&c)[DEPTH]) {
+  uint32_t j = 0, r = 0;
+#pragma unroll
+  for (int k = 0; k < DEPTH; k++) {
+    if (k && ++r == rpt) {
+      r = 0;
+      j++;
+    }
+    const uint32_t tk = slot + j * nslots;
+    c[k] = ulocate(w, static_tile<ORDER>(w, tk));
+    c[k].r = r;
+    c[k].grp = tk >> 3;
+  }
+}
+
+struct NoPre {
+  static constexpr bool on = false;
+};
+template <int DEPTH>
+struct SpecPre {
+  static constexpr bool on = true;
+  bool primed;
+  uint32_t slot, nslots, rpt;
+  uint32_t buf[DEPTH][16], ex[DEPTH], tl[DEPTH], sha[DEPTH];
+};
+
+template <int MODE, int ORDER, int NT, int DEPTH, int S, int BLOCK, int BUF, int COPY, int UNA, int GATHER,
+          class Tab, class PRE = NoPre>
+DEV void tiles_run(uint32_t *lds, const Tab sg, const SegDev *__restrict__ segs, uint32_t nseg, uint64_t total_rounds,
+                   uint64_t total_tiles, uint32_t *__restrict__ first_bad, unsigned long long *__restrict__ mism,
+                   unsigned long long *__restrict__ diag, uint32_t tune, uint32_t *__restrict__ gctr,
+                   const GridSummary *__restrict__ dyn, uint32_t utiles, bool fused, PRE *pre = nullptr) {
+  static_assert(ORDER != 0 || S == 1, "static per-wave slices serve one stream");
+  static_assert(ORDER != 7 || (MODE == kModeCompute && S == 1 && BUF && !COPY && !UNA && !GATHER), "columns shape");
+  static_assert(DEPTH >= 2 && DEPTH <= 4 && S >= 1 && S <= 4, "shape");
+  static_assert(GATHER == 0 || (MODE == kModeCompute && ORDER == 3 && S == 1), "gather: compute, schedule 3");
+  static_assert(!PRE::on || (ORDER == 3 && S == 1), "primed rounds: schedule 3, one stream");
+  LaneConst L;
+  lane_const(L, lds, tune, total_tiles);
 
   constexpr uint32_t wpb = BLOCK / 64;
   const uint32_t wave = rfl(blockIdx.x * wpb + (threadIdx.x >> 6));
   const uint32_t nwaves = gridDim.x * wpb;
   if (kDiag && diag && L.lane == 0) diag[3 * wave] = __builtin_amdgcn_s_memrealtime();
   uint64_t nrounds = 0;
-  Sched w{0, 0, 0, &lds[kLdsWords], L.lane};
-  w.ut = utiles;
-  w.ush = (utiles & (utiles - 1u)) == 0u ? static_cast<uint32_t>(__builtin_ctz(utiles | (utiles == 0u ? 1u : 0u)))
-                                         : 0xFFFFFFFFu;
-  w.um = (utiles && w.ush == 0xFFFFFFFFu) ? ~0ull / utiles + 1ull : 0ull;
+  Sched w = sched_init(lds, L.lane, utiles);
+  bool primed = false;
+  if constexpr (PRE::on) primed = rfl(pre->primed ? 1u : 0u) != 0u;
+  Cursor fixed[DEPTH];
   Cursor cur[DEPTH][S];
 #pragma unroll
   for (int s = 0; s < S; s++) cur[0][s] = Cursor{0u, 0u, 0u, false};
@@ -1005,28 +1121,11 @@
       }
     }
   } else {
-    const uint32_t pmin = (tune >> 16) & 0xffu;
-    const bool pool = ORDER >= 2 && total_rounds >= uint64_t(pmin ? pmin : 32u) * nwaves * S;
+    const bool pool = pool_on<ORDER, S>(total_rounds, nwaves, tune);
     if (ORDER >= 3) {
       w.gshift = ORDER == 7 ? kColShift : ORDER == 4 ? min((tune >> 8) & 15u, 3u) : (tune >> 8) & 15u;
       if (ORDER == 4) L.rmask = (1u << w.gshift) - 1u;
-      const uint64_t ngroups = (pool ? total_tiles * kPhase1Num / kPhase1Den : total_tiles) >> w.gshift;
-      const uint32_t b = blockIdx.x, G = gridDim.x, xm = (tune >> 12) & 3u;
-      if (xm == 2u && (G % 8u) == 0 && ngroups >= 8ull * (G / 8u)) {
-        const uint64_t ngx = ngroups / 8u;
-        const uint32_t G8 = G / 8u, l = b / 8u;
-        w.gfirst = (b % 8u) * ngx + l;
-        w.gstride = G8;
-        w.nk = static_cast<uint32_t>(((ngx - 1 - l) / G8 + 1) << (ORDER == 4 || ORDER == 7 ? 0u : w.gshift));
-        w.p2first = (ngx * 8u) << w.gshift;
-      } else {
-        w.gfirst = xm != 0u && (G % 8u) == 0 ? (b % 8u) * (G / 8u) + b / 8u : b;
-        w.gstride = gridDim.x;
-        w.nk = ngroups > w.gfirst
-                   ? static_cast<uint32_t>(((ngroups - 1 - w.gfirst) / gridDim.x + 1) << (ORDER == 4 || ORDER == 7 ? 0u : w.gshift))
-                   : 0u;
-        w.p2first = ngroups << w.gshift;
-      }
+      deal_static<ORDER>(w, total_tiles, pool, tune);
     } else {
       const uint64_t r_static = pool ? total_rounds * kPhase1Num / kPhase1Den : total_rounds;
       const uint64_t b0 = rfl64(r_static * blockIdx.x / gridDim.x);
@@ -1045,8 +1144,13 @@
     }
     w.gctr = gctr;
     w.slots = reinterpret_cast<uint64_t *>(&lds[kLdsWords + 2]);
-#pragma unroll
-    for (int s = 0; s < S; s++) {
+    if constexpr (PRE::on)
+      if (primed) {
+        fixed_cursors<ORDER, DEPTH>(w, pre->slot, pre->nslots, pre->rpt, fixed);
+        cur[0][0] = fixed[0];
+      }
+#pragma unroll
+    for (int s = 0; s < S && !primed; s++) {
       uint64_t g;
       const uint32_t tk = grab(w);
       if (ticket_tile<ORDER>(w, tk, g)) {
@@ -1091,13 +1195,25 @@
     gs[s] = Gst{0u, 0u, 0u, 0u, kNoSlot, 0u, 0u, 0u, 0u, nullptr};
     kc[s].seg = 0xFFFFFFFFu;
   }
-#pragma unroll
-  for (int k = 1; k < DEPTH; k++) {
+  if constexpr (PRE::on)
+    if (primed) {
+#pragma unroll
+      for (int k = 0; k < DEPTH; k++) {
+        cur[k][0] = fixed[k];
+#pragma unroll
+        for (int i = 0; i < 16; i++) buf[k][0][i] = pre->buf[k][i];
+        ex[k][0] = pre->ex[k];
+        tl[k][0] = pre->tl[k];
+        sha[k][0] = pre->sha[k];
+      }
+    }
+#pragma unroll
+  for (int k = 1; k < DEPTH && !primed; k++) {
 #pragma unroll
     for (int s = 0; s < S; s++) cur[k][s] = advance<ORDER>(cur[k - 1][s], sg, nseg, w, kc[s]);
   }
 #pragma unroll
-  for (int k = 0; k < DEPTH; k++) {
+  for (int k = 0; k < DEPTH && !primed; k++) {
 #pragma unroll
     for (int s = 0; s < S; s++) {
       ex[k][s] = 0u;
@@ -2401,6 +2517,7 @@
   __shared__ SpecRunTail *ep_xtail;
   __shared__ uint32_t ep_seq, ep_nruns;
   __shared__ uint32_t ecnt[kEarlyWords];
+  __shared__ uint32_t early_ok[16];
   const uint32_t t = threadIdx.x, lane = t & 63u, wv = t >> 6;
   unsigned long long *const ps = kDiag && a.stamps ? a.stamps + kSpecStampOff + 8u * blockIdx.x : nullptr;
   auto stamp = [&](int ph) {
@@ -2430,6 +2547,7 @@
         P = 0u;
       }
   };
+  u32x4 wd0{0u, 0u, 0u, 0u};
   if (wv == 0) {
     const uint32_t r = lane >> 2, q = lane & 3u;
     if (r < nruns) {
@@ -2441,19 +2559,107 @@
         const __amdgpu_buffer_rsrc_t rs = __builtin_amdgcn_make_buffer_rsrc(
             const_cast<uint8_t *>(a.s + (rem ? a.base : 0u)), 0, static_cast<int>(rem < kHdrWin ? rem : kHdrWin),
             0x00020000);
-        *reinterpret_cast<u32x4 *>(&win[0][16 * q]) =
-            __builtin_bit_cast(u32x4, __builtin_amdgcn_raw_buffer_load_b128(rs, 16u * q, 0, 0));
+        wd0 = __builtin_bit_cast(u32x4, __builtin_amdgcn_raw_buffer_load_b128(rs, 16u * q, 0, 0));
       } else {
         uint32_t wd[4] = {0u, 0u, 0u, 0u};
 #pragma unroll
         for (uint32_t i = 0; i < 16; i++)
           if (16u * q + i < left) wd[i / 4] |= uint32_t(S[P + 16u * q + i]) << (8u * (i % 4));
-        *reinterpret_cast<u32x4 *>(&win[r][16 * q]) = u32x4{wd[0], wd[1], wd[2], wd[3]};
-      }
-    }
-  }
-  fill_tables<1024, 0>(lds, a.gtab);
-  if (wv == 0) {
+        wd0 = u32x4{wd[0], wd[1], wd[2], wd[3]};
+      }
+    }
+  }
+  fill_tables_zero<1024, 0>(lds);
+  TabRegs<1024> tabregs;
+  fill_tables_load<1024>(a.gtab, tabregs);
+  constexpr int kDepth = 3;
+  uint32_t eslots = blockIdx.x == 0 ? 14u : 15u;
+  SpecPre<kDepth> pre;
+  pre.primed = false;
+  pre.slot = pre.nslots = pre.rpt = 0u;
+  SpecRun hint{};
+  Sched hw{};
+  bool early_wg = false;
+  uint32_t early_ctr = 0u;
+  if constexpr (!COPY && !BATCH) {
+    const uint32_t nch = a.hint_crc_len / 4u;
+    const uint64_t hcount = a.hint_stride ? min<uint64_t>(rem / a.hint_stride, a.max_count) : 0u;
+    if (a.hint_stride != 0u && a.hint_stride < kSpecMaxStride && !a.rwin && a.nruns <= 1u && nch != 0u &&
+        (a.hint_crc_len & 3u) == 0u && a.cs != 0u && a.cs % kRoundBytes == 0 &&
+        uint64_t(nch) * a.cs == uint64_t(a.hint_dlen) && a.hint_hl <= kHdrWin &&
+        uint64_t(a.hint_hl) + a.hint_crc_len + a.hint_dlen <= a.hint_stride && hcount >= 2u) {
+      hint.eligible = 1u;
+      hint.count = static_cast<uint32_t>(hcount);
+      hint.hl = a.hint_hl;
+      hint.crc_len = a.hint_crc_len;
+      hint.dlen = a.hint_dlen;
+      hint.nch = nch;
+      hint.T = (nch + kTileChunks - 1u) / kTileChunks;
+      hint.stride = a.hint_stride;
+      const uint32_t rpt = a.cs / kRoundBytes, nfix = fixed_tickets<kDepth>(rpt);
+      const uint64_t tiles = uint64_t(hint.count) * hint.T;
+      hw = sched_init(lds, lane, hint.T);
+      hw.gshift = (a.tune >> 8) & 15u;
+      deal_static<3>(hw, tiles, pool_on<3, 1>(tiles * rpt, gridDim.x * 16u, a.tune), a.tune);
+      eslots = min(eslots, hw.nk / nfix);
+      early_wg = tiles < (1ull << 32) && eslots >= 1u;
+      early_ctr = early_wg ? eslots * nfix : 0u;
+    }
+  }
+  fill_tables_store<1024>(lds, tabregs);
+  const bool wave0 = rfl(wv) == 0u;
+  const bool early_wave = !COPY && !BATCH && early_wg && rfl(wv) >= 1u && rfl(wv) <= eslots;
+  bool early_bad = false;
+  if (!wave0) {
+    if (early_wave) {
+      const uint32_t rpt = a.cs / kRoundBytes;
+      const uint64_t tiles = uint64_t(hint.count) * hint.T;
+      pre.slot = rfl(wv) - 1u;
+      pre.nslots = eslots;
+      pre.rpt = rpt;
+      LaneConst L;
+      lane_const(L, lds, a.tune, tiles);
+      const SpecHintTab htab{a.s + a.base + hint.hl, a.bm, hint.stride, hint.nch, a.cs};
+      Cursor c[kDepth];
+      fixed_cursors<3, kDepth>(hw, pre.slot, eslots, rpt, c);
+      if (kDiag) {
+#pragma unroll
+        for (int k = 0; k < kDepth; k++) {
+          const SegDev sd = htab[c[k].seg];
+          const uint32_t n = min(kTileChunks, sd.nchunks - c[k].tile * kTileChunks);
+          const uint8_t *lo = reinterpret_cast<const uint8_t *>(sd.crcs);
+          const uint8_t *hi = sd.data + uint64_t(c[k].tile) * kTileChunks * a.cs + uint64_t(c[k].r) * kRoundBytes +
+                              uint64_t(n - 1u) * a.cs + kRoundBytes;
+          (void)lo;
+          (void)hi;
+          if (!DCHK(c[k].seg < hint.count && c[k].tile < hint.T && c[k].r < rpt && lo >= a.s + a.base &&
+                        hi <= a.s + a.len,
+                    kDkSpecHint)) {
+            early_bad = true;
+            c[k] = Cursor{0u, 0u, 0u, true};
+          }
+        }
+      }
+      LaneOff lo{0u, {0u, 0u, 0u, 0u}, 0u};
+      SegCache kc;
+      kc.seg = 0xFFFFFFFFu;
+#pragma unroll
+      for (int k = 0; k < kDepth; k++) {
+        pre.ex[k] = 0u;
+        pre.tl[k] = 0u;
+        pre.sha[k] = 0u;
+        issue<kModeVerify, 1, 1, 1, false>(pre.buf[k], pre.ex[k], pre.tl[k], pre.sha[k], c[k], htab, L.hsel, L.loff, L.qg,
+                                           L.lane, lo, kc, L.store_policy);
+        if (k + 1 < kDepth) pad_store(a.fb);
+      }
+      pre.primed = true;
+      if (kDiag && ps && lane == 0 && pre.slot == 0u) ps[5] = __builtin_amdgcn_s_memrealtime();
+    }
+  } else {
+    {
+      const uint32_t r = lane >> 2, q = lane & 3u;
+      if (r < nruns) *reinterpret_cast<u32x4 *>(&win[r][16 * q]) = wd0;
+    }
     __builtin_amdgcn_fence(__ATOMIC_ACQUIRE, "wavefront", "local");
     const uint32_t r = lane;
     SpecRun d{};
@@ -2562,7 +2768,9 @@
     }
     if (BATCH && r < kSpecRunsMax) ecnt[r] = 0u;
     if (BATCH && r == 0) ecnt[49] = 0u;
-  }
+    if (early_wg && lane == 0) lds[kLdsWords] = early_ctr;
+  }
+  if (kDiag && early_wg && lane == 0) early_ok[wv] = early_bad ? 0u : 1u;
   __syncthreads();
   stamp(1);
   SpecRun d;
@@ -2578,6 +2786,19 @@
   d.stride = rfl64(run.stride);
   d.off0 = rfl64(run.off0);
   d.seq0 = rfl64(run.seq0);
+  if (early_wg) {
+    bool same = d.eligible == 1u && d.hl == hint.hl && d.crc_len == hint.crc_len && d.dlen == hint.dlen &&
+                d.stride == hint.stride && d.count == hint.count && d.T == hint.T;
+    if (kDiag) {
+      uint32_t okv = lane < 16u ? early_ok[lane] : 1u;
+      same = same && __builtin_amdgcn_ballot_w64(okv == 0u) == 0ull;
+    }
+    if (!same) {
+      pre.primed = false;
+      if (t == 0) lds[kLdsWords] = 0u;
+      __syncthreads();
+    }
+  }
   if (BATCH && d.eligible) {
     const uint32_t cnt0 = rfl(rcount[0]);
     const uint32_t per_t = cnt0 * d.T, ntl = per_t * nruns;
@@ -2787,9 +3008,10 @@
   if (hdr_first && j0 < ngroups) check(j0, h0);
   const SpecTabT<BATCH != 0> tab{(const CAS SpecTabData *)(a.tabs + blockIdx.x), ecnt};
   const uint64_t tiles = uint64_t(d.count) * d.T;
-  tiles_run<kModeVerify, 3, 1, 3, 1, 1024, 1, COPY, 1, 0>(lds, tab, nullptr, d.count, tiles * (a.cs / kRoundBytes),
-                                                          tiles, a.fb, &ctl->mism, kDiag ? a.stamps : nullptr, a.tune,
-                                                          &ctl->gctr, nullptr, d.T, false);
+  tiles_run<kModeVerify, 3, 1, kDepth, 1, 1024, 1, COPY, 1, 0>(lds, tab, nullptr, d.count,
+                                                               tiles * (a.cs / kRoundBytes), tiles, a.fb, &ctl->mism,
+                                                               kDiag ? a.stamps : nullptr, a.tune, &ctl->gctr, nullptr,
+                                                               d.T, false, &pre);
   for (uint32_t j = hdr_first ? j0 + 16u * G : j0; j < ngroups; j += 16u * G) {
     u32x4 h[kSpecHdrBytes / 16];
     if (j == j0) {
diff --git a/hadoofus_amd/csrc/crc32c_packets.cpp b/hadoofus_amd/csrc/crc32c_packets.cpp
--- a/hadoofus_amd/csrc/crc32c_packets.cpp
+++ b/hadoofus_amd/csrc/crc32c_packets.cpp
@@ -629,6 +629,7 @@
 };
 
 uint64_t g_spec_stats[4] = {0, 0, 0, 0};
+uint64_t g_spec_hint_stats[3] = {0, 0, 0};
 
 int spec_alloc(DevCtx &c, SpecSlot &S) {
   if (S.ctl) return HDFS_CRC32C_OK;
@@ -688,7 +689,23 @@
   uint8_t *bm = nullptr;
   hipStream_t st = nullptr;
   std::chrono::steady_clock::time_point t0, t1;
+  SpecHint key;
+  SpecHint hint;
 };
+
+void spec_hint_update(DevCtx &c, const SpecLaunch &L, const hdfs_crc32c_packet &r0, uint64_t stride) {
+  SpecHint h = L.key;
+  h.hl = uint32_t(r0.header_len);
+  h.dlen = uint32_t(r0.data_len);
+  h.crc_len = uint32_t(r0.crc_len);
+  h.stride = stride;
+  if (kDiag && L.hint.stride)
+    g_spec_hint_stats[h.hl == L.hint.hl && h.dlen == L.hint.dlen && h.crc_len == L.hint.crc_len &&
+                              h.stride == L.hint.stride
+                          ? 1
+                          : 2]++;
+  c.spec_hint = h;
+}
 
 int spec_launch(DevCtx &c, SpecSlot &S, hipStream_t st, const uint8_t *d, uint64_t len, uint64_t pos,
                 uint32_t max_count, int proto, uint32_t cs, int ctype, const CopyOut &co, uint64_t done_b, uint8_t *bm,
@@ -739,6 +756,19 @@
     a.xlen[r] = xlen[r];
   }
   a.xtail = S.xtail;
+  L.key = SpecHint{};
+  L.key.proto = proto;
+  L.key.ctype = ctype;
+  L.key.cs = cs;
+  L.hint = SpecHint{};
+  const SpecHint &h = c.spec_hint;
+  if (g_spec_hint && nruns == 1 && !co.win && !co.dst && h.stride && h.proto == proto && h.ctype == ctype && h.cs == cs)
+    L.hint = h;
+  a.hint_hl = L.hint.hl;
+  a.hint_dlen = L.hint.dlen;
+  a.hint_crc_len = L.hint.crc_len;
+  a.hint_stride = L.hint.stride;
+  if (kDiag && L.hint.stride) g_spec_hint_stats[0]++;
   L.t0 = std::chrono::steady_clock::now();
   HIPCHK(launch_spec_verify(a, L.grid, co.dst ? 1 : 0, st));
   S.n++;
@@ -755,7 +785,6 @@
 
 int spec_collect(DevCtx &c, SpecSlot &S, const SpecLaunch &L, const CopyOut &co, hdfs_crc32c_packet *dst,
                  SpecResult &res) {
-  (void)c;
   res = SpecResult{};
   using clk = std::chrono::steady_clock;
   auto *early = reinterpret_cast<SpecEarly *>(S.h);
@@ -766,10 +795,14 @@
   const auto t2 = clk::now();
   SpecEarly E;
   std::memcpy(&E, early, sizeof(E));
-  if (!E.eligible) return HDFS_CRC32C_OK;
+  if (!E.eligible) {
+    if (kDiag && L.hint.stride) g_spec_hint_stats[2]++;
+    return HDFS_CRC32C_OK;
+  }
   if (kDiag) g_spec_stats[1]++;
   hdfs_crc32c_packet r0;
   std::memcpy(&r0, E.r0, sizeof(r0));
+  spec_hint_update(c, L, r0, E.stride);
   for (uint32_t k = 0; k < E.count; k++) {
     hdfs_crc32c_packet &r = dst[k];
     r = r0;
@@ -879,7 +912,7 @@
   }
 }
 
-int spec_collect_batch(SpecSlot &S, const SpecLaunch &L, uint32_t nruns, const uint64_t *pos0,
+int spec_collect_batch(DevCtx &c, SpecSlot &S, const SpecLaunch &L, uint32_t nruns, const uint64_t *pos0,
                        hdfs_crc32c_packet *const *dst, std::vector<SpecRunResult> &res) {
   res.assign(nruns, SpecRunResult{});
   auto *early = reinterpret_cast<SpecEarly *>(S.h);
@@ -899,6 +932,7 @@
     prefix[r + 1] = prefix[r] + er[r].count;
     predict_run(r0[r], er[r].count, E.stride, pos0[r], dst[r]);
   }
+  spec_hint_update(c, L, r0[0], E.stride);
   if (prefix[nruns] != E.count) return fail(HDFS_CRC32C_EHIP, "speculative batch: %u packets, runs hold %u", E.count,
                                             prefix[nruns]);
   if ((rc = poll_seq(&fin->seq, L.seq, "speculative batch verify", L.st))) return rc;
@@ -1631,7 +1665,7 @@
     std::vector<hdfs_crc32c_packet *> dst(g->m);
     std::vector<uint64_t> pos0(g->m, 0);
     for (uint32_t r = 0; r < g->m; r++) dst[r] = g->recs.get() + r * g->per;
-    rc = spec_collect_batch(S, g->L, g->m, pos0.data(), dst.data(), g->rr);
+    rc = spec_collect_batch(c, S, g->L, g->m, pos0.data(), dst.data(), g->rr);
   }
   g->collected = true;
   g->rc = rc;
@@ -2986,6 +3020,15 @@
   }
   return HDFS_CRC32C_OK;
 }
+
+int hdfs_crc32c_diag_spec_hint_stats(uint64_t *out3, int reset) {
+  if (!out3) return fail(HDFS_CRC32C_EINVAL, "null out3");
+  for (int i = 0; i < 3; i++) {
+    out3[i] = g_spec_hint_stats[i];
+    if (reset) g_spec_hint_stats[i] = 0;
+  }
+  return HDFS_CRC32C_OK;
+}
 #endif
 
 int hdfs_crc32c_compose_packets(const void *data, uint64_t len, int64_t offset_in_block, int64_t seqno, int proto,
diff --git a/include/hadoofus_crc32c_diag.h b/include/hadoofus_crc32c_diag.h
--- a/include/hadoofus_crc32c_diag.h
+++ b/include/hadoofus_crc32c_diag.h
@@ -19,6 +19,8 @@
 int hdfs_crc32c_set_job_early(int on);
 int hdfs_crc32c_diag_job_early(uint64_t *out2, int reset);
 int hdfs_crc32c_diag_spec_stats(uint64_t *out4, int reset);
+int hdfs_crc32c_set_spec_hint(int on);
+int hdfs_crc32c_diag_spec_hint_stats(uint64_t *out3, int reset);
 int hdfs_crc32c_diag_stream_queries(uint64_t *out);
 int hdfs_crc32c_diag_stream_queues(uint64_t *out4);
 int hdfs_crc32c_diag_job_queues(uint64_t *out4);
```

New measurement: 6513 GiB/s, median of 2. No clear change (-0.8%).
